# lzhangbj/ASVA

Measured on AMD Instinct MI355X. Metric: UNet denoising steps/sec, 12x256x256 bf16, CFG on, higher is better.
Workload: dtype bf16; 1 GPU; BASELINE configs[1]: AVSync15 shape, 1 clip(s) per GPU per forward, 12x256x256 (latent 12x32x32), SD1.5-shaped AudioUNet3D 1.17B params random-init, CFG batch 2 (audio guidance 4.0), DDIM-50 schedule, step = UNet forward + guidance + scheduler update; clips_per_gpu=1, unet_batch=2, frames=12, launch=hipGraph replay, parallelism=dp1 (independent clips)

## Files before the change

### asva_amd/_lib.py

```python
from __future__ import annotations

import ctypes as C
import os

import torch

from . import precision as P

_HERE = os.path.dirname(os.path.abspath(__file__))
LIB_PATH = os.environ.get("AVSD_LIB_PATH") or os.path.join(_HERE, "libavsd_hip.so")
LIB_PATHS = {"bf16": LIB_PATH, "fp16": os.environ.get("AVSD_LIB_PATH_F16") or os.path.join(_HERE, "libavsd_hip_f16.so")}

c_void_p, c_int, c_float, c_int64 = C.c_void_p, C.c_int, C.c_float, C.c_int64


class GemmDesc(C.Structure):

    _fields_ = [
        ("A", c_void_p), ("A2", c_void_p), ("W", c_void_p), ("out", c_void_p),
        ("bias", c_void_p), ("rowvec", c_void_p), ("res1", c_void_p), ("res2", c_void_p),
        ("M", C.c_int32), ("N", C.c_int32), ("K", C.c_int32),
        ("lda", C.c_int32), ("lda2", C.c_int32), ("k_split", C.c_int32), ("ldw", C.c_int32),
        ("ldc", C.c_int32), ("ldr1", C.c_int32), ("ldr2", C.c_int32),
        ("rows_per_vec", C.c_int32), ("ldv", C.c_int32),
        ("alpha", C.c_float),
        ("mode", C.c_int32), ("flags", C.c_int32), ("batch", C.c_int32),
        ("batch_stride_a", C.c_int64), ("batch_stride_w", C.c_int64), ("batch_stride_out", C.c_int64),
        ("hw", C.c_int32), ("frames", C.c_int32), ("cseg", C.c_int32),
        ("hs", C.c_int32), ("ws", C.c_int32), ("ho", C.c_int32), ("wo", C.c_int32),
        ("cin", C.c_int32), ("stride", C.c_int32), ("ups", C.c_int32), ("pad", C.c_int32),
        ("tile", C.c_int32),
        ("split_k", C.c_int32), ("splitk_ws", c_void_p),
        ("rowstats", c_void_p), ("ln_stats", c_void_p), ("ln_colsum", c_void_p), ("ln_nblk", C.c_int32), ("ln_eps", C.c_float),
        ("out_master", c_void_p), ("ldm", C.c_int32), ("raster_g", C.c_int32),
        ("a_lo", C.c_int64), ("a2_lo", C.c_int64), ("w_lo", C.c_int64), ("out_lo", C.c_int64), ("res1_lo", C.c_int64),
        ("res2_lo", C.c_int64),
        ("stats_pos", c_void_p), ("ln_rowvec", c_void_p), ("pos_hw", C.c_int32), ("pos_frames", C.c_int32),
    ]


class XAttnDesc(C.Structure):

    _fields_ = [
        ("h", c_void_p), ("ldh", C.c_int32), ("res_f32", C.c_int32),
        ("res", c_void_p), ("ldres", C.c_int32),
        ("M", C.c_int32), ("C", C.c_int32), ("heads", C.c_int32), ("L", C.c_int32),
        ("ln_stats", c_void_p), ("ln_eps", C.c_float), ("scale", C.c_float),
        ("wq", c_void_p), ("ldwq", C.c_int32), ("lk", C.c_int32),
        ("q_colsum", c_void_p), ("q_bias", c_void_p),
        ("k", c_void_p), ("vt", c_void_p),
        ("lk_pad", C.c_int32), ("q_per_kv", C.c_int32),
        ("wo", c_void_p), ("ldwo", C.c_int32), ("ldo", C.c_int32),
        ("o_bias", c_void_p), ("out", c_void_p),
        ("out_master", c_void_p), ("ldm", C.c_int32), ("reserved0", C.c_int32),
        ("rowstats", c_void_p),
        ("stats_pos", c_void_p), ("pos_hw", C.c_int32), ("pos_frames", C.c_int32),
    ]


SIGNATURES = {
    "avsd_abi_version": (c_int, []),
    "avsd_precision": (C.c_char_p, []),
    "avsd_last_error": (C.c_char_p, []),
    "avsd_device_info": (c_int, [C.c_char_p, c_int, C.POINTER(c_int)]),
    "avsd_gemm_bf16": (c_int, [C.POINTER(GemmDesc), c_void_p]),
    "avsd_sizeof_gemm_desc": (c_int, []),
    "avsd_cross_attention_block": (c_int, [C.POINTER(XAttnDesc), c_void_p]),
    "avsd_gemm_conv3r_supported": (c_int, [c_int, c_int, c_int, c_int]),
    "avsd_gemm_conv3r2d_supported": (c_int, [c_int, c_int, c_int, c_int]),
    "avsd_cross_attention_block_supported": (c_int, [c_int, c_int, c_int]),
    "avsd_sizeof_xattn_desc": (c_int, []),
    "avsd_linear_small_m": (c_int, [c_void_p, c_void_p, c_void_p, c_void_p, c_int, c_int, c_int, c_int, c_int, c_int, c_void_p]),
    "avsd_groupnorm_stats": (c_int, [c_void_p, c_int, c_int, c_void_p, c_int, c_int, c_int, c_int, c_int, c_void_p, c_int, c_void_p]),
    "avsd_groupnorm_apply": (c_int, [c_void_p, c_int, c_int, c_void_p, c_int, c_int, c_int, c_int, c_int, c_void_p, c_void_p, c_float,
                                     c_void_p, c_int, c_int, c_void_p, c_int, c_void_p]),
    "avsd_ln_fold": (c_int, [c_void_p, c_int, c_int, c_void_p, c_void_p]),
    "avsd_groupnorm_fused_supported": (c_int, [c_int, c_int, c_int, c_int, c_int, c_int]),
    "avsd_groupnorm_fused": (c_int, [c_void_p, c_int, c_int, c_void_p, c_int, c_int, c_int, c_int, c_int, c_void_p, c_void_p, c_float,
                                     c_int, c_void_p, c_int, c_void_p]),
    "avsd_groupnorm_nchunks": (c_int, [c_int, c_int, c_int]),
    "avsd_groupnorm_scratch_floats": (c_int, [c_int, c_int, c_int, c_int]),
    "avsd_layernorm": (c_int, [c_void_p, c_int, c_void_p, c_int, c_int, c_int, c_void_p, c_void_p, c_float, c_void_p, c_int, c_int, c_void_p]),
    "avsd_softmax_rows": (c_int, [c_void_p, c_int, c_void_p, c_int, c_int, c_int, c_void_p]),
    "avsd_attention": (c_int, [c_void_p, c_int, c_void_p, c_int, c_void_p, c_int, c_void_p, c_int, c_int, c_int, c_int, c_int,
                               c_int, c_int, c_int, c_void_p, c_int, c_float, c_void_p]),
    "avsd_attention_fp8": (c_int, [c_void_p, c_int, c_void_p, c_int, c_void_p, c_int, c_void_p, c_int, c_int, c_int, c_int, c_int,
                                   c_int, c_int, c_int, c_void_p, c_int, c_float, c_float, c_float, c_float, c_void_p]),
    "avsd_temporal_attention": (c_int, [c_void_p, c_int, c_void_p, c_int, c_int, c_int, c_int, c_int, c_int, c_float, c_void_p]),
    "avsd_ncfhw_to_rows": (c_int, [c_void_p, c_void_p, c_int, c_int, c_int, c_int, c_int, c_int, c_float, c_void_p]),
    "avsd_rows_to_ncfhw": (c_int, [c_void_p, c_int, c_void_p, c_int, c_int, c_int, c_int, c_void_p]),
    "avsd_timestep_embedding": (c_int, [c_void_p, c_void_p, c_int, c_int, c_void_p]),
    "avsd_guided_step": (c_int, [c_void_p, c_int, c_float, c_float, c_void_p, c_int, c_float, C.POINTER(C.c_int32), C.POINTER(C.c_float),
                                 c_int, c_void_p, c_void_p, c_float, c_float, c_int, c_int, c_int, c_int, c_void_p]),
    "avsd_guided_multistep": (c_int, [c_void_p, c_int, c_float, c_float, c_void_p, c_int, C.POINTER(C.c_int32), C.POINTER(C.c_float),
                                      c_int, c_void_p, c_void_p, c_float, c_float, c_float, c_float, c_int, c_int, c_int, c_int, c_void_p]),
    "avsd_vae_postprocess":(c_int, [c_void_p, c_int, c_void_p, c_int, c_int, c_void_p]),
    "avsd_vae_postprocess_u8": (c_int, [c_void_p, c_int, c_void_p, c_int, c_int, c_void_p]),
    "avsd_kaldi_fbank": (c_int, [c_void_p, c_int, c_int, C.c_int64, c_void_p, c_void_p, c_int, c_int, c_int, c_int, c_float, c_int,
                                 c_void_p, c_int, c_float, c_float, c_void_p]),
    "avsd_resample_sinc_f32": (c_int, [c_void_p, c_int, c_int, c_int64, c_void_p, c_int, c_int, c_int, c_void_p, c_int, c_int64, c_void_p]),
    "avsd_patchify": (c_int, [c_void_p, c_void_p, c_int, c_int, c_int, c_int, c_int, c_int, c_int, c_void_p]),
    "avsd_vit_tokens": (c_int, [c_void_p, c_void_p, c_void_p, c_void_p, c_int, c_int, c_int, c_int, c_void_p]),
    "avsd_copy": (c_int, [c_void_p, c_void_p, c_int64, c_int, c_void_p]),
    "avsd_xattn_pack_kv": (c_int, [c_void_p, c_int, c_int, c_int, c_void_p, c_int, c_int, c_void_p, c_void_p, c_int, c_void_p]),
    "avsd_linear_small_m_x2": (c_int, [c_void_p, c_void_p, c_int64, c_void_p, c_void_p, c_int, c_int, c_int, c_int, c_int, c_int, c_void_p]),
    "avsd_groupnorm_stats_x2": (c_int, [c_void_p, c_int, c_int, c_int64, c_void_p, c_int, c_int, c_int64, c_int, c_int, c_int, c_void_p,
                                        c_int, c_void_p]),
    "avsd_groupnorm_apply_x2": (c_int, [c_void_p, c_int, c_int, c_int64, c_void_p, c_int, c_int, c_int64, c_int, c_int, c_int, c_void_p,
                                        c_void_p, c_float, c_void_p, c_int, c_int, c_void_p, c_int, c_int64, c_void_p]),
    "avsd_groupnorm_fused_x2": (c_int, [c_void_p, c_int, c_int, c_int64, c_void_p, c_int, c_int, c_int64, c_int, c_int, c_int, c_void_p,
                                        c_void_p, c_float, c_int, c_void_p, c_int, c_int64, c_void_p]),
    "avsd_layernorm_x2": (c_int, [c_void_p, c_int, c_int64, c_void_p, c_int, c_int64, c_int, c_int, c_void_p, c_void_p, c_float, c_void_p,
                                  c_int, c_int, c_void_p]),
    "avsd_attention_x2": (c_int, [c_void_p, c_int, c_int64, c_void_p, c_int, c_int64, c_void_p, c_int, c_int64, c_void_p, c_int, c_int64,
                                  c_int, c_int, c_int, c_int, c_int, c_int, c_int, c_void_p, c_int, c_float, c_void_p]),
    "avsd_temporal_attention_x2": (c_int, [c_void_p, c_int, c_int64, c_void_p, c_int, c_int64, c_int, c_int, c_int, c_int, c_int, c_float,
                                           c_void_p]),
    "avsd_softmax_rows_x2": (c_int, [c_void_p, c_int, c_void_p, c_int, c_int64, c_int, c_int, c_void_p]),
    "avsd_ncfhw_to_rows_x2": (c_int, [c_void_p, c_void_p, c_int64, c_int, c_int, c_int, c_int, c_int, c_int, c_float, c_void_p]),
    "avsd_split_f32": (c_int, [c_void_p, c_void_p, c_int64, c_int64, c_void_p]),
# ... 83 lines not shown
```

### asva_amd/build.py

```python
from __future__ import annotations

import os
import subprocess
import sys
from concurrent.futures import ThreadPoolExecutor

HERE = os.path.dirname(os.path.abspath(__file__))
CSRC = os.path.join(HERE, "csrc")
OBJ = os.path.join(CSRC, "_obj")
LIB = os.path.join(HERE, "libavsd_hip.so")
VARIANTS = {"bf16": ("", LIB, []), "fp16": ("_f16", os.path.join(HERE, "libavsd_hip_f16.so"), ["-DAVSD_F16=1"])}
SOURCES = ["lib.hip", "attention.hip", "attention_x2.hip", "gemm_f32.hip", "gemm4.hip", "nstream.hip", "conv3r.hip", "norm.hip", "groupnorm_fused.hip", "elementwise.hip", "audio.hip", "xattn.hip", "attention_fp8.hip", "avsync.hip", "clip_text.hip", "imagebind_eval.hip", "plan.hip"]
GEMM_UNITS = 7
HEADERS = [os.path.join(CSRC, "avsd_common.h"), os.path.join(CSRC, "gemm_common.h"), os.path.join(CSRC, "gemm4_loops.inc"),
           os.path.join(HERE, "..", "include", "avsd.h")]
FLAGS = ["--offload-arch=gfx950", "-O3", "-std=c++17", "-fPIC", "-Wall", "-Wno-unused-function"]


PLAN_HOST = os.path.join(HERE, "plan_host")


def _hipcc() -> str:
    for cand in (os.environ.get("HIPCC"), "/opt/rocm/bin/hipcc", "hipcc"):
        if cand and (os.path.isabs(cand) and os.path.exists(cand) or not os.path.isabs(cand)):
            return cand
    raise RuntimeError("hipcc not found")


def _stale(target: str, deps: list[str]) -> bool:
    if not os.path.exists(target):
        return True
    t = os.path.getmtime(target)
    return any(os.path.getmtime(d) > t for d in deps)


def build(verbose: bool = False, force: bool = False, variants=("bf16", "fp16")) -> str:
    hipcc = _hipcc()
    jobs = []
    links = []
    for var in variants:
        suffix, lib, defs = VARIANTS[var]
        objdir = OBJ + suffix
        os.makedirs(objdir, exist_ok=True)
        objs = []
        stale = False
        for src in SOURCES:
            s = os.path.join(CSRC, src)
            o = os.path.join(objdir, src.replace(".hip", ".o"))
            objs.append(o)
            if force or _stale(o, [s] + HEADERS):
                jobs.append([hipcc, *FLAGS, *defs, "-c", s, "-o", o])
                stale = True
        gsrc = os.path.join(CSRC, "gemm.hip")
        for u in range(GEMM_UNITS):
            o = os.path.join(objdir, f"gemm_tu{u}.o")
            objs.append(o)
            if force or _stale(o, [gsrc] + HEADERS):
                jobs.insert(0, [hipcc, *FLAGS, *defs, f"-DAVSD_GEMM_TU={u}", "-c", gsrc, "-o", o])
                stale = True
        links.append((lib, objs, stale))

    def run(cmd):
        if verbose:
            print(" ".join(cmd), flush=True)
        r = subprocess.run(cmd, capture_output=True, text=True)
        if r.returncode != 0:
            raise RuntimeError(f"hipcc failed: {' '.join(cmd)}\n{r.stdout}\n{r.stderr}")
        if verbose and r.stderr.strip():
            print(r.stderr, file=sys.stderr)

    with ThreadPoolExecutor(max_workers=min(7, max(1, len(jobs)))) as ex:
        list(ex.map(run, jobs))
    for lib, objs, stale in links:
        if force or stale or _stale(lib, objs):
            run([hipcc, "--offload-arch=gfx950", "-shared", "-fPIC", "-o", lib, *objs])
    host_src = os.path.join(HERE, "..", "tools", "plan_host.cpp")
    if os.path.exists(host_src) and (force or _stale(PLAN_HOST, [host_src] + HEADERS)):
        run([hipcc, "-O2", "-std=c++17", "-I", os.path.join(HERE, "..", "include"), host_src, "-ldl", "-o", PLAN_HOST])
    return LIB


if __name__ == "__main__":
    print(build(verbose=True, force="--force" in sys.argv))
```

### asva_amd/csrc/gemm.hip

```cpp
#include "avsd_common.h"
#include "gemm_common.h"

namespace {

constexpr int LDS_STRIDE = BK + 8;

struct RowInfo {
  int64_t o0, o1, o2;
  int hb, wb;
  bool valid;
};

template <int MODE>
__device__ __forceinline__ RowInfo make_row(const avsd_gemm_desc& p, int m) {
  RowInfo r;
  r.valid = m < p.M;
  r.o0 = r.o1 = r.o2 = 0;
  r.hb = r.wb = 0;
  if (!r.valid) return r;
  if (MODE == AVSD_GEMM_PLAIN) {
    r.o0 = (int64_t)m * p.lda;
    r.o1 = (int64_t)m * p.lda2;
  } else if (MODE == AVSD_GEMM_TMIX) {
    const int f = (m / p.hw) % p.frames;
// ... 156 lines not shown
int launch(const avsd_gemm_desc& d, hipStream_t s) {
  constexpr size_t lds = (size_t)2 * (BM + BN) * LDS_STRIDE * sizeof(h16_t);
  static bool attr_set = false;
  if (!attr_set) {
    hipError_t e = hipFuncSetAttribute(reinterpret_cast<const void*>(&gemm_kernel<BM, BN, MODE, EX>),
                                       hipFuncAttributeMaxDynamicSharedMemorySize, (int)lds);
    if (e != hipSuccess) {
      avsd_set_error("gemm: hipFuncSetAttribute(%zu B LDS): %s", lds, hipGetErrorString(e));
      return AVSD_ELAUNCH;
    }
    attr_set = true;
  }
  const int ntm = (d.M + BM - 1) / BM, ntn = (d.N + BN - 1) / BN;
  dim3 grid((unsigned)(ntm * ntn), 1, (unsigned)d.batch);
  hipLaunchKernelGGL((gemm_kernel<BM, BN, MODE, EX>), grid, dim3(256), lds, s, d);
  AVSD_CHECK_LAUNCH("gemm launch");
  return AVSD_OK;
}


constexpr unsigned OOB = 0x80000000u;

struct RowInfo32 {
  int o0, o1, o2;
  int hb, wb;
  bool valid;
};

template <int MODE>
__device__ __forceinline__ RowInfo32 make_row32(const avsd_gemm_desc& p, int m) {
  RowInfo32 r;
  r.valid = m < p.M;
  r.o0 = r.o1 = r.o2 = r.hb = r.wb = 0;
  if (!r.valid) return r;
  if (MODE == AVSD_GEMM_PLAIN) {
    r.o0 = m * p.lda;
    r.o1 = m * p.lda2;
  } else if (MODE == AVSD_GEMM_TMIX) {
    const int f = (m / p.hw) % p.frames;
    r.o0 = (m - f * p.hw) * p.lda;
    r.o1 = (f > 0 ? m - p.hw : m) * p.lda;
    r.o2 = m * p.lda;
  } else {
    const int per = p.ho * p.wo;
    const int n = m / per;
    const int rem = m - n * per;
    const int oh = rem / p.wo;
    r.o0 = n;
    r.hb = oh * p.stride - p.pad;
    r.wb = (rem - oh * p.wo) * p.stride - p.pad;
  }
  return r;
}

template <int MODE>
__device__ __forceinline__ unsigned a_voffset(const avsd_gemm_desc& p, const RowInfo32& r, int k0) {
  if (!r.valid || k0 >= p.K) return OOB;
  if (MODE == AVSD_GEMM_PLAIN) {
    return (unsigned)((k0 < p.k_split) ? (r.o0 + k0) : (r.o1 + (k0 - p.k_split))) * 2u;
  } else if (MODE == AVSD_GEMM_TMIX) {
    const int seg = k0 / p.cseg;
    const int kk = k0 - seg * p.cseg;
    const int o = r.o2 + (seg == 0 ? r.o0 - r.o2 : 0) + (seg == 1 ? r.o1 - r.o2 : 0);
    return (unsigned)(o + kk) * 2u;
  } else {
    const int tap = k0 / p.cin;
    const int c = k0 - tap * p.cin;
    const int kh = tap / 3;
    const int kw = tap - kh * 3;
    const int hi = r.hb + kh;
    const int wi = r.wb + kw;
    if (tap >= 9 || hi < 0 || hi >= (p.hs << p.ups) || wi < 0 || wi >= (p.ws << p.ups)) return OOB;
    return (unsigned)(((r.o0 * p.hs + (hi >> p.ups)) * p.ws + (wi >> p.ups)) * p.lda + c) * 2u;
  }
}

constexpr int gemm2_min_waves(int bm, int bn, int stages, bool x2, int waves) {
  const int lds = stages * (bm + bn) * 128 * (x2 ? 2 : 1);
  const int wgs = (160 * 1024) / lds < 1 ? 1 : (160 * 1024) / lds;
  const int w = (wgs * waves + 3) / 4;
  return w > 3 ? 3 : w;
}
constexpr int MODE_SUBPIX = 3;
template <int BM, int BN, int WM, int WN, int STAGES, int MODE, int LW = 0, bool X2 = false, int EX = EPI_PLAIN>
__global__ __launch_bounds__(64 * (WM * WN + LW), gemm2_min_waves(BM, BN, STAGES, X2, WM * WN + LW)) void gemm2_kernel(const avsd_gemm_desc p) {
  extern __shared__ __attribute__((aligned(1024))) unsigned char smem2[];
  constexpr int NC = WM * WN;
  constexpr int NWAVES = LW > 0 ? LW : NC;
  constexpr int A_BYTES = BM * 128;
  constexpr int W_BYTES = BN * 128;
  constexpr int PLANE_BYTES = A_BYTES + W_BYTES;
  constexpr int STAGE_BYTES = PLANE_BYTES * (X2 ? 2 : 1);
  constexpr int PA = (BM / 8) / NWAVES;
  constexpr int PW = (BN / 8) / NWAVES;
  static_assert(PA * NWAVES * 8 == BM && PW * NWAVES * 8 == BN, "tile rows must split evenly into 1-KiB pieces per wave");
  constexpr int LPT = (PA + PW) * (X2 ? 2 : 1);
  static_assert((STAGES - 2) * LPT < 64, "vmcnt is a 6-bit counter");
  constexpr int FM = BM / WM / 32;
  constexpr int FN = BN / WN / 32;

  const int tid = threadIdx.x;
  const int lane = tid & 63;
  const int wave_all = __builtin_amdgcn_readfirstlane(tid >> 6);
  const bool is_loader = LW == 0 || wave_all >= NC;
  const int wave = LW == 0 ? wave_all : (wave_all >= NC ? wave_all - NC : 0);
  const int wm = wave_all % WM;
  const int wn = (wave_all / WM) % WN;

  const int ntm = (p.M + BM - 1) / BM;
  const int ntn = (p.N + BN - 1) / BN;
  const int nwg = ntm * ntn;
  const int nsplit = p.split_k > 1 ? p.split_k : 1;
  int wg, ksplit;
  {
    const int total = nwg * nsplit;
    const int bid = blockIdx.y * gridDim.x + blockIdx.x;
    const int q = total >> 3, r = total & 7;
    const int xcd = bid & 7, idx = bid >> 3;
    const int c = (xcd < r ? xcd * (q + 1) : r * (q + 1) + (xcd - r) * q) + idx;
    wg = c / nsplit;
    ksplit = c - wg * nsplit;
  }
  int tm, tn;
  tile_of_item(wg, ntm, ntn, (p.flags & AVSD_GEMM_XCD_N) != 0, p.raster_g, tm, tn);
  const int64_t bz = blockIdx.z;
  const int nk_all = (p.K + BK - 1) / BK;
  const int per_split = (nk_all + nsplit - 1) / nsplit;
  const int kt0 = ksplit * per_split;
  const int kt1 = min(nk_all, kt0 + per_split);

  const h16_t* Ab = reinterpret_cast<const h16_t*>(p.A) + bz * p.batch_stride_a;
  const h16_t* A2b = p.A2 ? reinterpret_cast<const h16_t*>(p.A2) + bz * p.batch_stride_a : Ab;
  const h16_t* Wb = reinterpret_cast<const h16_t*>(p.W) + bz * p.batch_stride_w;
  const __amdgpu_buffer_rsrc_t rsA = __builtin_amdgcn_make_buffer_rsrc((void*)Ab, 0, 0x7fffffff, 0x00020000);
  const __amdgpu_buffer_rsrc_t rsA2 = __builtin_amdgcn_make_buffer_rsrc((void*)A2b, 0, 0x7fffffff, 0x00020000);
  const __amdgpu_buffer_rsrc_t rsW = __builtin_amdgcn_make_buffer_rsrc((void*)Wb, 0, 0x7fffffff, 0x00020000);
  const __amdgpu_buffer_rsrc_t rsAr = __builtin_amdgcn_make_buffer_rsrc((void*)(Ab + (X2 ? p.a_lo : 0)), 0, 0x7fffffff, 0x00020000);
  const __amdgpu_buffer_rsrc_t rsA2r = __builtin_amdgcn_make_buffer_rsrc((void*)(A2b + (X2 ? (p.A2 ? p.a2_lo : p.a_lo) : 0)), 0, 0x7fffffff, 0x00020000);
  const __amdgpu_buffer_rsrc_t rsWr = __builtin_amdgcn_make_buffer_rsrc((void*)(Wb + (X2 ? p.w_lo : 0)), 0, 0x7fffffff, 0x00020000);

  int ro0[PA], ro1[PA], ro2[PA], rhb[PA], rwb[PA], kca[PA];
  bool rvalid[PA];
#pragma unroll
  for (int j = 0; j < PA; ++j) {
    const int L = (wave + j * NWAVES) * 4 + (lane >> 4);
    const int x = (lane & 15) ^ (L & 15);
    const RowInfo32 r = make_row32<MODE>(p, tm * BM + 2 * L + (x >> 3));
    ro0[j] = r.o0; ro1[j] = r.o1; ro2[j] = r.o2; rhb[j] = r.hb; rwb[j] = r.wb; rvalid[j] = r.valid;
    kca[j] = (x & 7) * 8;
  }
  int wo[PW], kcw[PW];
  bool wv[PW];
#pragma unroll
  for (int j = 0; j < PW; ++j) {
    const int L = (wave + j * NWAVES) * 4 + (lane >> 4);
    const int x = (lane & 15) ^ (L & 15);
    const int n = tn * BN + 2 * L + (x >> 3);
    wv[j] = n < p.N;
    kcw[j] = (x & 7) * 8;
    wo[j] = n * p.ldw + kcw[j];
  }

  const bool fast = (MODE == AVSD_GEMM_PLAIN) || (MODE == AVSD_GEMM_TMIX && p.cseg % BK == 0) ||
                    ((MODE == AVSD_GEMM_CONV3 || MODE == MODE_SUBPIX) && p.cin % BK == 0);
  const int nk_slice = max(kt1 - kt0, 0);
  const int krot = ((p.flags & AVSD_GEMM_KROT) && nk_slice > 1 && ntm > 1) ? (int)(((long long)tm * nk_slice) / ntm) : 0;
  constexpr bool subpix = MODE == MODE_SUBPIX;
  constexpr int KS = subpix ? 2 : 3;
  const int ush = subpix ? 0 : p.ups;
  const int sub_par = subpix ? (tn * BN) / (p.N >> 2) : 0;
  const int sub_dy = sub_par >> 1, sub_dx = sub_par & 1;
  int i_kbase = 0;
  int i_c0 = 0;
  int i_kh = 0, i_kw = 0, i_seg = 0;
  bool i_second = false;
  auto seek = [&](int kbase) {
    i_kbase = kbase;
    if (MODE == AVSD_GEMM_PLAIN) {
      i_c0 = i_kbase;
      i_second = p.A2 != nullptr && i_kbase >= p.k_split;
    } else if (MODE == AVSD_GEMM_TMIX) {
      i_seg = i_kbase / p.cseg;
      i_c0 = i_kbase - i_seg * p.cseg;
    } else {
      const int tap = i_kbase / p.cin;
      i_c0 = i_kbase - tap * p.cin;
      i_kh = tap / KS;
      i_kw = tap - i_kh * KS;
    }
  };
  seek((kt0 + krot) * BK);
  const int hin = p.hs << ush, win = p.ws << ush;
  int abase[PA];
  bool aok[PA];

  auto rebase = [&]() {
#pragma unroll
    for (int j = 0; j < PA; ++j) {
      if (MODE == AVSD_GEMM_PLAIN) {
        abase[j] = (i_second ? ro1[j] - p.k_split : ro0[j]) + kca[j];
        aok[j] = rvalid[j];
      } else if (MODE == AVSD_GEMM_TMIX) {
        const int o = ro2[j] + (i_seg == 0 ? ro0[j] - ro2[j] : 0) + (i_seg == 1 ? ro1[j] - ro2[j] : 0);
        abase[j] = o + kca[j];
        aok[j] = rvalid[j] && i_seg < 3;
      } else {
        const int hi = rhb[j] + i_kh + sub_dy;
        const int wi = rwb[j] + i_kw + sub_dx;
        aok[j] = rvalid[j] && i_kh < KS && (unsigned)hi < (unsigned)hin && (unsigned)wi < (unsigned)win;
        abase[j] = ((ro0[j] * p.hs + (hi >> ush)) * p.ws + (wi >> ush)) * p.lda + kca[j];
      }
    }
  };
  rebase();

  auto issue = [&](int stage) {
    unsigned char* sb = smem2 + stage * STAGE_BYTES;
    const int kbase = i_kbase;
#pragma unroll
    for (int j = 0; j < PA; ++j) {
      unsigned vo;
      if (!fast) {
        RowInfo32 r;
        r.o0 = ro0[j]; r.o1 = ro1[j]; r.o2 = ro2[j]; r.hb = rhb[j]; r.wb = rwb[j]; r.valid = rvalid[j];
        vo = a_voffset<MODE>(p, r, kbase + kca[j]);
      } else {
        const bool ok = aok[j] && (kbase + kca[j] < p.K);
        vo = ok ? (unsigned)(abase[j] + i_c0) * 2u : OOB;
      }
      lds_ptr_t dst = (lds_ptr_t)(sb + (wave + j * NWAVES) * 1024);
      if (i_second) __builtin_amdgcn_raw_ptr_buffer_load_lds(rsA2, dst, 16, (int)vo, 0, 0, 0);
      else __builtin_amdgcn_raw_ptr_buffer_load_lds(rsA, dst, 16, (int)vo, 0, 0, 0);
      if constexpr (X2) {
        lds_ptr_t dr = (lds_ptr_t)(sb + PLANE_BYTES + (wave + j * NWAVES) * 1024);
        if (i_second) __builtin_amdgcn_raw_ptr_buffer_load_lds(rsA2r, dr, 16, (int)vo, 0, 0, 0);
        else __builtin_amdgcn_raw_ptr_buffer_load_lds(rsAr, dr, 16, (int)vo, 0, 0, 0);
      }
    }
#pragma unroll
    for (int j = 0; j < PW; ++j) {
      const unsigned vo = (wv[j] && kbase + kcw[j] < p.K) ? (unsigned)(wo[j] + kbase) * 2u : OOB;
      lds_ptr_t dst = (lds_ptr_t)(sb + A_BYTES + (wave + j * NWAVES) * 1024);
      __builtin_amdgcn_raw_ptr_buffer_load_lds(rsW, dst, 16, (int)vo, 0, 0, 0);
      if constexpr (X2) {
        lds_ptr_t dr = (lds_ptr_t)(sb + PLANE_BYTES + A_BYTES + (wave + j * NWAVES) * 1024);
        __builtin_amdgcn_raw_ptr_buffer_load_lds(rsWr, dr, 16, (int)vo, 0, 0, 0);
      }
    }
    i_kbase += BK;
    if (krot != 0 && i_kbase >= kt1 * BK) {
      seek(kt0 * BK);
      rebase();
    } else
    if (MODE == AVSD_GEMM_PLAIN) {
      i_c0 = i_kbase;
      if (!i_second && i_kbase >= p.k_split && i_kbase < p.K) { i_second = true; rebase(); }
    } else if (MODE == AVSD_GEMM_TMIX) {
      i_c0 += BK;
      if (i_c0 >= p.cseg) { i_c0 = 0; ++i_seg; rebase(); }
    } else {
      i_c0 += BK;
      if (i_c0 >= p.cin) {
        i_c0 = 0;
        if (++i_kw == KS) { i_kw = 0; ++i_kh; }
        rebase();
      }
    }
  };

  f32x16 acc[FN][FM];
#pragma unroll
  for (int a = 0; a < FN; ++a)
#pragma unroll
    for (int b = 0; b < FM; ++b)
#pragma unroll
      for (int r = 0; r < 16; ++r) acc[a][b][r] = 0.f;

  int a_line[FM], a_sw[FM], a_hi[FM];
#pragma unroll
  for (int b = 0; b < FM; ++b) {
    const int r = wm * (BM / WM) + b * 32 + (lane & 31);
    a_line[b] = (r >> 1) * 256;
    a_sw[b] = (r >> 1) & 15;
    a_hi[b] = (r & 1) << 3;
  }
  int w_line[FN], w_sw[FN], w_hi[FN];
#pragma unroll
  for (int a = 0; a < FN; ++a) {
    const int r = wn * (BN / WN) + a * 32 + (lane & 31);
    w_line[a] = (r >> 1) * 256;
    w_sw[a] = (r >> 1) & 15;
    w_hi[a] = (r & 1) << 3;
  }
  const int chalf = lane >> 5;

  const int nk = max(kt1 - kt0, 0);
  auto wait_stage = [&](int kt) {
    wait_tiles_ahead<STAGES - 2, LPT>(nk - 1 - kt);
  };
  if (is_loader) {
#pragma unroll
    for (int s = 0; s < STAGES - 1; ++s)
      if (s < nk) issue(s);
  }
  float pre_ln[2 * FM] = {};
  const bool pre = (p.flags & AVSD_GEMM_LNFUSE) != 0 && !(LW > 0 && is_loader);
  if (pre) {
#pragma unroll
    for (int b = 0; b < FM; ++b) {
      const int m = tm * BM + wm * (BM / WM) + b * 32 + (lane & 31);
      pre_ln[2 * b] = 1.f; pre_ln[2 * b + 1] = 0.f;
      if (m < p.M) ln_row_stats(p, m, bz, pre_ln[2 * b], pre_ln[2 * b + 1]);
    }
  }
  if (LW > 0 && is_loader) {
    for (int kt = 0; kt < nk; ++kt) {
      wait_stage(kt);
      __builtin_amdgcn_s_barrier();
      if (kt + STAGES - 1 < nk) issue((kt + STAGES - 1) % STAGES);
    }
    return;
  }

  for (int kt = 0; kt < nk; ++kt) {
    if (LW == 0) wait_stage(kt);
    __builtin_amdgcn_s_barrier();
    if (LW == 0 && kt + STAGES - 1 < nk) issue((kt + STAGES - 1) % STAGES);

    const unsigned char* sA = smem2 + (kt % STAGES) * STAGE_BYTES;
    const unsigned char* sW = sA + A_BYTES;
#pragma unroll
    for (int ks = 0; ks < BK / 16; ++ks) {
      const int c = ks * 2 + chalf;
      h16x8 xf[FM], wf[FN];
#pragma unroll
      for (int b = 0; b < FM; ++b)
        xf[b] = *reinterpret_cast<const h16x8*>(sA + a_line[b] + (((a_hi[b] | c) ^ a_sw[b]) << 4));
#pragma unroll
      for (int a = 0; a < FN; ++a)
        wf[a] = *reinterpret_cast<const h16x8*>(sW + w_line[a] + (((w_hi[a] | c) ^ w_sw[a]) << 4));
      if constexpr (X2) {
        h16x8 xr[FM], wr[FN];
#pragma unroll
        for (int b = 0; b < FM; ++b)
          xr[b] = *reinterpret_cast<const h16x8*>(sA + PLANE_BYTES + a_line[b] + (((a_hi[b] | c) ^ a_sw[b]) << 4));
#pragma unroll
        for (int a = 0; a < FN; ++a)
          wr[a] = *reinterpret_cast<const h16x8*>(sW + PLANE_BYTES + w_line[a] + (((w_hi[a] | c) ^ w_sw[a]) << 4));
        __builtin_amdgcn_s_setprio(1);
#pragma unroll
        for (int a = 0; a < FN; ++a)
#pragma unroll
          for (int b = 0; b < FM; ++b) {
            acc[a][b] = mfma32x32x16(wr[a], xf[b], acc[a][b], 0, 0, 0);
            acc[a][b] = mfma32x32x16(wf[a], xr[b], acc[a][b], 0, 0, 0);
            acc[a][b] = mfma32x32x16(wf[a], xf[b], acc[a][b], 0, 0, 0);
          }
        __builtin_amdgcn_s_setprio(0);
      } else {
      __builtin_amdgcn_s_setprio(1);
#pragma unroll
      for (int a = 0; a < FN; ++a)
#pragma unroll
        for (int b = 0; b < FM; ++b)
          acc[a][b] = mfma32x32x16(wf[a], xf[b], acc[a][b], 0, 0, 0);
      __builtin_amdgcn_s_setprio(0);
      }
    }
  }

  if (p.split_k > 1) {
    float* ws = p.splitk_ws + (int64_t)ksplit * p.M * p.N;
    const int hsel = (lane >> 5) * 4;
#pragma unroll
    for (int b = 0; b < FM; ++b) {
      const int m = tm * BM + wm * (BM / WM) + b * 32 + (lane & 31);
      if (m >= p.M) continue;
#pragma unroll
      for (int a = 0; a < FN; ++a)
#pragma unroll
        for (int q = 0; q < 4; ++q) {
          const int n = tn * BN + wn * (BN / WN) + a * 32 + 8 * q + hsel;
          if (n < p.N)
            *reinterpret_cast<float4*>(ws + (int64_t)m * p.N + n) =
                make_float4(acc[a][b][4 * q], acc[a][b][4 * q + 1], acc[a][b][4 * q + 2], acc[a][b][4 * q + 3]);
        }
    }
    if (p.split_k != 0x7fffffff) return;
#pragma unroll
    for (int a = 0; a < FN; ++a)
#pragma unroll
      for (int b = 0; b < FM; ++b)
#pragma unroll
        for (int r = 0; r < 16; ++r) acc[a][b][r] = 0.f;
    for (int sl = 0; sl < nsplit; ++sl) {
      const float* slab = p.splitk_ws + (int64_t)sl * p.M * p.N;
#pragma unroll
      for (int b = 0; b < FM; ++b) {
        const int m = min(tm * BM + wm * (BM / WM) + b * 32 + (lane & 31), p.M - 1);
#pragma unroll
        for (int a = 0; a < FN; ++a)
#pragma unroll
          for (int q = 0; q < 4; ++q) {
            const int n = min(tn * BN + wn * (BN / WN) + a * 32 + 8 * q + hsel, p.N - 4);
            const float4 v = *reinterpret_cast<const float4*>(slab + (int64_t)m * p.N + n);
            acc[a][b][4 * q] += v.x; acc[a][b][4 * q + 1] += v.y; acc[a][b][4 * q + 2] += v.z; acc[a][b][4 * q + 3] += v.w;
          }
      }
    }
  }
  if constexpr (subpix) {
    if constexpr (X2) epilogue_x2<FN, FM, true>(p, acc, tm * BM + wm * (BM / WM), tn * BN + wn * (BN / WN), lane, bz, pre_ln, pre);
    else epilogue_each<FN, FM, (64 * (WM * WN + LW) > 512), EPI_SHUF>(p, acc, tm * BM + wm * (BM / WM), tn * BN + wn * (BN / WN), lane, bz, pre_ln, pre);
  } else if constexpr (X2) epilogue_x2<FN, FM>(p, acc, tm * BM + wm * (BM / WM), tn * BN + wn * (BN / WN), lane, bz, pre_ln, pre);
  else if constexpr (EX == EPI_REST) {
    if constexpr (FN * FM >= 10) epilogue_each<FN, FM, (64 * (WM * WN + LW) > 512), EPI_REST>(p, acc, tm * BM + wm * (BM / WM), tn * BN + wn * (BN / WN), lane, bz, pre_ln, pre);
    else epilogue<FN, FM, (64 * (WM * WN + LW) > 512), EPI_REST>(p, acc, tm * BM + wm * (BM / WM), tn * BN + wn * (BN / WN), lane, bz, pre_ln, pre);
  } else if constexpr (FN * FM >= 10)
    epilogue_each<FN, FM, (64 * (WM * WN + LW) > 512)>(p, acc, tm * BM + wm * (BM / WM), tn * BN + wn * (BN / WN), lane, bz, pre_ln, pre);
  else epilogue<FN, FM, (64 * (WM * WN + LW) > 512)>(p, acc, tm * BM + wm * (BM / WM), tn * BN + wn * (BN / WN), lane, bz, pre_ln, pre);
}

template <int S, bool EXTRA = false>
__global__ __launch_bounds__(256) void splitk_reduce_kernel(const avsd_gemm_desc p) {
  const int nq = p.N / 4;
  const int64_t total = (int64_t)p.M * nq;
  const h16_t* R1 = reinterpret_cast<const h16_t*>(p.res1);
  const h16_t* R2 = reinterpret_cast<const h16_t*>(p.res2);
  const bool x2 = (p.flags & AVSD_GEMM_X2) != 0;
  const bool out_rest = EXTRA && (p.flags & AVSD_GEMM_OUT_REST) != 0;
  for (int64_t i = blockIdx.x * (int64_t)blockDim.x + threadIdx.x; i < total; i += (int64_t)gridDim.x * blockDim.x) {
    const int m = (int)(i / nq);
    const int n = (int)(i - (int64_t)m * nq) * 4;
    float4 acc = make_float4(0.f, 0.f, 0.f, 0.f);
    float4 pre_bias = make_float4(0.f, 0.f, 0.f, 0.f), pre_vec = pre_bias, pre_r1f = pre_bias, pre_r2f = pre_bias;
    uint2 pre_r1 = make_uint2(0, 0), pre_r1lo = pre_r1, pre_r2 = pre_r1, pre_r2lo = pre_r1;
    if (p.bias) pre_bias = *reinterpret_cast<const float4*>(p.bias + n);
    if (p.rowvec) pre_vec = *reinterpret_cast<const float4*>(p.rowvec + (int64_t)(m / p.rows_per_vec) * p.ldv + n);
    if (R1) {
      if (p.flags & AVSD_GEMM_RES1_F32) {
        pre_r1f = *reinterpret_cast<const float4*>(reinterpret_cast<const float*>(p.res1) + (int64_t)m * p.ldr1 + n);
      } else {
        pre_r1 = *reinterpret_cast<const uint2*>(R1 + (int64_t)m * p.ldr1 + n);
        if (x2) pre_r1lo = *reinterpret_cast<const uint2*>(R1 + p.res1_lo + (int64_t)m * p.ldr1 + n);
      }
    }
    if (R2) {
      if (p.flags & AVSD_GEMM_RES2_F32) {
        pre_r2f = *reinterpret_cast<const float4*>(reinterpret_cast<const float*>(p.res2) + (int64_t)m * p.ldr2 + n);
      } else {
        pre_r2 = *reinterpret_cast<const uint2*>(R2 + (int64_t)m * p.ldr2 + n);
        if (x2) pre_r2lo = *reinterpret_cast<const uint2*>(R2 + p.res2_lo + (int64_t)m * p.ldr2 + n);
      }
    }
    if constexpr (S > 0) {
      float4 sv[S];
#pragma unroll
      for (int s = 0; s < S; ++s) sv[s] = *reinterpret_cast<const float4*>(p.splitk_ws + ((int64_t)s * p.M + m) * p.N + n);
#pragma unroll
      for (int s = 0; s < S; ++s) { acc.x += sv[s].x; acc.y += sv[s].y; acc.z += sv[s].z; acc.w += sv[s].w; }
    } else {
      for (int s = 0; s < p.split_k; ++s) {
        const float4 v = *reinterpret_cast<const float4*>(p.splitk_ws + ((int64_t)s * p.M + m) * p.N + n);
        acc.x += v.x; acc.y += v.y; acc.z += v.z; acc.w += v.w;
      }
    }
    float v[4] = {p.alpha * acc.x, p.alpha * acc.y, p.alpha * acc.z, p.alpha * acc.w};
    if (p.flags & AVSD_GEMM_LNFUSE) {
      const float2* st = reinterpret_cast<const float2*>(p.ln_stats) + (int64_t)m * p.ln_nblk;
      float sm = 0.f, sq = 0.f;
      for (int j = 0; j < p.ln_nblk; ++j) { const float2 t = st[j]; sm += t.x; sq += t.y; }
      const float inv_k = 1.0f / (float)p.K;
      const float mean = sm * inv_k;
      const float rstd = rsqrtf(fmaxf(sq * inv_k - mean * mean, 0.f) + p.ln_eps);
      const float4 cs = *reinterpret_cast<const float4*>(p.ln_colsum + n);
      if (p.ln_rowvec) {
        const float4 pv = *reinterpret_cast<const float4*>(pos_row(p, p.ln_rowvec, m) + n);
        v[0] += pv.x; v[1] += pv.y; v[2] += pv.z; v[3] += pv.w;
      }
      v[0] = fmaf(v[0], rstd, -mean * rstd * cs.x); v[1] = fmaf(v[1], rstd, -mean * rstd * cs.y);
      v[2] = fmaf(v[2], rstd, -mean * rstd * cs.z); v[3] = fmaf(v[3], rstd, -mean * rstd * cs.w);
    }
    if (p.bias) { v[0] += pre_bias.x; v[1] += pre_bias.y; v[2] += pre_bias.z; v[3] += pre_bias.w; }
    if (p.rowvec) { v[0] += pre_vec.x; v[1] += pre_vec.y; v[2] += pre_vec.z; v[3] += pre_vec.w; }
    if (p.flags & AVSD_GEMM_GELU) {
      for (int i = 0; i < 4; ++i) v[i] = gelu_erf_f(v[i]);
    }
    if (R1) {
      if (p.flags & AVSD_GEMM_RES1_F32) {
        v[0] += pre_r1f.x; v[1] += pre_r1f.y; v[2] += pre_r1f.z; v[3] += pre_r1f.w;
      } else {
        v[0] += lo2f(pre_r1.x); v[1] += hi2f(pre_r1.x); v[2] += lo2f(pre_r1.y); v[3] += hi2f(pre_r1.y);
        if (x2) { v[0] += lo2f(pre_r1lo.x); v[1] += hi2f(pre_r1lo.x); v[2] += lo2f(pre_r1lo.y); v[3] += hi2f(pre_r1lo.y); }
// ... 12 lines not shown
    if (EXTRA && p.mode == AVSD_GEMM_CONV3 && p.ups == 2) {
      int radd;
      shuf_col(p, n, radd, no);
      mo = shuf_row(p, m) + radd;
    }
    if (p.out_master) *reinterpret_cast<float4*>(p.out_master + mo * p.ldm + no) = make_float4(v[0], v[1], v[2], v[3]);
    const int64_t o = mo * p.ldc + no;
    if (p.flags & AVSD_GEMM_OUT_F32) {
      *reinterpret_cast<float4*>(reinterpret_cast<float*>(p.out) + o) = make_float4(v[0], v[1], v[2], v[3]);
    } else {
      uint2 st;
      st.x = pack2h(v[0], v[1]);
      st.y = pack2h(v[2], v[3]);
      *reinterpret_cast<uint2*>(reinterpret_cast<h16_t*>(p.out) + o) = st;
      float e0 = 0.f, e1 = 0.f, e2 = 0.f, e3 = 0.f;
      if (x2 || out_rest) {
        uint2 sr;
        sr.x = pack2h(v[0] - lo2f(st.x), v[1] - hi2f(st.x));
        sr.y = pack2h(v[2] - lo2f(st.y), v[3] - hi2f(st.y));
        *reinterpret_cast<uint2*>(reinterpret_cast<h16_t*>(p.out) + p.out_lo + o) = sr;
        if (x2) { e0 = lo2f(sr.x); e1 = hi2f(sr.x); e2 = lo2f(sr.y); e3 = hi2f(sr.y); }
      }
      if (p.flags & AVSD_GEMM_ROWSTATS) {
        float a0 = lo2f(st.x) + e0, a1 = hi2f(st.x) + e1;
        float a2 = lo2f(st.y) + e2, a3 = hi2f(st.y) + e3;
        if (p.stats_pos) {
          const float4 pv = *reinterpret_cast<const float4*>(pos_row(p, p.stats_pos, m) + n);
          a0 += pv.x; a1 += pv.y; a2 += pv.z; a3 += pv.w;
        }
        float sm = (a0 + a1) + (a2 + a3);
        float sq = fmaf(a0, a0, fmaf(a1, a1, fmaf(a2, a2, a3 * a3)));
#pragma unroll
        for (int off = 1; off < 8; off <<= 1) {
          sm += __shfl_xor(sm, off, 64);
          sq += __shfl_xor(sq, off, 64);
        }
        if ((threadIdx.x & 7) == 0)
          reinterpret_cast<float2*>(p.rowstats)[(int64_t)m * (p.N >> 5) + (n >> 5)] = make_float2(sm, sq);
      }
    }
  }
}

template <int BM, int BN, int WM, int WN, int STAGES, int MODE, int LW = 0, bool X2 = false, int EX = EPI_PLAIN>
int launch2(const avsd_gemm_desc& d, hipStream_t s) {
  constexpr size_t lds = (size_t)STAGES * (BM + BN) * 128 * (X2 ? 2 : 1);
  static_assert(lds <= 160 * 1024, "tile does not fit the 160 KB of LDS");
  if (MODE == MODE_SUBPIX && (d.N / 4) % BN != 0) {
    avsd_set_error("gemm/conv3: ups = 2 needs whole column tiles per output-pixel parity: cout (%d) %% %d != 0 for this tile", d.N / 4, BN);
    return AVSD_EINVAL;
  }
  static bool attr_set = false;
  if (!attr_set) {
    hipError_t e = hipFuncSetAttribute(reinterpret_cast<const void*>(&gemm2_kernel<BM, BN, WM, WN, STAGES, MODE, LW, X2, EX>),
                                       hipFuncAttributeMaxDynamicSharedMemorySize, (int)lds);
    if (e != hipSuccess) {
      avsd_set_error("gemm2: hipFuncSetAttribute(%zu B LDS): %s", lds, hipGetErrorString(e));
      return AVSD_ELAUNCH;
    }
    attr_set = true;
  }
  const int ntm = (d.M + BM - 1) / BM, ntn = (d.N + BN - 1) / BN;
  const int nsplit = d.split_k > 1 ? d.split_k : 1;
  dim3 grid((unsigned)(ntm * ntn), (unsigned)nsplit, (unsigned)d.batch);
  hipLaunchKernelGGL((gemm2_kernel<BM, BN, WM, WN, STAGES, MODE, LW, X2, EX>), grid, dim3(64 * (WM * WN + LW)), lds, s, d);
  AVSD_CHECK_LAUNCH("gemm2 launch");
  if (nsplit > 1) {
    const int64_t total = (int64_t)d.M * (d.N / 4);
    int64_t g = (total + 255) / 256;
    if (g > 2048) g = 2048;
    if (MODE == MODE_SUBPIX || (d.flags & AVSD_GEMM_OUT_REST)) {
      hipLaunchKernelGGL((splitk_reduce_kernel<0, true>), dim3((unsigned)g), dim3(256), 0, s, d);
    } else
    switch (nsplit) {
      case 2: hipLaunchKernelGGL(splitk_reduce_kernel<2>, dim3((unsigned)g), dim3(256), 0, s, d); break;
      case 4: hipLaunchKernelGGL(splitk_reduce_kernel<4>, dim3((unsigned)g), dim3(256), 0, s, d); break;
      case 8: hipLaunchKernelGGL(splitk_reduce_kernel<8>, dim3((unsigned)g), dim3(256), 0, s, d); break;
      case 3: hipLaunchKernelGGL(splitk_reduce_kernel<3>, dim3((unsigned)g), dim3(256), 0, s, d); break;
      case 5: hipLaunchKernelGGL(splitk_reduce_kernel<5>, dim3((unsigned)g), dim3(256), 0, s, d); break;
      default: hipLaunchKernelGGL(splitk_reduce_kernel<0>, dim3((unsigned)g), dim3(256), 0, s, d); break;
    }
    AVSD_CHECK_LAUNCH("gemm split-K reduce launch");
  }
  return AVSD_OK;
}

template <int MODE, int EX = EPI_PLAIN>
int dispatch_tile(const avsd_gemm_desc& d, int tile, hipStream_t s) {
  switch (tile) {
    case 1: return launch<128, 128, MODE, EX>(d, s);
    case 2: return launch<128, 64, MODE, EX>(d, s);
    case 3: return launch<64, 64, MODE, EX>(d, s);
    case 4: return launch2<128, 64, 2, 2, 3, MODE, 0, false, EX>(d, s);
    case 6: return launch2<128, 128, 2, 4, 3, MODE, 0, false, EX>(d, s);
    case 7: return launch2<64, 64, 2, 2, 4, MODE, 0, false, EX>(d, s);
    case 9: return launch2<256, 128, 4, 2, 3, MODE, 0, false, EX>(d, s);
    case 11: return launch2<128, 128, 2, 2, 2, MODE, 0, false, EX>(d, s);
    case 12: return launch2<128, 64, 2, 2, 2, MODE, 0, false, EX>(d, s);
    case 13: return launch2<64, 64, 2, 2, 2, MODE, 0, false, EX>(d, s);
    case 14: return launch2<256, 128, 4, 2, 2, MODE, 0, false, EX>(d, s);
    case 17: return launch2<128, 320, 4, 2, 2, MODE, 0, false, EX>(d, s);
    case 19: return launch2<256, 320, 4, 2, 2, MODE, 0, false, EX>(d, s);
    case 20: return launch2<256, 128, 4, 2, 3, MODE, 4, false, EX>(d, s);
    case 24: return launch2<128, 64, 2, 2, 3, MODE, 2, false, EX>(d, s);
    case 25: return launch2<64, 64, 2, 2, 4, MODE, 2, false, EX>(d, s);
    case 30: return launch2<128, 128, 2, 4, 4, MODE, 0, false, EX>(d, s);
    case 31: return launch2<128, 256, 2, 4, 3, MODE, 0, false, EX>(d, s);
    case AVSD_GEMM_TILE_256x160_8W: return launch2<256, 160, 8, 1, 3, MODE, 4, false, EX>(d, s);
    default:
      avsd_set_error("gemm: tile id %d is not built (gemm.hip dispatch_tile)", tile);
      return AVSD_EINVAL;
  }
}

template <int MODE>
int dispatch_tile_x2(const avsd_gemm_desc& d, int tile, hipStream_t s) {
  switch (tile) {
    case 7: return launch2<64, 64, 2, 2, 4, MODE, 0, true>(d, s);
    case 11: return launch2<128, 128, 2, 2, 2, MODE, 0, true>(d, s);
    case 13: return launch2<64, 64, 2, 2, 2, MODE, 0, true>(d, s);
    case 24: return launch2<128, 64, 2, 2, 3, MODE, 2, true>(d, s);
    case 25: return launch2<64, 64, 2, 2, 4, MODE, 2, true>(d, s);
    case 34: return launch2<128, 160, 4, 1, 2, MODE, 0, true>(d, s);
    case 35: return launch2<256, 64, 4, 2, 2, MODE, 0, true>(d, s);
    case 36: return launch2<128, 192, 2, 2, 2, MODE, 0, true>(d, s);
    default:
      avsd_set_error("gemm: AVSD_GEMM_X2 runs on tiles 7, 11, 13, 24, 25, 34, 35, 36 (got %d)", tile);
      return AVSD_EINVAL;
  }
}

int pick_tile(int M, int N, int batch) {
  static int num_cu = 0;
  if (num_cu == 0) {
    hipDeviceProp_t prop;
    int dev = 0;
    if (hipGetDevice(&dev) == hipSuccess && hipGetDeviceProperties(&prop, dev) == hipSuccess)
      num_cu = prop.multiProcessorCount;
    if (num_cu <= 0) num_cu = 256;
  }
  const int bm[3] = {128, 128, 64}, bn[3] = {128, 64, 64};
  const double eff[3] = {1.0, 0.85, 0.62};
  const int slots[3] = {2 * num_cu, 3 * num_cu, 4 * num_cu};
  int best = 3;
  double best_cost = 1e300;
  for (int t = 0; t < 3; ++t) {
    const long blocks = (long)((M + bm[t] - 1) / bm[t]) * ((N + bn[t] - 1) / bn[t]) * batch;
    const long waves = (blocks + slots[t] - 1) / slots[t];
    const double cost = (double)waves * bm[t] * bn[t] / eff[t] * slots[t];
    if (cost < best_cost) { best_cost = cost; best = t + 1; }
  }
  return best;
}

}

int avsd_gemm_dispatch_plain(const avsd_gemm_desc& d, int tile, hipStream_t s);
int avsd_gemm_dispatch_tmix(const avsd_gemm_desc& d, int tile, hipStream_t s);
int avsd_gemm_dispatch_conv3(const avsd_gemm_desc& d, int tile, hipStream_t s);
#ifdef AVSD_F16
#define AVSD_DISPATCH_TILE(MODE) ((d.flags & AVSD_GEMM_OUT_REST) ? dispatch_tile<MODE, EPI_REST>(d, tile, s) : dispatch_tile<MODE>(d, tile, s))
#else
#define AVSD_DISPATCH_TILE(MODE) dispatch_tile<MODE>(d, tile, s)
#endif
#if !defined(AVSD_GEMM_TU) || AVSD_GEMM_TU == 0
int avsd_gemm_dispatch_plain(const avsd_gemm_desc& d, int tile, hipStream_t s) { return AVSD_DISPATCH_TILE(AVSD_GEMM_PLAIN); }
#endif
#if !defined(AVSD_GEMM_TU) || AVSD_GEMM_TU == 1
int avsd_gemm_dispatch_tmix(const avsd_gemm_desc& d, int tile, hipStream_t s) { return AVSD_DISPATCH_TILE(AVSD_GEMM_TMIX); }
#endif
#if !defined(AVSD_GEMM_TU) || AVSD_GEMM_TU == 2
int avsd_gemm_dispatch_conv3(const avsd_gemm_desc& d, int tile, hipStream_t s) { return AVSD_DISPATCH_TILE(AVSD_GEMM_CONV3); }
#endif
int avsd_gemm_dispatch_subpix(const avsd_gemm_desc& d, int tile, hipStream_t s);
int avsd_gemm_dispatch_x2_subpix(const avsd_gemm_desc& d, int tile, hipStream_t s);
#if !defined(AVSD_GEMM_TU) || AVSD_GEMM_TU == 6
int avsd_gemm_dispatch_subpix(const avsd_gemm_desc& d, int tile, hipStream_t s) {
  switch (tile) {
    case 4: return launch2<128, 64, 2, 2, 3, MODE_SUBPIX>(d, s);
    case 6: return launch2<128, 128, 2, 4, 3, MODE_SUBPIX>(d, s);
    case 9: return launch2<256, 128, 4, 2, 3, MODE_SUBPIX>(d, s);
    case 11: return launch2<128, 128, 2, 2, 2, MODE_SUBPIX>(d, s);
    case 13: return launch2<64, 64, 2, 2, 2, MODE_SUBPIX>(d, s);
    case 17: return launch2<128, 320, 4, 2, 2, MODE_SUBPIX>(d, s);
    case 20: return launch2<256, 128, 4, 2, 3, MODE_SUBPIX, 4>(d, s);
    case 24: return launch2<128, 64, 2, 2, 3, MODE_SUBPIX, 2>(d, s);
    case 25: return launch2<64, 64, 2, 2, 4, MODE_SUBPIX, 2>(d, s);
    case 30: return launch2<128, 128, 2, 4, 4, MODE_SUBPIX>(d, s);
    case AVSD_GEMM_TILE_256x160_8W: return launch2<256, 160, 8, 1, 3, MODE_SUBPIX, 4>(d, s);
    default:
      avsd_set_error("gemm/conv3: ups = 2 runs on tiles 4, 6, 9, 11, 13, 17, 20, 24, 25, 30, 38 (got %d)", tile);
      return AVSD_EINVAL;
  }
}
int avsd_gemm_dispatch_x2_subpix(const avsd_gemm_desc& d, int tile, hipStream_t s) {
  switch (tile) {
    case 7: return launch2<64, 64, 2, 2, 4, MODE_SUBPIX, 0, true>(d, s);
    case 11: return launch2<128, 128, 2, 2, 2, MODE_SUBPIX, 0, true>(d, s);
    case 13: return launch2<64, 64, 2, 2, 2, MODE_SUBPIX, 0, true>(d, s);
    case 24: return launch2<128, 64, 2, 2, 3, MODE_SUBPIX, 2, true>(d, s);
    case 25: return launch2<64, 64, 2, 2, 4, MODE_SUBPIX, 2, true>(d, s);
    case 34: return launch2<128, 160, 4, 1, 2, MODE_SUBPIX, 0, true>(d, s);
    case 35: return launch2<256, 64, 4, 2, 2, MODE_SUBPIX, 0, true>(d, s);
    default:
      avsd_set_error("gemm/conv3: ups = 2 with AVSD_GEMM_X2 runs on tiles 7, 11, 13, 24, 25, 34, 35 (got %d)", tile);
      return AVSD_EINVAL;
  }
}
#endif

int avsd_gemm_dispatch_x2_plain(const avsd_gemm_desc& d, int tile, hipStream_t s);
int avsd_gemm_dispatch_x2_tmix(const avsd_gemm_desc& d, int tile, hipStream_t s);
int avsd_gemm_dispatch_x2_conv3(const avsd_gemm_desc& d, int tile, hipStream_t s);
#if !defined(AVSD_GEMM_TU) || AVSD_GEMM_TU == 4
int avsd_gemm_dispatch_x2_plain(const avsd_gemm_desc& d, int tile, hipStream_t s) { return dispatch_tile_x2<AVSD_GEMM_PLAIN>(d, tile, s); }
int avsd_gemm_dispatch_x2_tmix(const avsd_gemm_desc& d, int tile, hipStream_t s) { return dispatch_tile_x2<AVSD_GEMM_TMIX>(d, tile, s); }
#endif
#if !defined(AVSD_GEMM_TU) || AVSD_GEMM_TU == 5
int avsd_gemm_dispatch_x2_conv3(const avsd_gemm_desc& d, int tile, hipStream_t s) { return dispatch_tile_x2<AVSD_GEMM_CONV3>(d, tile, s); }
#endif

#if !defined(AVSD_GEMM_TU) || AVSD_GEMM_TU == 3
int avsd_gemm_dispatch_conv3r(const avsd_gemm_desc& d, hipStream_t s);
int avsd_gemm_dispatch_asm(const avsd_gemm_desc& d, hipStream_t s);
int avsd_gemm_dispatch_nstream(const avsd_gemm_desc& d, hipStream_t s);

int avsd_gemm_splitk_reduce(const avsd_gemm_desc& d, hipStream_t s) {
  const int64_t total = (int64_t)d.M * (d.N / 4);
  int64_t g = (total + 255) / 256;
  if (g > 2048) g = 2048;
  if (d.flags & AVSD_GEMM_OUT_REST) {
    hipLaunchKernelGGL((splitk_reduce_kernel<0, true>), dim3((unsigned)g), dim3(256), 0, s, d);
  } else
  switch (d.split_k) {
    case 2: hipLaunchKernelGGL(splitk_reduce_kernel<2>, dim3((unsigned)g), dim3(256), 0, s, d); break;
    case 4: hipLaunchKernelGGL(splitk_reduce_kernel<4>, dim3((unsigned)g), dim3(256), 0, s, d); break;
    case 8: hipLaunchKernelGGL(splitk_reduce_kernel<8>, dim3((unsigned)g), dim3(256), 0, s, d); break;
    case 3: hipLaunchKernelGGL(splitk_reduce_kernel<3>, dim3((unsigned)g), dim3(256), 0, s, d); break;
    case 5: hipLaunchKernelGGL(splitk_reduce_kernel<5>, dim3((unsigned)g), dim3(256), 0, s, d); break;
    case 10: hipLaunchKernelGGL(splitk_reduce_kernel<10>, dim3((unsigned)g), dim3(256), 0, s, d); break;
    default: hipLaunchKernelGGL(splitk_reduce_kernel<0>, dim3((unsigned)g), dim3(256), 0, s, d); break;
  }
  AVSD_CHECK_LAUNCH("gemm split-K reduce launch");
  return AVSD_OK;
}

extern "C" int avsd_gemm_bf16(const avsd_gemm_desc* dp, void* stream) {
  AVSD_REQUIRE(dp != nullptr, "gemm: null descriptor");
  avsd_gemm_desc d = *dp;
  AVSD_REQUIRE(d.A && d.W && d.out, "gemm: A, W and out must be non-null");
  AVSD_REQUIRE(d.M > 0 && d.N > 0 && d.K > 0, "gemm: M,N,K must be positive (got %d,%d,%d)", d.M, d.N, d.K);
  AVSD_REQUIRE(!(d.flags & AVSD_GEMM_W_FRAG) || d.tile == AVSD_GEMM_TILE_NSTREAM, "gemm: fragment-ordered W (AVSD_GEMM_W_FRAG) is read by tile %d only (got %d)", AVSD_GEMM_TILE_NSTREAM, d.tile);
  if (d.flags & AVSD_GEMM_W_FRAG) d.ldw = d.K;
  AVSD_REQUIRE(d.K % 8 == 0 && d.ldw % 8 == 0 && d.ldw >= d.K, "gemm: K (%d) and ldw (%d) must be multiples of 8, ldw >= K", d.K, d.ldw);
  AVSD_REQUIRE(d.N % 4 == 0 && d.ldc % 4 == 0, "gemm: N (%d) and ldc (%d) must be multiples of 4", d.N, d.ldc);
  AVSD_REQUIRE(d.lda % 8 == 0, "gemm: lda (%d) must be a multiple of 8", d.lda);
  if (d.batch <= 0) d.batch = 1;
  AVSD_REQUIRE(d.raster_g >= 0 && d.raster_g <= 64, "gemm: raster_g (%d) must be 0 (library default) .. 64", d.raster_g);
  if (d.flags & AVSD_GEMM_GEGLU) AVSD_REQUIRE(d.N % 32 == 0, "gemm: GEGLU needs N %% 32 == 0 (got %d)", d.N);
  AVSD_REQUIRE(!((d.flags & AVSD_GEMM_GEGLU) && (d.flags & AVSD_GEMM_GELU)), "gemm: GEGLU and GELU are exclusive");
  if (d.flags & AVSD_GEMM_ROWSTATS) {
    AVSD_REQUIRE(d.rowstats, "gemm: ROWSTATS without a rowstats buffer");
    AVSD_REQUIRE(!(d.flags & (AVSD_GEMM_GEGLU | AVSD_GEMM_OUT_F32)) && d.N % 32 == 0 && d.ldc % 8 == 0 &&
                     (!d.res1 || d.ldr1 % 8 == 0) && (!d.res2 || d.ldr2 % 8 == 0),
                 "gemm: ROWSTATS needs bf16 output, N %% 32 == 0 and 16-byte-aligned rows");
  }
  if (d.flags & AVSD_GEMM_LNFUSE) {
    AVSD_REQUIRE(d.ln_stats && d.ln_colsum && d.ln_nblk > 0 && d.mode == AVSD_GEMM_PLAIN && !d.A2,
                 "gemm: LNFUSE needs ln_stats, ln_colsum, ln_nblk and a single-source PLAIN operand");
    AVSD_REQUIRE(d.ln_nblk * 32 == d.K || d.ln_nblk == 1, "gemm: LNFUSE statistics are K / 32 pairs per row or one pre-folded pair (got %d for K = %d)", d.ln_nblk, d.K);
    AVSD_REQUIRE(d.batch == 1 || d.batch_stride_a % d.lda == 0, "gemm: LNFUSE batch stride must be whole rows");
  }
  if (d.stats_pos || d.ln_rowvec) {
    AVSD_REQUIRE(d.pos_hw > 0 && d.pos_frames > 0 && d.batch == 1 && !(d.flags & AVSD_GEMM_X2),
                 "gemm: stats_pos / ln_rowvec need pos_hw > 0, pos_frames > 0, batch 1 and no AVSD_GEMM_X2 (got hw %d, frames %d)", d.pos_hw, d.pos_frames);
    AVSD_REQUIRE(!d.stats_pos || (d.flags & AVSD_GEMM_ROWSTATS), "gemm: stats_pos without AVSD_GEMM_ROWSTATS");
    AVSD_REQUIRE(!d.ln_rowvec || (d.flags & AVSD_GEMM_LNFUSE), "gemm: ln_rowvec without AVSD_GEMM_LNFUSE");
  }
  if (d.res1) AVSD_REQUIRE(d.ldr1 % 4 == 0, "gemm: ldr1 must be a multiple of 4");
  if (d.res2) AVSD_REQUIRE(d.ldr2 % 4 == 0, "gemm: ldr2 must be a multiple of 4");
  if (d.out_master) AVSD_REQUIRE(d.ldm % 4 == 0 && d.ldm >= ((d.mode == AVSD_GEMM_CONV3 && d.ups == 2) ? d.N / 4 : d.N) && !(d.flags & AVSD_GEMM_GEGLU),
                                 "gemm: out_master needs ldm %% 4 == 0, ldm >= N (ups = 2: cout) and no GEGLU");
  if (d.rowvec) AVSD_REQUIRE(d.rows_per_vec > 0 && d.ldv % 4 == 0, "gemm: rowvec needs rows_per_vec > 0 and ldv %% 4 == 0");
  if (d.flags & AVSD_GEMM_OUT_REST) {
#ifndef AVSD_F16
    AVSD_REQUIRE(d.mode == AVSD_GEMM_CONV3 && d.ups == 2,
                 "gemm: OUT_REST is compiled into the IEEE-half build only (libavsd_hip_f16.so: the per-layer precision plan is fp16 storage)");
#endif
    AVSD_REQUIRE(!(d.flags & (AVSD_GEMM_X2 | AVSD_GEMM_OUT_F32 | AVSD_GEMM_GEGLU)) && d.out_lo != 0 && (d.out_lo & 7) == 0 && d.batch == 1 &&
                     d.tile != AVSD_GEMM_TILE_NSTREAM && !(d.tile >= AVSD_GEMM_TILE_CONV3R_FIRST && d.tile <= AVSD_GEMM_TILE_CONV3R2D_LAST),
                 "gemm: OUT_REST is for one-pass 16-bit outputs (no X2 / OUT_F32 / GEGLU / batch, not on tiles 40..54 / 70) and needs out_lo %% 8 == 0, != 0");
  }
  if (d.mode == AVSD_GEMM_PLAIN) {
    if (!d.A2) d.k_split = d.K;
    AVSD_REQUIRE(d.k_split % 8 == 0 && d.k_split <= d.K, "gemm: k_split (%d) must be a multiple of 8 and <= K", d.k_split);
    if (d.A2) AVSD_REQUIRE(d.lda2 % 8 == 0, "gemm: lda2 must be a multiple of 8");
  } else if (d.mode == AVSD_GEMM_TMIX) {
    AVSD_REQUIRE(d.cseg > 0 && d.cseg % 8 == 0 && d.K == 3 * d.cseg, "gemm/tmix: K (%d) must equal 3*cseg (%d)", d.K, d.cseg);
    AVSD_REQUIRE(d.hw > 0 && d.frames > 0 && d.M % (d.hw * d.frames) == 0, "gemm/tmix: M (%d) must be a multiple of frames*hw (%d*%d)", d.M, d.frames, d.hw);
  } else if (d.mode == AVSD_GEMM_CONV3) {
    AVSD_REQUIRE(d.stride == 1 || d.stride == 2, "gemm/conv3: stride must be 1 or 2");
    if (d.ups == 2) {
      AVSD_REQUIRE(d.cin > 0 && d.cin % 64 == 0 && d.K == 4 * d.cin, "gemm/conv3: ups = 2 needs K (%d) == 4*cin (%d), cin %% 64 == 0", d.K, d.cin);
      AVSD_REQUIRE(d.stride == 1 && d.pad == 1 && d.hs > 0 && d.ws > 0 && d.ho == d.hs && d.wo == d.ws && d.M % (d.hs * d.ws) == 0,
                   "gemm/conv3: ups = 2 needs stride 1, pad 1, (ho, wo) = (hs, ws) and whole images");
      AVSD_REQUIRE(d.N % 4 == 0 && (d.N / 4) % 64 == 0 && d.ldc >= d.N / 4, "gemm/conv3: ups = 2 needs N = 4 * cout, cout %% 64 == 0, ldc >= cout");
      AVSD_REQUIRE(!d.A2 && !d.res1 && !d.res2 && !d.rowvec && !(d.flags & (AVSD_GEMM_GEGLU | AVSD_GEMM_GELU | AVSD_GEMM_ROWSTATS | AVSD_GEMM_LNFUSE)) && d.batch == 1,
                   "gemm/conv3: ups = 2 takes bias / out_master / the rest plane only");
      AVSD_REQUIRE((double)d.M * 4.0 * d.ldc < 2147483648.0, "gemm/conv3: ups = 2 output too large");
      AVSD_REQUIRE(d.tile >= 4 && !(d.tile >= AVSD_GEMM_TILE_CONV3R_FIRST && d.tile <= AVSD_GEMM_TILE_CONV3R2D_LAST) && !(d.tile >= AVSD_GEMM_TILE_ASM_FIRST),
                   "gemm/conv3: ups = 2 runs on the LDS-direct tiles (4..38), got %d", d.tile);
    } else {
    AVSD_REQUIRE(d.cin > 0 && d.cin % 8 == 0 && d.K == 9 * d.cin, "gemm/conv3: K (%d) must equal 9*cin (%d), cin %% 8 == 0", d.K, d.cin);
    AVSD_REQUIRE(d.ups == 0 || d.ups == 1, "gemm/conv3: ups must be 0, 1 or 2");
    AVSD_REQUIRE(d.pad == 0 || d.pad == 1, "gemm/conv3: pad must be 0 or 1");
    AVSD_REQUIRE(d.hs > 0 && d.ws > 0 && d.ho > 0 && d.wo > 0 && d.M % (d.ho * d.wo) == 0, "gemm/conv3: bad image geometry");
    const int hin = d.hs << d.ups, win = d.ws << d.ups;
    AVSD_REQUIRE(d.ho == (hin + 2 - 3) / d.stride + 1 && d.wo == (win + 2 - 3) / d.stride + 1, "gemm/conv3: (ho,wo)=(%d,%d) inconsistent with input (%d,%d) stride %d", d.ho, d.wo, hin, win, d.stride);
    }
  } else {
    AVSD_REQUIRE(false, "gemm: unknown mode %d", d.mode);
  }
  if ((d.tile >= AVSD_GEMM_TILE_CONV3R_FIRST && d.tile <= AVSD_GEMM_TILE_CONV3R_LAST) ||
      (d.tile >= AVSD_GEMM_TILE_CONV3R2D_FIRST && d.tile <= AVSD_GEMM_TILE_CONV3R2D_LAST)) {
    if (d.split_k > 1) AVSD_REQUIRE(d.splitk_ws != nullptr, "gemm: split_k needs a workspace");
    return avsd_gemm_dispatch_conv3r(d, reinterpret_cast<hipStream_t>(stream));
  }
  AVSD_REQUIRE(d.mode == AVSD_GEMM_PLAIN || !d.A2, "gemm: a two-source A needs the PLAIN mode or a resident convolution tile (40..54), got mode %d tile %d", d.mode, d.tile);
  if (d.tile == AVSD_GEMM_TILE_NSTREAM) return avsd_gemm_dispatch_nstream(d, reinterpret_cast<hipStream_t>(stream));
  const bool asm_tile = d.tile >= AVSD_GEMM_TILE_ASM_FIRST && d.tile <= AVSD_GEMM_TILE_ASM_LAST;
  if (asm_tile && !(d.flags & AVSD_GEMM_X2)) return avsd_gemm_dispatch_asm(d, reinterpret_cast<hipStream_t>(stream));
  if (d.split_k > 1 && !asm_tile) {
    AVSD_REQUIRE(d.splitk_ws != nullptr, "gemm: split_k needs a workspace");
    AVSD_REQUIRE(!(d.flags & AVSD_GEMM_GEGLU) && d.batch == 1, "gemm: split_k cannot be combined with GEGLU or batching");
    AVSD_REQUIRE((d.tile >= 4 && d.tile <= ((d.flags & AVSD_GEMM_X2) ? AVSD_GEMM_MAX_TILE_X2 : AVSD_GEMM_MAX_TILE)) ||
                     (!(d.flags & AVSD_GEMM_X2) && d.tile == AVSD_GEMM_TILE_256x160_8W),
                 "gemm: split_k needs an LDS-direct tile (4..33; split precision: ..36), got %d", d.tile);
    AVSD_REQUIRE(d.split_k <= (d.K + 63) / 64, "gemm: split_k (%d) exceeds the number of K tiles", d.split_k);
  }
  if (d.flags & AVSD_GEMM_X2) {
    AVSD_REQUIRE(d.a_lo != 0 && d.w_lo != 0 && (!d.A2 || d.a2_lo != 0), "gemm/x2: A, A2 and W need their rest-plane offsets");
    AVSD_REQUIRE((d.flags & AVSD_GEMM_OUT_F32) || d.out_lo != 0, "gemm/x2: a 16-bit output needs out_lo");
    AVSD_REQUIRE(!d.res1 || (d.flags & AVSD_GEMM_RES1_F32) || d.res1_lo != 0, "gemm/x2: a 16-bit res1 needs res1_lo");
    AVSD_REQUIRE(!d.res2 || (d.flags & AVSD_GEMM_RES2_F32) || d.res2_lo != 0, "gemm/x2: a 16-bit res2 needs res2_lo");
    AVSD_REQUIRE(((d.a_lo | d.a2_lo | d.w_lo | d.out_lo | d.res1_lo | d.res2_lo) & 7) == 0, "gemm/x2: plane offsets must be multiples of 8 elements");
    AVSD_REQUIRE(d.mode != AVSD_GEMM_PLAIN || !d.A2 || d.k_split % 64 == 0, "gemm/x2: a two-source A needs k_split %% 64 == 0 (got %d)", d.k_split);
    const double a_rows = d.mode == AVSD_GEMM_CONV3 ? (double)(d.M / (d.ho * d.wo)) * d.hs * d.ws : (double)d.M;
    AVSD_REQUIRE(a_rows * d.lda * 2.0 < 2147483648.0 && (double)d.N * d.ldw * 2.0 < 2147483648.0, "gemm/x2: operands must be < 2 GiB per plane");
    hipStream_t sx = reinterpret_cast<hipStream_t>(stream);
    if (asm_tile) return avsd_gemm_dispatch_asm(d, sx);
    switch (d.mode) {
      case AVSD_GEMM_PLAIN: return avsd_gemm_dispatch_x2_plain(d, d.tile, sx);
      case AVSD_GEMM_TMIX: return avsd_gemm_dispatch_x2_tmix(d, d.tile, sx);
      default: return d.ups == 2 ? avsd_gemm_dispatch_x2_subpix(d, d.tile, sx) : avsd_gemm_dispatch_x2_conv3(d, d.tile, sx);
    }
  }
  int tile = d.tile;
  {
    const double a_rows = d.mode == AVSD_GEMM_CONV3 ? (double)(d.M / (d.ho * d.wo)) * d.hs * d.ws : (double)d.M;
    const bool big = a_rows * d.lda * 2.0 >= 2147483648.0 || (double)d.N * d.ldw * 2.0 >= 2147483648.0 ||
                     (d.A2 && (double)d.M * d.lda2 * 2.0 >= 2147483648.0);
    AVSD_REQUIRE(!(big && d.mode == AVSD_GEMM_CONV3 && d.ups == 2), "gemm/conv3: ups = 2 needs operands < 2 GiB");
    if (big && (tile < 1 || tile > 3)) tile = (d.N > 64 && d.M > 2048) ? 1 : 3;
    if (d.mode == AVSD_GEMM_PLAIN && d.A2 && d.k_split % 64 != 0 && (tile < 1 || tile > 3)) {
      AVSD_REQUIRE(d.split_k <= 1, "gemm: split_k with a two-source A needs k_split %% 64 == 0 (got %d)", d.k_split);
      tile = (d.N > 64 && d.M > 2048) ? 2 : 3;
    }
  }
  if (tile < 1 || (tile > AVSD_GEMM_MAX_TILE && tile != AVSD_GEMM_TILE_256x160_8W)) tile = pick_tile(d.M, (d.flags & AVSD_GEMM_GEGLU) ? d.N : d.N, d.batch);
  hipStream_t s = reinterpret_cast<hipStream_t>(stream);
  switch (d.mode) {
    case AVSD_GEMM_PLAIN: return avsd_gemm_dispatch_plain(d, tile, s);
    case AVSD_GEMM_TMIX: return avsd_gemm_dispatch_tmix(d, tile, s);
    default: return d.ups == 2 ? avsd_gemm_dispatch_subpix(d, tile, s) : avsd_gemm_dispatch_conv3(d, tile, s);
  }
}
#endif
```

### asva_amd/csrc/gemm_common.h

```cpp
#pragma once
#include <utility>

#include "avsd_common.h"

namespace {

constexpr int BK = 64;

template <class F, int... I>
__device__ __forceinline__ void static_for_impl(F&& f, std::integer_sequence<int, I...>) {
  (f(std::integral_constant<int, I>{}), ...);
}
template <int N, class F>
__device__ __forceinline__ void static_for(F&& f) {
  static_for_impl(f, std::make_integer_sequence<int, N>{});
}

__device__ __forceinline__ void ln_row_stats(const avsd_gemm_desc& p, int m, int64_t bz, float& rstd, float& mr) {
  const float2* st = reinterpret_cast<const float2*>(p.ln_stats) + ((int64_t)bz * (p.batch_stride_a / p.lda) + m) * p.ln_nblk;
  float sm = 0.f, sq = 0.f;
  int j = 0;
  for (; j + 10 <= p.ln_nblk; j += 10) {
    float2 t[10];
#pragma unroll
    for (int u = 0; u < 10; ++u) t[u] = st[j + u];
#pragma unroll
    for (int u = 0; u < 10; ++u) { sm += t[u].x; sq += t[u].y; }
  }
  for (; j < p.ln_nblk; ++j) {
    const float2 t = st[j];
    sm += t.x;
    sq += t.y;
  }
  const float inv_k = 1.0f / (float)p.K;
  const float mean = sm * inv_k;
  const float var = fmaxf(sq * inv_k - mean * mean, 0.f);
  rstd = rsqrtf(var + p.ln_eps);
  mr = mean * rstd;
}

__device__ __forceinline__ const float* pos_row(const avsd_gemm_desc& p, const float* table, int m) {
  return table + (int64_t)((m / p.pos_hw) % p.pos_frames) * p.N;
}

__device__ __forceinline__ void rowstats16(const unsigned (&w8)[8], const float* pos16, float& sm, float& sq) {
  float pv[16];
#pragma unroll
  for (int i = 0; i < 16; ++i) pv[i] = 0.f;
  if (pos16) {
#pragma unroll
    for (int j = 0; j < 4; ++j) {
      const float4 t = *reinterpret_cast<const float4*>(pos16 + 4 * j);
      pv[4 * j] = t.x; pv[4 * j + 1] = t.y; pv[4 * j + 2] = t.z; pv[4 * j + 3] = t.w;
    }
  }
  sm = 0.f;
  sq = 0.f;
#pragma unroll
  for (int i = 0; i < 8; ++i) {
    const float lo = lo2f(w8[i]) + pv[2 * i], hi = hi2f(w8[i]) + pv[2 * i + 1];
    sm += lo + hi;
    sq = fmaf(lo, lo, fmaf(hi, hi, sq));
  }
}

constexpr int EPI_PLAIN = 0, EPI_REST = 1, EPI_SHUF = 2;
__device__ __forceinline__ unsigned rest2h(float v0, float v1, unsigned mainw) { return pack2h(v0 - lo2f(mainw), v1 - hi2f(mainw)); }
__device__ __forceinline__ int64_t shuf_row(const avsd_gemm_desc& p, int m) { return 4 * (int64_t)m - 2 * (m % p.ws); }
__device__ __forceinline__ void shuf_col(const avsd_gemm_desc& p, int n, int& radd, int& col) {
  const int cout = p.N >> 2, par = n / cout;
  col = n - par * cout;
  radd = (par >> 1) * 2 * p.ws + (par & 1);
}
template <int EX>
__device__ __forceinline__ bool epi_rest(const avsd_gemm_desc& p) {
  if constexpr (EX == EPI_REST) return true;
  else if constexpr (EX == EPI_SHUF) return (p.flags & AVSD_GEMM_OUT_REST) != 0;
  else return false;
}

template <int FN, int FM>
__device__ __forceinline__ void epilogue_fence() {
  if constexpr (FN * FM >= 8) __builtin_amdgcn_sched_barrier(0);
}

template <int FN, int FM>
__device__ __forceinline__ void epilogue_add_residual(const avsd_gemm_desc& p, f32x16 (&acc)[FN][FM], const void* R, int ldr, bool f32,
                                                      const int (&mld)[FM], int n_base, int hsel, int nmax, int64_t bo, bool wide_ok) {
  if (f32) {
    const float* Rf = reinterpret_cast<const float*>(R) + bo;
#pragma unroll
    for (int b = 0; b < FM; ++b)
#pragma unroll
      for (int a = 0; a < FN; ++a) {
#pragma unroll
        for (int q = 0; q < 4; ++q) {
          const float4 rr = *reinterpret_cast<const float4*>(Rf + (int64_t)mld[b] * ldr + min(n_base + a * 32 + 8 * q + hsel, nmax));
          acc[a][b][4 * q + 0] += rr.x; acc[a][b][4 * q + 1] += rr.y; acc[a][b][4 * q + 2] += rr.z; acc[a][b][4 * q + 3] += rr.w;
        }
        epilogue_fence<FN, FM>();
      }
    return;
  }
  const h16_t* Rh = reinterpret_cast<const h16_t*>(R) + bo;
#pragma unroll
  for (int b = 0; b < FM; ++b)
#pragma unroll
    for (int a = 0; a < FN; ++a) {
      const int nb = n_base + a * 32;
      if (wide_ok && nb + 32 <= p.N) {
        const h16_t* rp = Rh + (int64_t)mld[b] * ldr + nb + 4 * hsel;
        const uint4 lo = *reinterpret_cast<const uint4*>(rp);
        const uint4 hi = *reinterpret_cast<const uint4*>(rp + 8);
        const unsigned s0[2] = {lo.x, lo.y}, s1[2] = {lo.z, lo.w}, s2[2] = {hi.x, hi.y}, s3[2] = {hi.z, hi.w};
#pragma unroll
        for (int d = 0; d < 2; ++d) {
          const auto e = __builtin_amdgcn_permlane32_swap(s0[d], s1[d], false, false);
          const auto o = __builtin_amdgcn_permlane32_swap(s2[d], s3[d], false, false);
          acc[a][b][0 + 2 * d] += lo2f(e[0]); acc[a][b][1 + 2 * d] += hi2f(e[0]);
          acc[a][b][8 + 2 * d] += lo2f(e[1]); acc[a][b][9 + 2 * d] += hi2f(e[1]);
          acc[a][b][4 + 2 * d] += lo2f(o[0]); acc[a][b][5 + 2 * d] += hi2f(o[0]);
          acc[a][b][12 + 2 * d] += lo2f(o[1]); acc[a][b][13 + 2 * d] += hi2f(o[1]);
        }
      } else {
#pragma unroll
        for (int q = 0; q < 4; ++q) {
          const uint2 rr = *reinterpret_cast<const uint2*>(Rh + (int64_t)mld[b] * ldr + min(nb + 8 * q + hsel, nmax));
          acc[a][b][4 * q + 0] += lo2f(rr.x); acc[a][b][4 * q + 1] += hi2f(rr.x);
          acc[a][b][4 * q + 2] += lo2f(rr.y); acc[a][b][4 * q + 3] += hi2f(rr.y);
        }
      }
      epilogue_fence<FN, FM>();
    }
}

template <int FN, int FM, int EX = EPI_PLAIN>
__device__ __forceinline__ void epilogue_by_term(const avsd_gemm_desc& p, f32x16 (&acc)[FN][FM], int m_base, int n_base,
                                                 int lane, int64_t bz, const float (&pre_ln)[2 * FM], bool have_pre, int mstride = 32) {
  const int frow = lane & 31;
  const bool geglu = (p.flags & AVSD_GEMM_GEGLU) != 0;
  const bool out_f32 = (p.flags & AVSD_GEMM_OUT_F32) != 0;
  const bool gelu = (p.flags & AVSD_GEMM_GELU) != 0;
  const bool lnfuse = (p.flags & AVSD_GEMM_LNFUSE) != 0;
  const bool rowstats = (p.flags & AVSD_GEMM_ROWSTATS) != 0;
  const bool r1f = (p.flags & AVSD_GEMM_RES1_F32) != 0, r2f = (p.flags & AVSD_GEMM_RES2_F32) != 0;
  const int hsel = (lane >> 5) * 4;
  const int64_t bo = bz * p.batch_stride_out;
  int mrow[FM], mld[FM];
#pragma unroll
// ... 625 lines not shown
```

### asva_amd/ops.py

```python
from __future__ import annotations

import os
import ctypes as C
from typing import Optional

import torch

from . import _lib
from . import precision as P
from ._lib import GemmDesc, XAttnDesc, check

PLAIN, TMIX, CONV3 = 0, 1, 2
GEGLU, OUT_F32, GELU, XCD_N, ROWSTATS, LNFUSE, RES1_F32, RES2_F32, X2, KROT, W_FRAG, OUT_REST = 1, 2, 4, 8, 16, 32, 64, 128, 256, 512, 1024, 2048
_XCD_MODE = "auto"
F32 = torch.float32


class KernelTimer:

    def __init__(self):
        self.records = []
        self.replays = []

    def start(self):
        ev = torch.cuda.Event(enable_timing=True)
        ev.record()
        return ev

    def stop(self, ev0, family: str, flops: float, nbytes: float, flops_once: Optional[float] = None, flops_ref: Optional[float] = None):
        ev1 = torch.cuda.Event(enable_timing=True)
        ev1.record()
        once = flops if flops_once is None else flops_once
        self.records.append((family, flops, nbytes, ev0, ev1, once, once if flops_ref is None else flops_ref))

    def add_replay(self, family: str, fn, keep):
        self.replays.append((family, fn, keep))

    def replay_ms(self, families, reps: int = 3) -> float:
        fns = [fn for fam, fn, _ in self.replays if fam in families]
        g = torch.cuda.CUDAGraph()
        with torch.cuda.graph(g):
            for fn in fns:
                fn()
        g.replay()
        e0, e1 = torch.cuda.Event(enable_timing=True), torch.cuda.Event(enable_timing=True)
        e0.record()
        for _ in range(reps):
            g.replay()
        e1.record()
        e1.synchronize()
        return e0.elapsed_time(e1) / reps

    def summary(self):
        torch.cuda.synchronize()
        out = {}
        for fam, fl, nb, e0, e1, fo, fr in self.records:
            d = out.setdefault(fam, {"launches": 0, "ms": 0.0, "flops": 0.0, "bytes": 0.0, "flops_once": 0.0, "flops_ref": 0.0})
            d["launches"] += 1
            d["ms"] += e0.elapsed_time(e1)
            d["flops"] += fl
            d["bytes"] += nb
            d["flops_once"] += fo
            d["flops_ref"] += fr
        return out


_TIMER: Optional[KernelTimer] = None


def set_timer(t: Optional[KernelTimer]) -> None:
    global _TIMER
    _TIMER = t


def _timed(family: str, flops: float, nbytes: float, keep, *calls) -> None:
    ev = _TIMER.start() if _TIMER is not None else None
    for c in calls:
        c()
    if ev is not None:
        _TIMER.add_replay(family, lambda: [c() for c in calls], keep)
        _TIMER.stop(ev, family, flops, nbytes)


def _nbytes(*ts) -> float:
    return float(sum(t.numel() * t.element_size() for t in ts if t is not None))


def _stream() -> int:
    return torch.cuda.current_stream().cuda_stream


TILE_CANDIDATES = ((4, 1), (6, 1), (7, 1), (9, 1), (3, 1), (11, 1), (12, 1), (13, 1), (14, 1), (17, 1), (19, 1),
                   (20, 1), (24, 1), (25, 1), (30, 1), (31, 1), (38, 1))
SPLITK_CANDIDATES = ((6, 2), (6, 4), (6, 8), (9, 2), (9, 4), (4, 2), (4, 4), (4, 8), (7, 2), (7, 4),
                     (20, 2), (20, 4), (24, 2), (24, 4), (24, 8), (25, 2), (25, 4),
                     (30, 2), (30, 4), (30, 8), (31, 2), (31, 4), (31, 8))
X2_TILE_CANDIDATES = ((7, 1), (11, 1), (13, 1), (24, 1), (25, 1), (34, 1), (35, 1), (36, 1))
X2_SPLITK_CANDIDATES = ((34, 2), (34, 4), (35, 2), (35, 4), (36, 2), (36, 4), (7, 2), (7, 4), (7, 8), (11, 2), (11, 4), (24, 2), (24, 4), (24, 8), (25, 2), (25, 4), (25, 8))
ASM_CANDIDATES = ((60, 1), (61, 1), (62, 1), (63, 1), (64, 1), (65, 1), (66, 1), (67, 1))
ASM_SPLITK_CANDIDATES = ((63, 2), (63, 4), (63, 8), (61, 2), (62, 2), (62, 4), (64, 2), (64, 4), (65, 2), (65, 4), (66, 2), (66, 4),
                         (67, 2), (67, 3), (67, 4), (67, 5), (67, 6))
ASM_TILES = tuple(range(60, 68))
SUBPIX_TILES = (4, 6, 9, 11, 13, 17, 20, 24, 25, 30, 38)
SUBPIX_X2_TILES = (7, 11, 13, 24, 25, 34, 35)
TILE_BN = {4: 64, 6: 128, 7: 64, 9: 128, 11: 128, 12: 64, 13: 64, 14: 128, 17: 320, 19: 320, 20: 128, 24: 64, 25: 64, 30: 128, 31: 256, 34: 160,
           35: 64, 36: 192, 38: 160}
_SUBPIX_RELATIVE = {14: 20, 12: 24, 19: 17, 7: 25}
_SUBPIX_BY_BN = ({320: 17, 160: 38, 128: 11, 64: 24}, {160: 34, 128: 11, 64: 24})
ASM_X2_CANDIDATES = ((63, 1), (64, 1), (65, 1), (66, 1))
ASM_X2_SPLITK_CANDIDATES = ((63, 2), (63, 4), (64, 2), (64, 4), (65, 2), (65, 4), (66, 2), (66, 4), (66, 8))
_ASM_TILES = True
_KROT = os.environ.get("AVSD_KROT", "1") != "0"
_KROT_ASM_ONLY = False
_KROT_MAX_W = 16 << 20


def set_krot(on: bool) -> None:
    global _KROT
    _KROT = bool(on)


def _subpix_tile(tile: int, cout: int, x2: bool) -> int:
    if cout <= 0 or cout % 64:
        raise ValueError(f"gemm: ups = 2 needs cout % 64 == 0 (got {cout})")
    built = SUBPIX_X2_TILES if x2 else SUBPIX_TILES

    def ok(t):
        return t in built and cout % TILE_BN[t] == 0

    if ok(tile):
        return tile
    if ok(_SUBPIX_RELATIVE.get(tile, 0)):
        return _SUBPIX_RELATIVE[tile]
    bn0 = TILE_BN.get(tile, 128)
    return next(t for bn, t in sorted(_SUBPIX_BY_BN[int(x2)].items(), reverse=True) if bn <= max(bn0, 64) and ok(t))


NSTREAM_TILE = 70
_NSTREAM = os.environ.get("AVSD_NSTREAM", "1") != "0"


def nstream_supported(M: int, N: int, K: int) -> bool:
    return K in (320, 640) and N % 256 == 0 and N >= 4 * K and M >= 96


_RASTER_G = 0
CONV3R_TILES = (40, 42, 43, 44, 48)
CONV3R2D_TILES = (51, 52, 53, 54)
_CONV3R2D_BN = {51: 128, 52: 160, 53: 128, 54: 128}
CONV3R_SPLITS = (1, 2, 4, 5, 8, 10)
_CONV3R = True


_CONV3R_BN = (128, 128, 160, 160, 128, 128, 256, 320, 256, 64)


def conv3r_candidates(hs: int, ws: int, cin: int, M: int, N: int, one_d_only: bool = False):
    out = []
    for t in CONV3R_TILES:
        bm = _lib.lib().avsd_gemm_conv3r_supported(t, hs, ws, cin)
        if bm <= 0:
            continue
        bn = _CONV3R_BN[t - 40]
        wgs = ((M + bm - 1) // bm) * ((N + bn - 1) // bn)
        for sk in CONV3R_SPLITS:
            if sk > 1 and (wgs >= 256 or (cin // 64) // sk < 2 or (cin // 64) % sk != 0):
                continue
            out.append((t, sk))
    if not one_d_only:
        for t in CONV3R2D_TILES:
            bm = _lib.lib().avsd_gemm_conv3r2d_supported(t, hs, ws, cin)
            if bm <= 0:
                continue
            wgs = (M // bm) * ((N + _CONV3R2D_BN[t] - 1) // _CONV3R2D_BN[t])
            for sk in CONV3R_SPLITS:
                if sk > 1 and (wgs >= 256 or (cin // 64) // sk < 2 or (cin // 64) % sk != 0):
                    continue
                out.append((t, sk))
    return tuple(out)


def _heuristic_conv3r(cands, M: int, N: int):
    def cost(c):
        t, sk = c
        bn = _CONV3R_BN[t - 40] if t < 50 else _CONV3R2D_BN[t]
        bm = 256 if t in (40, 41, 42, 43, 48, 51, 52, 53) else 128
        wg = ((M + bm - 1) // bm) * ((N + bn - 1) // bn) * sk
        pad = ((N + bn - 1) // bn) * bn / N
        return (round(pad, 2), abs(wg - 256) if wg < 256 else (wg - 256) // 4, sk)
    return min(cands, key=cost)


_TILE_CACHE: dict = {}
# ... 204 lines not shown


def from_act(t: torch.Tensor) -> torch.Tensor:
    if not P.SPLIT:
        return t.float()
    half = _lo(t)
    return t.float() + torch.as_strided(t, t.shape, t.stride(), t.storage_offset() + half).float()


def alloc_planes(shape, device):
    n = 1
    for d in shape:
        n *= int(d)
    npad = (n + 7) // 8 * 8
    buf = torch.empty((2, npad), dtype=P.ACT, device=device)
    return buf[0, :n].view(tuple(shape)), buf[1, :n].view(tuple(shape))


def split_planes(x: torch.Tensor):
    x = x.contiguous()
    _req(x, F32, "x")
    main, rest = alloc_planes(tuple(x.shape), x.device)
    check(_lib.lib().avsd_split_f32(_p(x), _p(main), _rest_off(main, rest), x.numel(), _stream()), "avsd_split_f32")
    return main, rest


def _rest_off(main: torch.Tensor, rest: Optional[torch.Tensor]) -> int:
    if rest is None:
        return 0
    if rest.dtype != main.dtype or rest.shape != main.shape or rest.stride() != main.stride():
        raise ValueError("rest plane must match its main plane in dtype, shape and strides")
    off = rest.data_ptr() - main.data_ptr()
    if off == 0 or off % 16:
        raise ValueError("rest plane must be a distinct tensor, a multiple of 8 elements away from its main plane")
    return off // 2


def _req(t: torch.Tensor, dtype, name: str):
    if t.dtype != dtype:
        raise TypeError(f"{name}: expected {dtype}, got {t.dtype}")
    if not t.is_cuda:
        raise ValueError(f"{name}: expected a device tensor (libavsd_hip.so has no host path)")
    if t.dim() >= 1 and t.stride(-1) != 1:
        raise ValueError(f"{name}: innermost dimension must be contiguous")


def _ld(t: torch.Tensor) -> int:
    return t.stride(0) if t.dim() == 2 else t.stride(-2)


def gemm(
    a: torch.Tensor,
    w: torch.Tensor,
    *,
    n: Optional[int] = None,
    k: Optional[int] = None,
    a2: Optional[torch.Tensor] = None,
    bias: Optional[torch.Tensor] = None,
    rowvec: Optional[torch.Tensor] = None,
    rows_per_vec: int = 0,
    res1: Optional[torch.Tensor] = None,
    res2: Optional[torch.Tensor] = None,
    alpha: float = 1.0,
    geglu: bool = False,
    gelu: bool = False,
    rowstats: Optional[torch.Tensor] = None,
    ln: Optional[tuple] = None,
    stats_pos: Optional[tuple] = None,
    ln_pos: Optional[tuple] = None,
    out_f32: bool = False,
    out: Optional[torch.Tensor] = None,
    master: Optional[torch.Tensor] = None,
    mode: int = PLAIN,
    tmix: Optional[tuple] = None,
    conv: Optional[tuple] = None,
    m: Optional[int] = None,
    tile: int = 0,
    split_k: int = 1,
    a_rest: Optional[torch.Tensor] = None,
    a2_rest: Optional[torch.Tensor] = None,
    w_rest: Optional[torch.Tensor] = None,
    out_rest: Optional[torch.Tensor] = None,
    w_frag: Optional[torch.Tensor] = None,
) -> torch.Tensor:
    _req(a, P.ACT, "a")
    _req(w, P.ACT, "w")
    planes = w_rest is not None
    if planes:
        if P.SPLIT:
            raise ValueError("gemm: explicit rest planes are for the non-split modes (split precision carries them implicitly)")
        if a_rest is None or (a2 is not None) != (a2_rest is not None) or rowstats is not None or ln is not None:
            raise ValueError("gemm: a three-pass product needs a_rest and w_rest (a2_rest with a2), no rowstats / LayerNorm fold")
        if out_f32 == (out_rest is not None) or (out_f32 and master is not None):
            raise ValueError("gemm: a three-pass product writes f32 (out_f32) or a (main, rest) pair of planes (out=, out_rest=; optional f32 master)")
        if any(r is not None and r.dtype != F32 for r in (res1, res2)):
            raise ValueError("gemm: a three-pass product reads f32 residuals")
    elif a_rest is not None or a2_rest is not None:
        raise ValueError("gemm: a_rest / a2_rest without w_rest")
    if out_rest is not None and (P.SPLIT or out_f32 or geglu or out is None):
        raise ValueError("gemm: out_rest goes with an explicit 16-bit `out` outside split precision (no GEGLU)")
    x2 = P.SPLIT or planes
    if x2 and mode == PLAIN and a2 is not None and a.shape[1] % 64 != 0:
        if res1 is not None and res2 is not None:
            raise ValueError("gemm: split precision with an unaligned two-source A supports one residual")
        if gelu or geglu or rowstats is not None or ln is not None or stats_pos is not None or ln_pos is not None or (master is not None and not planes) or n is not None \
                or k is not None or m is not None or tile or split_k != 1:
            raise ValueError("gemm: split precision with an unaligned two-source A takes bias / rowvec / one residual / alpha only")
        k1 = a.shape[1]
        part = gemm(a, w[:, :k1], alpha=alpha, out_f32=True, a_rest=a_rest, w_rest=None if w_rest is None else w_rest[:, :k1])
        return gemm(a2, w[:, k1:], bias=bias, rowvec=rowvec, rows_per_vec=rows_per_vec, res1=part, res2=res1 if res1 is not None else res2,
                    alpha=alpha, out_f32=out_f32, out=out, out_rest=out_rest, master=master, a_rest=a2_rest, w_rest=None if w_rest is None else w_rest[:, k1:])
    d = GemmDesc()
    N = w.shape[0] if n is None else n
    lda = _ld(a)
    if mode == PLAIN:
        M = a.shape[0] if m is None else m
        K1 = a.shape[1]
        K = K1 + (a2.shape[1] if a2 is not None else 0)
        if a2 is not None:
            _req(a2, P.ACT, "a2")
            d.A2, d.lda2, d.k_split = _p(a2), _ld(a2), K1
        else:
            d.k_split = K
        if k is not None:
            K = k
    elif mode == TMIX:
        hw, frames = tmix
        M = a.shape[0]
        cseg = a.shape[1]
        K = 3 * cseg
        d.hw, d.frames, d.cseg = hw, frames, cseg
    elif mode == CONV3:
        n_img, hs, ws, stride, ups = conv[:5]
        pad = conv[5] if len(conv) > 5 else 1
        cin = a.shape[1]
        if a2 is not None:
            _req(a2, P.ACT, "a2")
            d.A2, d.lda2, d.k_split = _p(a2), _ld(a2), cin
            cin += a2.shape[1]
        if ups == 2:
            if stride != 1 or pad != 1 or a2 is not None or N % 4 or w.shape[1] != 4 * cin or cin % 64 or (N // 4) % 64:
                raise ValueError("gemm: ups = 2 (sub-pixel upsample convolution) needs stride 1, pad 1, one source, w [4 cout, 4 cin], cin % 64 == 0, cout % 64 == 0")
            if geglu or gelu or rowstats is not None or ln is not None or res1 is not None or res2 is not None or rowvec is not None:
                raise ValueError("gemm: ups = 2 takes bias / master / out_rest only")
            ho, wo = hs, ws
            M = n_img * hs * ws
            K = 4 * cin
        else:
            hin, win = hs << ups, ws << ups
            ho, wo = (hin + 2 - 3) // stride + 1, (win + 2 - 3) // stride + 1
            M = n_img * ho * wo
            K = 9 * cin
        d.hs, d.ws, d.ho, d.wo, d.cin, d.stride, d.ups, d.pad = hs, ws, ho, wo, cin, stride, ups, pad
    else:
        raise ValueError(f"unknown gemm mode {mode}")
    n_out = N // 2 if geglu else N
    m_out = M
    if mode == CONV3 and d.ups == 2:
        m_out, n_out = 4 * M, N // 4
    if out is None:
        out = torch.empty((m_out, n_out), dtype=F32, device=a.device) if out_f32 else alloc16((m_out, n_out), a.device)
    else:
        _req(out, F32 if out_f32 else P.ACT, "out")
        if tuple(out.shape) != (m_out, n_out) and mode == CONV3 and d.ups == 2:
            raise ValueError(f"gemm: ups = 2 writes [{m_out}, {n_out}], got {tuple(out.shape)}")
    d.A, d.W, d.out = _p(a), _p(w), _p(out)
    d.M, d.N, d.K = M, N, K
    d.lda, d.ldw, d.ldc = lda, _ld(w), _ld(out)
    if bias is not None:
        _req(bias, F32, "bias")
        d.bias = _p(bias)
    if rowvec is not None:
        _req(rowvec, F32, "rowvec")
        d.rowvec, d.rows_per_vec, d.ldv = _p(rowvec), rows_per_vec, _ld(rowvec)
    d.flags = (GEGLU if geglu else 0) | (OUT_F32 if out_f32 else 0) | (GELU if gelu else 0)
    if res1 is not None:
        _req(res1, F32 if res1.dtype == F32 else P.ACT, "res1")
        d.res1, d.ldr1 = _p(res1), _ld(res1)
        d.flags |= RES1_F32 if res1.dtype == F32 else 0
    if res2 is not None:
        _req(res2, F32 if res2.dtype == F32 else P.ACT, "res2")
        d.res2, d.ldr2 = _p(res2), _ld(res2)
        d.flags |= RES2_F32 if res2.dtype == F32 else 0
    if master is not None:
        _req(master, F32, "master")
        if master.shape != (m_out, n_out) or geglu:
            raise ValueError("gemm: master must be f32 [M, N] (not available with GEGLU)")
        d.out_master, d.ldm = _p(master), _ld(master)
    d.alpha = alpha
    d.mode = mode
    if rowstats is not None:
        _req(rowstats, F32, "rowstats")
        if not rowstats.is_contiguous() or rowstats.numel() != M * (N // 32) * 2:
            raise ValueError("gemm: rowstats must be contiguous f32 [M, N/32, 2]")
        d.rowstats = _p(rowstats)
        d.flags |= ROWSTATS
    x2_now = P.SPLIT or planes
    use_nstream = False
    if tile == NSTREAM_TILE or (tile == 0 and _NSTREAM and w_frag is not None):
        use_nstream = (w_frag is not None and not x2_now and mode == PLAIN and a2 is None and split_k == 1 and K in (320, 640) and N % 32 == 0
                       and (tile == NSTREAM_TILE or nstream_supported(M, N, K))
                       and stats_pos is None and ln_pos is None and w_frag.dtype == P.ACT and w_frag.is_contiguous() and w_frag.numel() == N * K)
        if tile == NSTREAM_TILE and not use_nstream:
            raise ValueError("gemm: tile 70 needs w_frag (weights.pack_frag) and a PLAIN single-source product with K = 320 / 640, N % 32 == 0")
    if w_frag is not None and not use_nstream and ln is not None and geglu and ln[0].shape[-2] != 1 and ln_pos is None:
        ln = (ln_fold(ln[0]), ln[1], ln[2])
    if ln is not None:
        st, colsum, eps = ln
        _req(st, F32, "ln stats")
        _req(colsum, F32, "ln colsum")
        if not st.is_contiguous() or st.shape[-2:] not in ((K // 32, 2), (1, 2)) or colsum.numel() != N:
            raise ValueError("gemm: ln = (stats [rows, K/32, 2], colsum [N], eps)")
        d.ln_stats, d.ln_colsum, d.ln_nblk, d.ln_eps = _p(st), _p(colsum), st.shape[-2], float(eps)
        d.flags |= LNFUSE
    for name, arg in (("stats_pos", stats_pos), ("ln_pos", ln_pos)):
        if arg is None:
            continue
        tbl, hw_, fr_ = arg
        _req(tbl, F32, name)
        if P.SPLIT or not tbl.is_contiguous() or tbl.shape != (fr_, N) or hw_ <= 0 or (rowstats is None if name == "stats_pos" else ln is None):
            raise ValueError(f"gemm: {name} = (f32 [frames, N], hw, frames) goes with " + ("rowstats" if name == "stats_pos" else "ln") +
                             "; not in split precision")
        if name == "stats_pos":
            d.stats_pos = _p(tbl)
        else:
            d.ln_rowvec = _p(tbl)
        d.pos_hw, d.pos_frames = int(hw_), int(fr_)
    a_bytes = M * (K // (4 if d.ups == 2 else 9) if mode == CONV3 else K // 3 if mode == TMIX else K)
    if _XCD_MODE == "n" or (_XCD_MODE == "auto" and N * K > a_bytes):
        d.flags |= XCD_N
    d.batch = 1
    d.raster_g = _RASTER_G
    ws = None
    key_flags, key_master = None, int(master is not None)
    if planes:
        d.flags |= X2
        d.a_lo, d.a2_lo, d.w_lo = _rest_off(a, a_rest), (_rest_off(a2, a2_rest) if a2 is not None else 0), _rest_off(w, w_rest)
        if out_rest is not None:
            d.out_lo = _rest_off(out, out_rest)
            key_flags, key_master = d.flags | OUT_F32, 0
    elif out_rest is not None:
        key_flags = d.flags
        d.flags |= OUT_REST
        d.out_lo = _rest_off(out, out_rest)
    elif P.SPLIT:
        if master is not None:
            raise ValueError("gemm: split precision has no f32 master (the planes carry 16 bits)")
        d.flags |= X2
        d.a_lo, d.a2_lo, d.w_lo = _lo(a), _lo(a2), _lo(w)
        d.out_lo = 0 if out_f32 else _lo(out)
        d.res1_lo = _lo(res1) if (res1 is not None and res1.dtype != F32) else 0
        d.res2_lo = _lo(res2) if (res2 is not None and res2.dtype != F32) else 0

    if use_nstream:
        tile = NSTREAM_TILE
        d.W = _p(w_frag)
        d.flags |= W_FRAG

    def _set(t, sk):
        nonlocal ws
        d.tile, d.split_k = t, sk
        krot = _KROT and (t in ASM_TILES or not _KROT_ASM_ONLY) and 2 * N * K <= _KROT_MAX_W
        d.flags = (d.flags | KROT) if krot else (d.flags & ~KROT)
        if sk > 1:
            if ws is None or ws.numel() < sk * M * N:
                ws = torch.empty((sk * M * N,), dtype=F32, device=a.device)
            d.splitk_ws = _p(ws)

    if tile == 0:
        def _launch(t, sk):
            _set(t, sk)
            check(_lib.lib().avsd_gemm_bf16(C.byref(d), _stream()), "avsd_gemm_bf16")

        cands = X2_TILE_CANDIDATES if x2 else TILE_CANDIDATES
        nk = (K + 63) // 64
        two_src_unaligned = a2 is not None and (a.shape[1] % 64 != 0)
        if not geglu and not two_src_unaligned and ((M + 127) // 128) * ((N + 127) // 128) < 256 and nk >= 16:
            cands = cands + tuple(c for c in (X2_SPLITK_CANDIDATES if x2 else SPLITK_CANDIDATES) if nk // c[1] >= 4)
        splitk_ok = not geglu and not two_src_unaligned
        if mode == CONV3 and d.ups == 2:
            ok_tiles = SUBPIX_X2_TILES if x2 else SUBPIX_TILES
            cands = tuple(c for c in cands if c[0] in ok_tiles and (N // 4) % TILE_BN[c[0]] == 0)
        two_src_conv = mode == CONV3 and a2 is not None
        if two_src_conv:
            cands = conv3r_candidates(d.hs, d.ws, d.cin, M, N)
            if not cands:
                raise ValueError("gemm: no LDS-resident convolution tile takes this two-source geometry")
        elif (_CONV3R and mode == CONV3 and not x2 and d.stride == 1 and d.ups == 0 and d.pad == 1 and ln is None and out_rest is None):
            cands = cands + conv3r_candidates(d.hs, d.ws, d.cin, M, N)
        key = (mode, M, N, K, d.flags if key_flags is None else key_flags, d.stride, d.ups, d.pad, key_master)
        if mode == CONV3 and not x2:
            key = key + (d.hs, d.ws)
        if two_src_conv:
            key = key + ("a2", d.k_split)
        asm = ()
        if (_ASM_TILES and a2 is None and K % 64 == 0 and M * lda < (1 << 29) and N * _ld(w) < (1 << 29) and
                (mode == PLAIN or (mode == TMIX and d.cseg % 64 == 0 and ln is None))):
            asm = ASM_X2_CANDIDATES if x2 else tuple(c for c in ASM_CANDIDATES if mode == PLAIN or c[0] != 60)
            if splitk_ok and ((M + 127) // 128) * ((N + 127) // 128) < 256 and nk >= 8:
                asm = asm + tuple(c for c in (ASM_X2_SPLITK_CANDIDATES if x2 else ASM_SPLITK_CANDIDATES)
                                  if nk // c[1] >= 4 and (c[1] - 1) * -(-nk // c[1]) < nk)
        if RECORD_KEYS is not None:
            rec = RECORD_KEYS.setdefault(key, {"n": 0, "cands": tuple(dict.fromkeys(tuple(cands) + tuple(asm))), "flops": 2.0 * M * N * K})
            rec["n"] += 1
        picked = _pick_tile(key, _launch, cands, warm=(a, a2, res1, res2), challengers=asm)
        if picked is not None and picked[0] in ASM_TILES and not asm:
            picked = None
        if picked is not None and picked[0] in CONV3R_TILES and not ((_CONV3R or two_src_conv) and _lib.lib().avsd_gemm_conv3r_supported(picked[0], d.hs, d.ws, d.cin)):
            picked = None
        if picked is not None and picked[0] in CONV3R2D_TILES and not ((_CONV3R or two_src_conv) and _lib.lib().avsd_gemm_conv3r2d_supported(picked[0], d.hs, d.ws, d.cin)):
            picked = None
        if picked is not None and two_src_conv and picked not in cands:
            picked = None
        if picked is not None and out_rest is not None and not planes and (picked[0] in CONV3R_TILES or picked[0] in CONV3R2D_TILES):
            picked = None
        heur = _heuristic_tile_x2 if x2 else _heuristic_tile
        if picked is None and two_src_conv:
            picked = _heuristic_conv3r(cands, M, N)
        tile, split_k = picked if picked is not None else heur(M, N, K, geglu, splitk_ok)
        if mode == CONV3 and d.ups == 2:
            tile = _subpix_tile(tile, N // 4, x2)
    _set(tile, split_k)
    ev = _TIMER.start() if _TIMER is not None else None
    check(_lib.lib().avsd_gemm_bf16(C.byref(d), _stream()), "avsd_gemm_bf16")
    if ev is not None:
        fam = ("gemm_plain", "gemm_tmix", "gemm_conv3")[mode]
        dc = GemmDesc.from_buffer_copy(d)
        _TIMER.add_replay(fam, lambda dc=dc: check(_lib.lib().avsd_gemm_bf16(C.byref(dc), _stream()), "avsd_gemm_bf16"),
                          (a, a2, w, out, bias, rowvec, res1, res2, ws, rowstats, ln, master, stats_pos, ln_pos, a_rest, a2_rest, w_rest, w_frag, out_rest))
        subpix = mode == CONV3 and d.ups == 2
        _TIMER.stop(ev, fam, 2.0 * M * N * K * (3 if x2 else 1), 2.0 * M * K * (1.0 / (4 if subpix else 9) if mode == CONV3 else 1.0 / 3 if mode == TMIX else 1.0)
                    + 2.0 * N * K + _nbytes(out, res1, res2), flops_once=2.0 * M * N * K, flops_ref=2.0 * M * N * K * (2.25 if subpix else 1.0))
    return out


def gemm_f32(a: torch.Tensor, w: torch.Tensor, bias: Optional[torch.Tensor] = None) -> torch.Tensor:
    _req(a, F32, "a")
    _req(w, F32, "w")
    M, K = a.shape
    N = w.shape[0]
    out = torch.empty((M, N), dtype=F32, device=a.device)
    check(_lib.lib().avsd_gemm_f32(_p(a), _ld(a), _p(w), _ld(w), _p(bias), _p(out), _ld(out), M, N, K, _stream()), "avsd_gemm_f32")
    return out


def gemm_batched(a: torch.Tensor, w: torch.Tensor, *, alpha: float = 1.0, out_f32: bool = False,
                 bias: Optional[torch.Tensor] = None, tile: int = 0, ln: Optional[tuple] = None) -> torch.Tensor:
    _req(a, P.ACT, "a")
    _req(w, P.ACT, "w")
    B, M, K = a.shape
    N = w.shape[1]
    out = torch.empty((B, M, N), dtype=F32, device=a.device) if out_f32 else alloc16((B, M, N), a.device)
    d = GemmDesc()
    d.A, d.W, d.out = _p(a), _p(w), _p(out)
    d.M, d.N, d.K, d.k_split = M, N, K, K
    d.lda, d.ldw, d.ldc = a.stride(1), w.stride(1), out.stride(1)
    d.alpha, d.mode, d.flags, d.batch, d.tile = alpha, PLAIN, (OUT_F32 if out_f32 else 0), B, tile
    d.batch_stride_a, d.batch_stride_w, d.batch_stride_out = a.stride(0), w.stride(0), out.stride(0)
    if bias is not None:
        _req(bias, F32, "bias")
        d.bias = _p(bias)
    if ln is not None:
        st, colsum, eps = ln
        _req(st, F32, "ln stats")
        _req(colsum, F32, "ln colsum")
        d.ln_stats, d.ln_colsum, d.ln_nblk, d.ln_eps = _p(st), _p(colsum), K // 32, float(eps)
        d.flags |= LNFUSE
    if P.SPLIT:
        d.flags |= X2
        d.a_lo, d.w_lo, d.out_lo = _lo(a), _lo(w), (0 if out_f32 else _lo(out))
    if tile == 0:
        def _launch(t):
            d.tile = t
            check(_lib.lib().avsd_gemm_bf16(C.byref(d), _stream()), "avsd_gemm_bf16(batched)")

        picked = _pick_tile(("batched", B, M, N, K, d.flags), lambda t, sk: _launch(t), X2_TILE_CANDIDATES if P.SPLIT else TILE_CANDIDATES)
        d.tile = picked[0] if picked is not None else (_heuristic_tile_x2 if P.SPLIT else _heuristic_tile)(B * M, N, K, False, False)[0]
    dc = GemmDesc.from_buffer_copy(d) if _TIMER is not None else d
    _timed("gemm_plain", 2.0 * B * M * N * K * (3 if P.SPLIT else 1), 2.0 * B * (M * K + N * K) + _nbytes(out), (a, w, out, bias, ln),
           lambda: check(_lib.lib().avsd_gemm_bf16(C.byref(dc), _stream()), "avsd_gemm_bf16(batched)"))
    return out


def linear_small_m(x: torch.Tensor, w: torch.Tensor, bias: Optional[torch.Tensor], *, act_in: bool = False,
                   act_out: bool = False, out: Optional[torch.Tensor] = None) -> torch.Tensor:
    _req(x, F32, "x")
    _req(w, P.ACT, "w")
    M, K = x.shape
    N = w.shape[0]
    if not x.is_contiguous():
        raise ValueError("linear_small_m: x must be contiguous")
    if out is None:
        out = torch.empty((M, N), dtype=F32, device=x.device)
    if P.SPLIT:
        check(_lib.lib().avsd_linear_small_m_x2(_p(x), _p(w), _lo(w), _p(bias), _p(out), M, N, K, _ld(w), int(act_in), int(act_out),
                                                _stream()), "avsd_linear_small_m_x2")
        return out
    check(_lib.lib().avsd_linear_small_m(_p(x), _p(w), _p(bias), _p(out), M, N, K, _ld(w), int(act_in), int(act_out),
                                         _stream()), "avsd_linear_small_m")
    return out


_GN_FUSED = True

def groupnorm(x1: torch.Tensor, x2: Optional[torch.Tensor], nb: int, rows_per_batch: int, groups: int,
              gamma: torch.Tensor, beta: torch.Tensor, eps: float, act: bool,
              out: Optional[torch.Tensor] = None) -> torch.Tensor:
    _req(x1, P.ACT, "x1")
    c1 = x1.shape[1]
    c2 = 0
    if x2 is not None:
        _req(x2, P.ACT, "x2")
        c2 = x2.shape[1]
# ... 55 lines not shown
def ncfhw_to_rows_planes(x: torch.Tensor, cpad: int, rep: int = 1, scale: float = 1.0):
    _req(x, F32, "x")
    if not x.is_contiguous():
        raise ValueError("ncfhw_to_rows: x must be contiguous")
    B, Cc, Fr, H, W = x.shape
    out, rest = alloc_planes((rep * B * Fr * H * W, cpad), x.device)
    check(_lib.lib().avsd_ncfhw_to_rows_x2(_p(x), _p(out), _rest_off(out, rest), B, Cc, Fr, H * W, cpad, rep, float(scale), _stream()),
          "avsd_ncfhw_to_rows_x2")
    return out, rest


def ln_fold(stats: torch.Tensor) -> torch.Tensor:
    _req(stats, F32, "stats")
    M, nblk = stats.shape[0], stats.shape[1]
    out = torch.empty((M, 1, 2), dtype=F32, device=stats.device)
    _timed("ln_fold", 0.0, _nbytes(stats, out), (stats, out), lambda: check(_lib.lib().avsd_ln_fold(_p(stats), M, nblk, _p(out), _stream()), "avsd_ln_fold"))
    return out


def layernorm(x: torch.Tensor, gamma: torch.Tensor, beta: torch.Tensor, eps: float = 1e-5,
              pos: Optional[torch.Tensor] = None, hw: int = 1, frames: int = 1,
              out: Optional[torch.Tensor] = None) -> torch.Tensor:
    _req(x, P.ACT, "x")
    _req(gamma, F32, "gamma")
    _req(beta, F32, "beta")
    M, Cc = x.shape
    if pos is not None:
        _req(pos, F32, "pos")
        if not pos.is_contiguous() or pos.shape != (frames, Cc):
            raise ValueError("layernorm: pos must be contiguous [frames, C]")
    if out is None:
        out = alloc16((M, Cc), x.device)
    if P.SPLIT:
        a_ = (_p(x), _ld(x), _lo(x), _p(out), _ld(out), _lo(out), M, Cc, _p(gamma), _p(beta), float(eps), _p(pos), hw, frames)
        call = lambda: check(_lib.lib().avsd_layernorm_x2(*a_, _stream()), "avsd_layernorm_x2")
    else:
        a_ = (_p(x), _ld(x), _p(out), _ld(out), M, Cc, _p(gamma), _p(beta), float(eps), _p(pos), hw, frames)
        call = lambda: check(_lib.lib().avsd_layernorm(*a_, _stream()), "avsd_layernorm")
    _timed("layernorm", 0.0, _nbytes(x, out), (x, out, gamma, beta, pos), call)
    return out


def softmax_rows(s: torch.Tensor) -> torch.Tensor:
    _req(s, F32, "s")
    rows, L = s.shape
    out = alloc16((rows, L), s.device)
    check(_lib.lib().avsd_softmax_rows_x2(_p(s), _ld(s), _p(out), _ld(out), _lo(out), rows, L, _stream()), "avsd_softmax_rows_x2")
    return out


def attention(q: torch.Tensor, k: torch.Tensor, v: torch.Tensor, *, bq: int, lq: int, lk: int, kv_rows: int,
              heads: int, q_per_kv: int, frames: int, key_index: Optional[torch.Tensor] = None,
              scale: Optional[float] = None, out: Optional[torch.Tensor] = None, fp8: Optional[tuple] = None) -> torch.Tensor:
    _req(q, P.ACT, "q")
    _req(k, P.ACT, "k")
    _req(v, P.ACT, "v")
    Cc = q.shape[1]
    d = Cc // heads
    if key_index is not None:
        if key_index.dtype != torch.int32 or not key_index.is_contiguous() or key_index.shape != (frames, lk):
            raise ValueError("attention: key_index must be contiguous int32 [frames, lk]")
    if out is None:
        out = alloc16((bq * lq, Cc), q.device)
    if scale is None:
        scale = float(d) ** -0.5
    if P.SPLIT:
        if fp8 is not None:
            raise ValueError("attention: fp8 Q/K/V and split precision are exclusive")
        a_ = (_p(q), _ld(q), _lo(q), _p(k), _ld(k), _lo(k), _p(v), _ld(v), _lo(v), _p(out), _ld(out), _lo(out), bq, lq, lk, kv_rows, heads, d,
              q_per_kv, _p(key_index), frames, float(scale))
        call = lambda: check(_lib.lib().avsd_attention_x2(*a_, _stream()), "avsd_attention_x2")
    elif fp8 is not None:
        qs, ks, vs = (float(x) for x in fp8)
        a_ = (_p(q), _ld(q), _p(k), _ld(k), _p(v), _ld(v), _p(out), _ld(out), bq, lq, lk, kv_rows, heads, d, q_per_kv, _p(key_index), frames,
              float(scale), qs, ks, vs)
        call = lambda: check(_lib.lib().avsd_attention_fp8(*a_, _stream()), "avsd_attention_fp8")
    else:
        a_ = (_p(q), _ld(q), _p(k), _ld(k), _p(v), _ld(v), _p(out), _ld(out), bq, lq, lk, kv_rows, heads, d, q_per_kv, _p(key_index), frames,
              float(scale))
        call = lambda: check(_lib.lib().avsd_attention(*a_, _stream()), "avsd_attention")
    _timed("attention", 4.0 * bq * heads * lq * lk * d * (3 if P.SPLIT else 1), _nbytes(q, out) + 4.0 * (bq // q_per_kv) * lk * Cc,
           (q, k, v, out, key_index), call)
    return out


def cross_attention_block_supported(C: int, heads: int, lk_pad: int, M: int, L: int) -> bool:
    return not P.SPLIT and bool(_lib.lib().avsd_cross_attention_block_supported(C, heads, lk_pad)) and M % 128 == 0 and L % 128 == 0


def cross_attention_block(h: torch.Tensor, stats: torch.Tensor, wq: torch.Tensor, q_colsum: torch.Tensor, q_bias: torch.Tensor,
                          k: torch.Tensor, vt: torch.Tensor, lk: int, wo: torch.Tensor, o_bias: torch.Tensor, *, res: torch.Tensor,
                          heads: int, L: int, q_per_kv: int, eps: float = 1e-5, scale: Optional[float] = None,
                          rowstats: Optional[torch.Tensor] = None, master: Optional[torch.Tensor] = None,
                          out: Optional[torch.Tensor] = None, stats_pos: Optional[tuple] = None) -> torch.Tensor:
    if P.SPLIT:
        raise ValueError("cross_attention_block: not built for split precision (use the separate kernels)")
    _req(h, P.ACT, "h")
    _req(wq, P.ACT, "wq")
    _req(wo, P.ACT, "wo")
    _req(k, P.ACT, "k")
    _req(vt, P.ACT, "vt")
    _req(stats, F32, "stats")
    M, Cc = h.shape
    lk_pad = k.shape[1]
    if not k.is_contiguous() or not vt.is_contiguous() or vt.shape != (k.shape[0], Cc, lk_pad) or k.shape[2] != Cc:
        raise ValueError("cross_attention_block: k must be contiguous [nkv, lk_pad, C] and vt [nkv, C, lk_pad]")
    if not stats.is_contiguous() or stats.shape != (M, Cc // 32, 2):
        raise ValueError("cross_attention_block: stats must be contiguous f32 [M, C/32, 2]")
    if (M // L) // q_per_kv > k.shape[0] or (M // L) % q_per_kv:
        raise ValueError("cross_attention_block: K/V blocks do not cover the query batches")
    if out is None:
        out = torch.empty((M, Cc), dtype=P.ACT, device=h.device)
    d = XAttnDesc()
    d.h, d.ldh = _p(h), _ld(h)
    _req(res, F32 if res.dtype == F32 else P.ACT, "res")
    d.res, d.ldres, d.res_f32 = _p(res), _ld(res), int(res.dtype == F32)
    d.M, d.C, d.heads, d.L = M, Cc, heads, L
    d.ln_stats, d.ln_eps = _p(stats), float(eps)
    d.scale = float(scale) if scale is not None else float(Cc // heads) ** -0.5
    d.wq, d.ldwq, d.q_colsum, d.q_bias = _p(wq), _ld(wq), _p(q_colsum), _p(q_bias)
    d.k, d.vt, d.lk, d.lk_pad, d.q_per_kv = _p(k), _p(vt), lk, lk_pad, q_per_kv
    d.wo, d.ldwo, d.o_bias = _p(wo), _ld(wo), _p(o_bias)
    d.out, d.ldo = _p(out), _ld(out)
    if master is not None:
        _req(master, F32, "master")
        d.out_master, d.ldm = _p(master), _ld(master)
    if rowstats is not None:
        _req(rowstats, F32, "rowstats")
        d.rowstats = _p(rowstats)
    if stats_pos is not None:
        tbl, hw_, fr_ = stats_pos
        _req(tbl, F32, "stats_pos")
        if rowstats is None or not tbl.is_contiguous() or tbl.shape != (fr_, Cc) or hw_ <= 0:
            raise ValueError("cross_attention_block: stats_pos = (f32 [frames, C], hw, frames) goes with rowstats")
        d.stats_pos, d.pos_hw, d.pos_frames = _p(tbl), int(hw_), int(fr_)
    ev = _TIMER.start() if _TIMER is not None else None
    check(_lib.lib().avsd_cross_attention_block(C.byref(d), _stream()), "avsd_cross_attention_block")
    if ev is not None:
        dc = XAttnDesc.from_buffer_copy(d)
        _TIMER.add_replay("cross_attention_block", lambda dc=dc: check(_lib.lib().avsd_cross_attention_block(C.byref(dc), _stream()),
                                                                         "avsd_cross_attention_block"),
                          (h, stats, wq, q_colsum, q_bias, k, vt, wo, o_bias, res, out, master, rowstats, stats_pos))
        _TIMER.stop(ev, "cross_attention_block", 4.0 * M * Cc * Cc + 4.0 * M * lk * Cc, _nbytes(h, out, res, master) + 4.0 * Cc * Cc)
    return out


def temporal_attention(qkv: torch.Tensor, *, b: int, frames: int, hw: int, heads: int,
                       scale: Optional[float] = None, out: Optional[torch.Tensor] = None) -> torch.Tensor:
    _req(qkv, P.ACT, "qkv")
    Cc = qkv.shape[1] // 3
    d = Cc // heads
    if out is None:
        out = alloc16((qkv.shape[0], Cc), qkv.device)
    if scale is None:
        scale = float(d) ** -0.5
    if P.SPLIT:
        a_ = (_p(qkv), _ld(qkv), _lo(qkv), _p(out), _ld(out), _lo(out), b, frames, hw, heads, d, float(scale))
        call = lambda: check(_lib.lib().avsd_temporal_attention_x2(*a_, _stream()), "avsd_temporal_attention_x2")
    else:
        a_ = (_p(qkv), _ld(qkv), _p(out), _ld(out), b, frames, hw, heads, d, float(scale))
        call = lambda: check(_lib.lib().avsd_temporal_attention(*a_, _stream()), "avsd_temporal_attention")
    _timed("temporal_attention", 4.0 * b * hw * heads * frames * frames * d, _nbytes(qkv, out), (qkv, out), call)
    return out


def ncfhw_to_rows(x: torch.Tensor, cpad: int, rep: int = 1, scale: float = 1.0) -> torch.Tensor:
# ... 495 lines not shown
```

### asva_amd/unet.py

```python
from __future__ import annotations

import inspect
import json
import math
import os
from typing import Any, Dict, Optional, Tuple, Union

import torch
from torch import nn

from . import precision as P

from . import ops
from .conditioning import mask_to_key_index
from .weights import Blob, _Pk, _Ref, from_act, pack_conv1x1, pack_device, pack_frag, pack_geglu, pack_linear, subpixel_ups, to_act, to_planes

CONFIG_NAME = "config.json"
SAFETENSORS_NAME = "diffusion_pytorch_model.safetensors"
BIN_NAME = "diffusion_pytorch_model.bin"

DOWN_TYPES = ("FFSpatioAudioTempCrossAttnDownBlock3D", "FFSpatioTempCrossAttnDownBlock3D", "FFSpatioTempResDownBlock3D")
UP_TYPES = ("FFSpatioAudioTempCrossAttnUpBlock3D", "FFSpatioTempCrossAttnUpBlock3D", "FFSpatioTempResUpBlock3D")
MID_TYPES = ("FFSpatioAudioTempCrossAttnUNetMidBlock3D", "FFSpatioTempCrossAttnUNetMidBlock3D")


_FUSE_LN = True
_FUSE_LN_TEMP = True
_F32_RES = os.environ.get("AVSD_F32_RESIDUAL", "0") != "0"
_ATTN_FP8 = os.environ.get("AVSD_ATTN_FP8", "0") != "0"
_FUSE_XATTN = True
_LN_PREFOLD = True
_SHARE_PREFIX = True
_F32_CONV_Y = True


def _replicate(a: "_Act", r: int) -> "_Act":
    return _Act(ops.copy(a.lo, rep=r), None if a.hi is None else ops.copy(a.hi, rep=r),
                None if a.rest is None else ops.copy(a.rest, rep=r))


def _xa_fill(kv: torch.Tensor, n_kv: int, rows: int, C: int, idx: Optional[torch.Tensor], old=None):
    nb, lk = (n_kv, rows) if idx is None else (n_kv * idx.shape[0], idx.shape[1])
    lkp = (lk + 31) // 32 * 32
    if lkp > 96 or P.SPLIT:
        return None
    if old is None:
        old = _Pk(k=torch.empty((nb, lkp, C), dtype=kv.dtype, device=kv.device),
                  vt=torch.empty((nb, C, lkp), dtype=kv.dtype, device=kv.device), lk=lk)
    ops.xattn_pack_kv(kv, n_kv, rows, C, idx, old.k, old.vt)
    return old


_FRAME_INDEX: dict = {}
_KEY_INDEX: dict = {}


def key_index_for(mask: torch.Tensor, device) -> torch.Tensor:
    key = (tuple(mask.shape), mask.numpy().tobytes(), str(device))
    if key not in _KEY_INDEX:
        if len(_KEY_INDEX) > 64:
            _KEY_INDEX.clear()
        _KEY_INDEX[key] = mask_to_key_index(mask).to(device)
    return _KEY_INDEX[key]



def frame_index(frames: int, device) -> torch.Tensor:
    key = (frames, str(device))
    if key not in _FRAME_INDEX:
        _FRAME_INDEX[key] = torch.arange(frames, dtype=torch.float32, device=device)
    return _FRAME_INDEX[key]


class FrozenConfig(dict):

    def __getattr__(self, k):
        try:
            return self[k]
        except KeyError as e:
            raise AttributeError(k) from e

    def __setattr__(self, k, v):
        raise AttributeError("config is read-only")


class UNet3DConditionOutput:

    def __init__(self, sample: torch.Tensor):
        self.sample = sample

    def __getitem__(self, i):
        return (self.sample,)[i]


class _Affine(nn.Module):

    def __init__(self, c: int):
        super().__init__()
        self.weight = nn.Parameter(torch.ones(c))
        self.bias = nn.Parameter(torch.zeros(c))


class _Linear(nn.Module):
    def __init__(self, cin: int, cout: int, bias: bool = True, zero: bool = False):
        super().__init__()
        w = torch.zeros(cout, cin)
        if not zero:
            nn.init.kaiming_uniform_(w, a=math.sqrt(5))
        self.weight = nn.Parameter(w)
        if bias:
# ... 504 lines not shown
        self._packed = None
        self._cond = None
        self._cond_key = None
        self._cond_refs = None

    @property
    def attn_processors(self) -> Dict[str, Any]:
        return {f"{n}.processor": "avsd_hip" for n, m in self.named_modules() if isinstance(m, _Attention)}

    def set_attn_processor(self, processor):
        if isinstance(processor, dict) and len(processor) != len(self.attn_processors):
            raise ValueError(f"expected {len(self.attn_processors)} processors, got {len(processor)}")

    def set_default_attn_processor(self):
        pass

    def set_attention_slice(self, slice_size):
        pass

    def pack(self, device: Optional[torch.device] = None):
        device = pack_device(device)
        if self._packed is not None and self._packed.key == P.pack_key() and (device is None or self._packed.blob.device == device):
            return self._packed
        device = pack_device(device, self.device, ops, "AudioUNet3DConditionModel.pack")
        pr = Packer()
        pk = _Pk(conv_in=pr.ffconv(self.conv_in, "conv_in"), t1=pr.lin(self.time_embedding.linear_1), t2=pr.lin(self.time_embedding.linear_2),
                 down=[pr.block(b, f"down_blocks.{i}") for i, b in enumerate(self.down_blocks)], mid=pr.block(self.mid_block, "mid_block"),
                 up=[pr.block(b, f"up_blocks.{i}") for i, b in enumerate(self.up_blocks)],
                 norm_out=pr.aff(self.conv_norm_out), conv_out=pr.ffconv(self.conv_out, "conv_out"))
        self._packed = pr.finish(pk, device, meta=next(self.parameters()).is_meta)
        return self._packed

    @torch.no_grad()
    def set_conditioning(self, encoder_hidden_states: torch.Tensor, audio_encoder_hidden_states: Optional[torch.Tensor],
                         audio_attention_mask: Optional[torch.Tensor], video_length: int):
        pk = self.pack()
        dev = pk.blob.device
        Fr = video_length
        self._cond_key = None
        self._cond_refs = None

        def rows(x):
            if x is None:
                return None, 1
            per_frame = 1
            if x.dim() == 4:
                if x.stride(1) == 0 or x.shape[1] == 1:
                    x = x[:, 0]
                else:
                    per_frame = x.shape[1]
                    x = x.reshape(x.shape[0] * x.shape[1], *x.shape[2:])
            return ops.to_act(x.to(device=dev)), per_frame

        text, text_pf = rows(encoder_hidden_states)
        audio, audio_pf = rows(audio_encoder_hidden_states)
        key_index, idx_frames = None, Fr
        if audio_attention_mask is not None:
            m = audio_attention_mask.detach().to("cpu", torch.bool)
            if m.dim() == 3:
                if bool((m == m[:1]).all()):
                    m = m[0]
                else:
                    m = m.reshape(-1, m.shape[-1])
            if not bool(m.all()):
                key_index = key_index_for(m, dev)
                idx_frames = m.shape[0]
        sig = (tuple(text.shape), text_pf, None if audio is None else tuple(audio.shape), audio_pf,
               None if key_index is None else tuple(key_index.shape), idx_frames, Fr, P.NAME, P.SPLIT, id(pk))
        nb = text.shape[0] // text_pf
        share = {r: bool(nb % r == 0 and all(torch.equal(text[: text.shape[0] // r], c) for c in text.chunk(r)[1:])) for r in (2, 3)}
        old = self._cond
        if old is not None and getattr(old, "sig", None) == sig:
            tb = text.reshape(-1, text.shape[-1])
            ab = None if audio is None else audio.reshape(-1, audio.shape[-1])
            if key_index is not None and key_index is not old.key_index:
                old.key_index.copy_(key_index)
            old.share = share
            for tp, c in zip(self._transformers(pk), old.blocks):
                ops.gemm(tb, tp.attn2.wkv, out=c.text_kv)
                if tp.audio:
                    ops.gemm(ab, tp.attn_audio.wkv, out=c.audio_kv)
                self._xa_caches(c, tp, old.key_index, idx_frames, Fr)
            return old
        blocks = [self.make_cond_block(tp, text, text_pf, audio, audio_pf, Fr, key_index, idx_frames) for tp in self._transformers(pk)]
        self._cond_version = getattr(self, "_cond_version", 0) + 1
        self._cond = _Pk(blocks=blocks, key_index=key_index, idx_frames=idx_frames, frames=Fr,
                         batch=text.shape[0] // text_pf, sig=sig, version=self._cond_version, share=share)
        return self._cond

    @staticmethod
    def _xa_caches(c, tp, key_index, idx_frames, frames):
        C = tp.dim
        c.xa_text = c.xa_audio = None
        if not _FUSE_XATTN:
            return
        if c.text_pf == 1:
            c.xa_text = _xa_fill(c.text_kv, c.text_kv.shape[0] // c.text_len, c.text_len, C, None, getattr(c, "_xa_text", None))
            if c.xa_text is not None:
                c.xa_text.q_per_kv = frames
        if tp.audio and c.audio_pf == 1 and key_index is not None and idx_frames == frames:
            c.xa_audio = _xa_fill(c.audio_kv, c.audio_kv.shape[0] // c.audio_len, c.audio_len, C, key_index, getattr(c, "_xa_audio", None))
            if c.xa_audio is not None:
                c.xa_audio.q_per_kv = 1
        c._xa_text, c._xa_audio = c.xa_text, c.xa_audio

    @staticmethod
    def make_cond_block(tp, text, text_pf, audio, audio_pf, frames, key_index=None, idx_frames=None):
        C = tp.dim
        c = _Pk()
        c.text_kv = ops.gemm(text.reshape(-1, text.shape[-1]), tp.attn2.wkv)
        c.text_len, c.text_pf = text.shape[1], text_pf
        if tp.audio:
            if audio is None:
                raise ValueError("audio_encoder_hidden_states is required by the audio cross-attention blocks")
            c.audio_kv = ops.gemm(audio.reshape(-1, audio.shape[-1]), tp.attn_audio.wkv)
            c.audio_len, c.audio_pf = audio.shape[1], audio_pf
        ar = frame_index(frames, text.device)
        emb = ops.timestep_embedding(ar, C)
        hid = ops.linear_small_m(emb, tp.pos1.w, tp.pos1.b, act_out=True)
        c.pos = ops.linear_small_m(hid, tp.pos2.w, tp.pos2.b)
        c.posw = None if P.SPLIT else ops.linear_small_m(c.pos, tp.attn_temp.wqkv_ln, None)
        AudioUNet3DConditionModel._xa_caches(c, tp, key_index, idx_frames if idx_frames is not None else frames, frames)
        return c

    @staticmethod
    def _transformers(pk):
        for b in list(pk.down) + [pk.mid] + list(pk.up):
            if b.attentions:
                yield from b.attentions

    @torch.no_grad()
    def forward(
        self,
        sample: torch.Tensor,
        timestep: Union[torch.Tensor, float, int],
        encoder_hidden_states: Optional[torch.Tensor] = None,
        audio_encoder_hidden_states: Optional[torch.Tensor] = None,
        class_labels=None,
        timestep_cond=None,
        attention_mask=None,
        audio_attention_mask: Optional[torch.Tensor] = None,
        cross_attention_kwargs=None,
        down_block_additional_residuals=None,
        mid_block_additional_residual=None,
        return_dict: bool = True,
    ):
        for name, v in (("class_labels", class_labels), ("timestep_cond", timestep_cond), ("attention_mask", attention_mask),
                        ("cross_attention_kwargs", cross_attention_kwargs),
                        ("down_block_additional_residuals", down_block_additional_residuals),
                        ("mid_block_additional_residual", mid_block_additional_residual)):
            if v is not None:
                raise NotImplementedError(f"{name} is not on the AVSyncD inference path")
        assert sample.ndim == 5, sample.size()
        pk = self.pack()
        B, Cin, Fr, H, W = sample.shape
        nblk = len(self.config.block_out_channels)
        if H % (1 << (nblk - 1)) or W % (1 << (nblk - 1)):
            raise NotImplementedError("latent H, W must be multiples of 2**(num_blocks-1)")
        if encoder_hidden_states is not None:
            key = tuple((t.data_ptr(), tuple(t.shape), t._version) if t is not None else None
                        for t in (encoder_hidden_states, audio_encoder_hidden_states, audio_attention_mask)) + (Fr,)
            if self._cond is None or self._cond_key != key:
                self._cond_key = None
                self.set_conditioning(encoder_hidden_states, audio_encoder_hidden_states, audio_attention_mask, Fr)
                self._cond_key = key
                self._cond_refs = (encoder_hidden_states, audio_encoder_hidden_states, audio_attention_mask)
        if self._cond is None:
            raise RuntimeError("no conditioning: pass encoder_hidden_states or call set_conditioning first")
        dev = pk.blob.device
        in_dtype = sample.dtype
        x32 = sample.to(device=dev, dtype=torch.float32).contiguous()
        if torch.is_tensor(timestep):
            t = timestep.to(device=dev, dtype=torch.float32).reshape(-1)
        else:
            t = torch.full((1,), float(timestep), dtype=torch.float32, device=dev)
        out = self.denoise_forward(x32, t, rep=1)
        if in_dtype != torch.float32:
            out = out.to(in_dtype)
        if not return_dict:
            return (out,)
        return UNet3DConditionOutput(sample=out)

    @torch.no_grad()
    def denoise_forward(self, x32: torch.Tensor, t: torch.Tensor, rep: int = 1) -> torch.Tensor:
        pk = self.pack()
        cond = self._cond
        if cond is None:
            raise RuntimeError("no conditioning: call set_conditioning first")
        b, Cin, Fr, H, W = x32.shape
        B = rep * b
        nblk = len(self.config.block_out_channels)
        if cond.frames != Fr or cond.batch != B:
            raise ValueError(f"conditioning was prepared for batch {cond.batch} x {cond.frames} frames, sample has {B} x {Fr}")
        if t.numel() not in (1, B):
            raise ValueError("timestep must be a scalar or have one entry per batch element")
        ch0 = self.config.block_out_channels[0]
        e = ops.timestep_embedding(t, ch0)
        e = ops.linear_small_m(e, pk.t1.w, pk.t1.b, act_out=True)
        e = ops.linear_small_m(e, pk.t2.w, pk.t2.b)
        temb = ops.linear_small_m(e, pk.temb_w, pk.temb_b, act_in=True)
        st = _Pk(B=B, F=Fr, temb=temb, temb_rows=(Fr if (t.numel() == B and B > 1) else B * Fr), cond=cond, tr_i=0,
                 groups=self.config.norm_num_groups, eps=float(self.config.norm_eps),
                 heads=_per_block(self.config.attention_head_dim, nblk), fuse_ln=getattr(self, "fuse_layernorm", _FUSE_LN),
                 f32_stream=(getattr(self, "f32_residual", _F32_RES) or P.PLAN is not None) and not P.SPLIT,
                 fp8=(tuple(getattr(self, "fp8_scales", (1.0, 1.0, 1.0))) if getattr(self, "fp8_attention", _ATTN_FP8) else None))

# ... 120 lines not shown
    B, Fr = st.B, st.F
    L = hw[0] * hw[1]
    C = p.dim
    c = st.cond.blocks[st.tr_i]
    st.tr_i += 1
    n = ops.groupnorm(x.lo, None, B * Fr, L, st.groups, p.norm.g, p.norm.b, 1e-6, False)
    fused = C % 32 == 0 and st.fuse_ln
    eps = 1e-5
    M = B * Fr * L
    stats = [torch.empty((M, C // 32, 2), dtype=torch.float32, device=n.device) for _ in range(2)] if fused else None
    si = 0

    def stream(a, w, bias, res, want_stats=True, stats_pos=None, rest=False):
        nonlocal si
        m = _master(st, a, w.shape[0])
        if fused and want_stats:
            si ^= 1
            return _Act(ops.gemm(a, w, bias=bias, res1=None if res is None else res.res, rowstats=stats[si], master=m, stats_pos=stats_pos), m)
        o16 = o16r = None
        if rest and m is not None:
            o16, o16r = ops.alloc_planes((a.shape[0], w.shape[0]), a.device)
        return _Act(ops.gemm(a, w, bias=bias, res1=None if res is None else res.res, master=m, out=o16, out_rest=o16r), m, o16r)

    def cross(h, a, norm, xa, want_stats, unfused, stats_pos=None):
        nonlocal si
        if fused and st.fp8 is None and xa is not None and ops.cross_attention_block_supported(C, heads, xa.k.shape[1], M, L):
            m = _master(st, h.lo, C)
            s_in = stats[si]
            s_out = None
            if want_stats:
                si ^= 1
                s_out = stats[si]
            out = ops.cross_attention_block(h.lo, s_in, a.wq_ln, a.sq_ln, a.bq_ln, xa.k, xa.vt, xa.lk, a.wo, a.bo, res=h.res,
                                            heads=heads, L=L, q_per_kv=xa.q_per_kv, eps=eps, rowstats=s_out, master=m, stats_pos=stats_pos)
            return _Act(out, m)
        return stream(unfused(), a.wo, a.bo, h, want_stats=want_stats, stats_pos=stats_pos)

    def proj(h, norm, wl, bl, sl, w_plain):
        if fused:
            return ops.gemm(h.lo, wl, bias=bl, ln=(stats[si], sl, eps))
        return ops.gemm(ops.layernorm(h.lo, norm.g, norm.b), w_plain)

    h = stream(n, p.proj_in.w, p.proj_in.b, None)
    a1 = p.attn1
    if fused:
        kv = ops.gemm_batched(h.lo.view(B, Fr * L, C)[:, :L], a1.wkv_ln.unsqueeze(0).expand(B, 2 * C, C), bias=a1.bkv_ln,
                              ln=(stats[si], a1.skv_ln, eps)).view(B * L, 2 * C)
        q = ops.gemm(h.lo, a1.wq_ln, bias=a1.bq_ln, ln=(stats[si], a1.sq_ln, eps))
    else:
        n1 = ops.layernorm(h.lo, p.norm1.g, p.norm1.b)
        q = ops.gemm(n1, a1.wq)
        kv = ops.gemm_batched(n1.view(B, Fr * L, C)[:, :L], a1.wkv.unsqueeze(0).expand(B, 2 * C, C)).view(B * L, 2 * C)
    o = ops.attention(q, kv[:, :C], kv[:, C:], bq=B * Fr, lq=L, lk=L, kv_rows=L, heads=heads, q_per_kv=Fr, frames=Fr, fp8=st.fp8)
    h = stream(o, a1.wo, a1.bo, h)
    if split > 1:
        h, x = _replicate(h, split), _replicate(x, split)
        st.B = B = B * split
        M = B * Fr * L
        if fused:
            cur = stats[si]
            stats = [torch.empty((M, C // 32, 2), dtype=torch.float32, device=n.device) for _ in range(2)]
            ops.copy(cur, stats[si], rep=split)
    if p.audio:
        aa = p.attn_audio

        def audio_attention():
            q = proj(h, p.norm_audio, getattr(aa, "wq_ln", None), getattr(aa, "bq_ln", None), getattr(aa, "sq_ln", None), aa.wq)
            idx = st.cond.key_index
            return ops.attention(q, c.audio_kv[:, :C], c.audio_kv[:, C:], bq=B * Fr, lq=L,
                                 lk=idx.shape[1] if idx is not None else c.audio_len, kv_rows=c.audio_len, heads=heads,
                                 q_per_kv=Fr if c.audio_pf == 1 else 1, frames=st.cond.idx_frames if idx is not None else Fr,
                                 key_index=idx, fp8=st.fp8)

        h = cross(h, aa, p.norm_audio, getattr(c, "xa_audio", None), True, audio_attention)
    a2 = p.attn2

    def text_attention():
        q = proj(h, p.norm2, getattr(a2, "wq_ln", None), getattr(a2, "bq_ln", None), getattr(a2, "sq_ln", None), a2.wq)
        return ops.attention(q, c.text_kv[:, :C], c.text_kv[:, C:], bq=B * Fr, lq=L, lk=c.text_len, kv_rows=c.text_len,
                             heads=heads, q_per_kv=Fr if c.text_pf == 1 else 1, frames=Fr, fp8=st.fp8)

    fold_temp = fused and _FUSE_LN_TEMP and not P.SPLIT and getattr(c, "posw", None) is not None and hasattr(p.attn_temp, "wqkv_ln")
    h = cross(h, a2, p.norm2, getattr(c, "xa_text", None), fold_temp, text_attention, stats_pos=(c.pos, L, Fr) if fold_temp else None)
    if fold_temp:
        qkv = ops.gemm(h.lo, p.attn_temp.wqkv_ln, bias=p.attn_temp.bqkv_ln, ln=(stats[si], p.attn_temp.sqkv_ln, eps), ln_pos=(c.posw, L, Fr))
    else:
        nt = ops.layernorm(h.lo, p.norm_temp.g, p.norm_temp.b, pos=c.pos, hw=L, frames=Fr)
        qkv = ops.gemm(nt, p.attn_temp.wqkv)
    o = ops.temporal_attention(qkv, b=B, frames=Fr, hw=L, heads=heads)
    h = stream(o, p.attn_temp.wo, p.attn_temp.bo, h)
    if fused:
        wf = getattr(p, "w1_ln_f", None)
        if wf is not None and ops._NSTREAM and not P.SPLIT and ops.nstream_supported(M, 8 * C, C):
            g = ops.gemm(h.lo, p.w1_ln, bias=p.b1_ln, geglu=True, ln=(stats[si], p.s1_ln, eps), w_frag=wf)
        else:
            g = ops.gemm(h.lo, p.w1_ln, bias=p.b1_ln, geglu=True, ln=(ops.ln_fold(stats[si]) if _LN_PREFOLD else stats[si], p.s1_ln, eps))
    else:
        g = ops.gemm(ops.layernorm(h.lo, p.norm3.g, p.norm3.b), p.w1, bias=p.b1, geglu=True)
    h = stream(g, p.ff2.w, p.ff2.b, h, want_stats=False)
    return stream(h.lo, p.proj_out.w, p.proj_out.b, x, want_stats=False, rest=rest)


AudioUNet3DConditionModel._ffconv = staticmethod(_ffconv)
AudioUNet3DConditionModel._resblock = staticmethod(_resblock)
AudioUNet3DConditionModel._transformer = staticmethod(_transformer)
```

### asva_amd/weights.py

```python
from __future__ import annotations

import torch

from . import precision as P


def to_act(w: torch.Tensor) -> torch.Tensor:
    w = w.detach().float().contiguous()
    if not P.SPLIT or w.device.type == "meta":
        return w.to(P.ACT)
    n = w.numel()
    npad = (n + 7) // 8 * 8
    base = torch.zeros((2, npad), dtype=P.ACT, device=w.device)
    main = w.reshape(-1).to(P.ACT)
    base[0, :n] = main
    base[1, :n] = (w.reshape(-1) - main.float()).to(P.ACT)
    return base[0, :n].view(w.shape)


def to_planes(w: torch.Tensor):
    w = w.detach().float().contiguous()
    main = w.to(P.ACT)
    if w.device.type == "meta":
        return main, torch.empty_like(main)
    return main, (w - main.float()).to(P.ACT)


def is_twin(t: torch.Tensor) -> bool:
    nb = t.untyped_storage().nbytes()
    if t.numel() == 0 or nb % 32:
        return False
    last = sum((s - 1) * st for s, st in zip(t.shape, t.stride()))
    return (t.storage_offset() + last + 1) * t.element_size() <= nb // 2


def rest_of(t: torch.Tensor) -> torch.Tensor:
    half = t.untyped_storage().nbytes() // 2 // t.element_size()
    return torch.as_strided(t, t.shape, t.stride(), t.storage_offset() + half)


def from_act(t: torch.Tensor) -> torch.Tensor:
    if P.SPLIT and is_twin(t):
        return t.float() + rest_of(t).float()
    return t.float()


def pack_linear(w: torch.Tensor) -> torch.Tensor:
    return to_act(w)


def pack_conv1x1(w: torch.Tensor) -> torch.Tensor:
    return to_act(w.detach().reshape(w.shape[0], w.shape[1]))


def pack_conv3x3(w: torch.Tensor, cin_pad: int | None = None, cout_pad: int | None = None) -> torch.Tensor:
    cout, cin, kh, kw = w.shape
    assert kh == 3 and kw == 3
    cin_pad = cin_pad or (cin + 7) // 8 * 8
    cout_pad = cout_pad or (cout + 3) // 4 * 4
    p = torch.zeros((cout_pad, 3, 3, cin_pad), dtype=torch.float32, device=w.device)
    p[:cout, :, :, :cin] = w.detach().float().permute(0, 2, 3, 1)
    return to_act(p.reshape(cout_pad, 9 * cin_pad))


def subpixel_conv3x3(wf: torch.Tensor) -> torch.Tensor:
    cout, kh, kw, cin = wf.shape
    assert kh == 3 and kw == 3
    sets = (((0,), (1, 2)), ((0, 1), (2,)))
    out = torch.zeros((2, 2, cout, 2, 2, cin), dtype=torch.float32, device=wf.device)
    for dy in range(2):
        for dx in range(2):
            for i in range(2):
                for j in range(2):
                    for ky in sets[dy][i]:
                        for kx in sets[dx][j]:
                            out[dy, dx, :, i, j, :] += wf[:, ky, kx, :]
    return out.reshape(4 * cout, 4 * cin)


def subpixel_ups(wf: torch.Tensor, b: torch.Tensor):
    return subpixel_conv3x3(wf), b.repeat(4)


def geglu_row_order(nh: int) -> torch.Tensor:
    assert nh % 16 == 0, "GEGLU packing needs the inner dim to be a multiple of 16"
    blk = torch.arange(nh // 16).repeat_interleave(32)
    p = torch.arange(32).repeat(nh // 16)
    return torch.where(p < 16, blk * 16 + p, nh + blk * 16 + p - 16)


def pack_geglu(w: torch.Tensor, b: torch.Tensor | None):
    nh = w.shape[0] // 2
    order = geglu_row_order(nh).to(w.device)
    wp = to_act(w.detach()[order])
    bp = None if b is None else b.detach()[order].float().contiguous()
    return wp, bp


def pack_frag(wp: torch.Tensor) -> torch.Tensor:
    N, K = wp.shape
    assert N % 32 == 0 and K % 16 == 0
    return wp.reshape(N // 32, 32, K // 16, 2, 8).permute(0, 2, 3, 1, 4).contiguous().reshape(N // 32, K // 16, 64, 8)


def pad_rows(w: torch.Tensor, mult: int = 4) -> torch.Tensor:
    n = w.shape[0]
    if n % mult == 0:
        return w
    pad = torch.zeros((mult - n % mult,) + tuple(w.shape[1:]), dtype=w.dtype, device=w.device)
    return torch.cat([w, pad], 0).contiguous()


class _Pk:

    def __init__(self, **kw):
        self.__dict__.update(kw)


class _Ref:

    def __init__(self, idx: int):
        self.idx = idx


class Blob:

    def __init__(self):
        self.items = []

    def reg(self, t: torch.Tensor) -> _Ref:
        self.items.append(t.contiguous())
        return _Ref(len(self.items) - 1)

    def finish(self, root: _Pk, device, meta: bool = False) -> _Pk:
        offs, total = [], 0
        for t in self.items:
            offs.append(total)
            total += (t.numel() * t.element_size() + 255) // 256 * 256
        blob = torch.zeros(total * (2 if P.SPLIT else 1), dtype=torch.uint8, device=device)
        views = []
        for t, o in zip(self.items, offs):
            nb = t.numel() * t.element_size()
            if not meta:
                blob[o:o + nb].copy_(t.reshape(-1).view(torch.uint8))
                if P.SPLIT and t.dtype == P.ACT:
                    if not is_twin(t):
                        raise RuntimeError("split-precision packing: a 16-bit item was not produced by weights.to_act")
                    blob[total + o:total + o + nb].copy_(rest_of(t).reshape(-1).view(torch.uint8))
            views.append(blob[o:o + nb].view(t.dtype).view(t.shape))

        def resolve(obj):
            if isinstance(obj, _Pk):
                for k, v in list(obj.__dict__.items()):
                    if isinstance(v, _Ref):
                        obj.__dict__[k] = views[v.idx]
                    else:
                        resolve(v)
            elif isinstance(obj, list):
                for v in obj:
                    resolve(v)

        resolve(root)
        root.blob = blob
        root.key = P.pack_key()
        root.split = P.SPLIT
        return root


def pack_device(device, own=None, ops=None, who="pack"):
    if device is not None:
        device = torch.device(device)
        if device.type == "cuda" and device.index is None:
            device = torch.device("cuda", torch.cuda.current_device())
    if own is None:
        return device
    device = own if device is None else device
    if device.type == "meta":
        raise RuntimeError(f"{who}: pass the target device explicitly for a meta-initialised model")
    if device.type != "cuda" and not getattr(ops, "EMULATED", False):
        raise RuntimeError(f"{who}: the MI355X path needs a cuda (HIP) device; move the model with .to('cuda') first — "
                           "there is no CPU compute path")
    return device
```

### include/avsd.h

```cpp
#ifndef AVSD_H
#define AVSD_H

#include <stddef.h>
#include <stdint.h>

#ifdef __cplusplus
extern "C" {
#endif

#define AVSD_OK 0
#define AVSD_EINVAL (-1)
#define AVSD_ELAUNCH (-2)
#define AVSD_ENODEV (-3)

#define AVSD_ABI_VERSION 10

int avsd_abi_version(void);
const char* avsd_precision(void);
const char* avsd_last_error(void);
int avsd_device_info(char* name_host, int len, int* num_cu_host);

enum { AVSD_GEMM_PLAIN = 0, AVSD_GEMM_TMIX = 1, AVSD_GEMM_CONV3 = 2 };
enum { AVSD_GEMM_GEGLU = 1, AVSD_GEMM_OUT_F32 = 2, AVSD_GEMM_GELU = 4, AVSD_GEMM_XCD_N = 8, AVSD_GEMM_ROWSTATS = 16,
       AVSD_GEMM_LNFUSE = 32, AVSD_GEMM_RES1_F32 = 64, AVSD_GEMM_RES2_F32 = 128, AVSD_GEMM_X2 = 256, AVSD_GEMM_KROT = 512, AVSD_GEMM_W_FRAG = 1024,
       AVSD_GEMM_OUT_REST = 2048 };
#define AVSD_GEMM_MAX_TILE 33
#define AVSD_GEMM_MAX_TILE_X2 36
#define AVSD_GEMM_TILE_256x160_8W 38
#define AVSD_GEMM_TILE_ASM_FIRST 60
#define AVSD_GEMM_TILE_ASM_LAST 67
#define AVSD_GEMM_TILE_NSTREAM 70
#define AVSD_GEMM_TILE_CONV3R_FIRST 40
#define AVSD_GEMM_TILE_CONV3R_LAST 49
#define AVSD_GEMM_TILE_CONV3R2D_FIRST 51
#define AVSD_GEMM_TILE_CONV3R2D_LAST 54
typedef struct avsd_gemm_desc {
  const void* A;
  const void* A2;
  const void* W;
  void* out;
  const float* bias;
  const float* rowvec;
  const void* res1;
  const void* res2;
  int32_t M, N, K;
  int32_t lda, lda2, k_split, ldw, ldc, ldr1, ldr2;
  int32_t rows_per_vec, ldv;
  float alpha;
  int32_t mode, flags;
  int32_t batch;
  int64_t batch_stride_a, batch_stride_w, batch_stride_out;
  int32_t hw, frames, cseg;
  int32_t hs, ws, ho, wo, cin, stride, ups;
  int32_t pad;
  int32_t tile;
  int32_t split_k;
  float* splitk_ws;
  float* rowstats;
  const float* ln_stats;
  const float* ln_colsum;
  int32_t ln_nblk;
  float ln_eps;
  float* out_master;
  int32_t ldm;
  int32_t raster_g;
  int64_t a_lo, a2_lo, w_lo, out_lo, res1_lo, res2_lo;
  const float* stats_pos;
  const float* ln_rowvec;
  int32_t pos_hw, pos_frames;
} avsd_gemm_desc;

int avsd_gemm_bf16(const avsd_gemm_desc* desc_host, void* stream);
int avsd_gemm_conv3r_supported(int tile, int hs, int ws, int cin);
int avsd_gemm_conv3r2d_supported(int tile, int hs, int ws, int cin);
int avsd_sizeof_gemm_desc(void);

typedef struct avsd_xattn_desc {
  const void* h;        int32_t ldh;
  int32_t res_f32;
  const void* res;      int32_t ldres;
  int32_t M, C, heads, L;
  const float* ln_stats; float ln_eps;
  float scale;
  const void* wq;       int32_t ldwq;  int32_t lk;
  const float* q_colsum;
  const float* q_bias;
  const void* k;        const void* vt;
  int32_t lk_pad, q_per_kv;
  const void* wo;       int32_t ldwo;  int32_t ldo;
  const float* o_bias;
  void* out;
  float* out_master;    int32_t ldm;   int32_t reserved0;
  float* rowstats;
  const float* stats_pos;
  int32_t pos_hw, pos_frames;
} avsd_xattn_desc;
int avsd_cross_attention_block_supported(int C, int heads, int lk_pad);
int avsd_cross_attention_block(const avsd_xattn_desc* desc_host, void* stream);
int avsd_sizeof_xattn_desc(void);

int avsd_linear_small_m(const float* x, const void* W_bf16, const float* bias, float* out,
                        int M, int N, int K, int ldw, int act_in, int act_out, void* stream);

int avsd_groupnorm_stats(const void* x1, int ld1, int c1, const void* x2, int ld2, int c2,
                         int nb, int rows_per_batch, int groups, float* scratch, int nchunks, void* stream);
int avsd_groupnorm_apply(const void* x1, int ld1, int c1, const void* x2, int ld2, int c2,
                         int nb, int rows_per_batch, int groups, const float* gamma, const float* beta, float eps,
                         const float* scratch, int nchunks, int act, void* y, int ldy, void* stream);
int avsd_groupnorm_fused_supported(int nb, int rows_per_batch, int groups, int c1, int c2, int split);
int avsd_groupnorm_fused(const void* x1, int ld1, int c1, const void* x2, int ld2, int c2, int nb, int rows_per_batch,
                         int groups, const float* gamma, const float* beta, float eps, int act, void* y, int ldy, void* stream);
int avsd_groupnorm_nchunks(int nb, int rows_per_batch, int channels);
int avsd_groupnorm_scratch_floats(int nb, int nchunks, int groups, int channels);

int avsd_ln_fold(const float* stats, int M, int nblk, float* out, void* stream);
int avsd_layernorm(const void* x, int ldx, void* y, int ldy, int M, int C,
                   const float* gamma, const float* beta, float eps,
                   const float* pos, int hw, int frames, void* stream);

int avsd_softmax_rows(const float* S, int lds, void* P, int ldp, int rows, int L, void* stream);

int avsd_attention(const void* Q, int ldq, const void* K, int ldk, const void* V, int ldv,
                   void* O, int ldo, int Bq, int Lq, int Lk, int kv_rows, int heads, int d,
                   int q_per_kv, const int32_t* key_index, int frames, float scale, void* stream);

int avsd_attention_fp8(const void* Q, int ldq, const void* K, int ldk, const void* V, int ldv, void* O, int ldo,
                       int Bq, int Lq, int Lk, int kv_rows, int heads, int d, int q_per_kv,
                       const int32_t* key_index, int frames, float scale, float q_scale, float k_scale,
                       float v_scale, void* stream);

int avsd_temporal_attention(const void* QKV, int ldqkv, void* O, int ldo, int B, int frames,
                            int hw, int heads, int d, float scale, void* stream);

int avsd_ncfhw_to_rows(const float* src, void* dst, int B, int C, int F, int HW, int cpad,
                       int rep, float scale, void* stream);
int avsd_rows_to_ncfhw(const float* src, int ld, float* dst, int B, int C, int F, int HW,
                       void* stream);
int avsd_timestep_embedding(const float* t, float* out, int n, int dim, void* stream);

int avsd_guided_step(const float* noise_pred, int n_branch, float g, float g2, float* eps_hist,
                     int store_slot, float w_cur, const int32_t* hist_idx_host,
                     const float* w_host, int n_hist, const float* x_in, float* x_out, float ca,
                     float cb, int B, int C, int F, int HW, void* stream);

int avsd_guided_multistep(const float* noise_pred, int n_branch, float g, float g2, float* hist, int store_slot,
                          const int32_t* hist_idx_host, const float* w_host, int n_hist, const float* x_in,
                          float* x_out, float ca, float c_cur, float s_x, float s_e, int B, int C, int F,
                          int HW, void* stream);

int avsd_vae_postprocess(const void* src, int ld, float* dst, int N, int HW, void* stream);
int avsd_vae_postprocess_u8(const void* src, int ld, void* dst_u8, int N, int HW, void* stream);

// ... 104 lines not shown
```

Baseline: 85.62 steps/s.

## Fuse temporal self-attention into the LN-folded QKV GEMM epilogue

Adds an EPI_TATTN epilogue to the gemm2 kernel that computes temporal self-attention directly from the QKV tile held in LDS. Row tiles are remapped so each tile holds whole frame sequences for a set of pixels, and QKV weights are repacked head-major and padded to 128/256 columns per head. This removes the QKV activation round trip to memory and the separate temporal attention launch, at the cost of padded GEMM columns (120 of 128 used) and extra epilogue work. It is enabled by default only for head_dim 40 blocks.

```diff
diff --git a/asva_amd/_lib.py b/asva_amd/_lib.py
--- a/asva_amd/_lib.py
+++ b/asva_amd/_lib.py
@@ -36,6 +36,7 @@
         ("a_lo", C.c_int64), ("a2_lo", C.c_int64), ("w_lo", C.c_int64), ("out_lo", C.c_int64), ("res1_lo", C.c_int64),
         ("res2_lo", C.c_int64),
         ("stats_pos", c_void_p), ("ln_rowvec", c_void_p), ("pos_hw", C.c_int32), ("pos_frames", C.c_int32),
+        ("heads", C.c_int32), ("head_dim", C.c_int32), ("attn_scale", C.c_float),
     ]
 
 
diff --git a/asva_amd/build.py b/asva_amd/build.py
--- a/asva_amd/build.py
+++ b/asva_amd/build.py
@@ -11,7 +11,7 @@
 LIB = os.path.join(HERE, "libavsd_hip.so")
 VARIANTS = {"bf16": ("", LIB, []), "fp16": ("_f16", os.path.join(HERE, "libavsd_hip_f16.so"), ["-DAVSD_F16=1"])}
 SOURCES = ["lib.hip", "attention.hip", "attention_x2.hip", "gemm_f32.hip", "gemm4.hip", "nstream.hip", "conv3r.hip", "norm.hip", "groupnorm_fused.hip", "elementwise.hip", "audio.hip", "xattn.hip", "attention_fp8.hip", "avsync.hip", "clip_text.hip", "imagebind_eval.hip", "plan.hip"]
-GEMM_UNITS = 7
+GEMM_UNITS = 8
 HEADERS = [os.path.join(CSRC, "avsd_common.h"), os.path.join(CSRC, "gemm_common.h"), os.path.join(CSRC, "gemm4_loops.inc"),
            os.path.join(HERE, "..", "include", "avsd.h")]
 FLAGS = ["--offload-arch=gfx950", "-O3", "-std=c++17", "-fPIC", "-Wall", "-Wno-unused-function"]
diff --git a/asva_amd/csrc/gemm.hip b/asva_amd/csrc/gemm.hip
--- a/asva_amd/csrc/gemm.hip
+++ b/asva_amd/csrc/gemm.hip
@@ -262,6 +262,130 @@
   return w > 3 ? 3 : w;
 }
 constexpr int MODE_SUBPIX = 3;
+
+template <int BM>
+__host__ __device__ __forceinline__ int tattn_row_tiles(const avsd_gemm_desc& p) {
+  const int ppt = BM / p.frames;
+  return (p.M / (p.frames * p.hw)) * ((p.hw + ppt - 1) / ppt);
+}
+template <int D, int F, int SS>
+__device__ __forceinline__ void tattn_query(const h16_t* sT, int pl, int i, int s, float scale, float (&o)[20]) {
+  constexpr int DS = D / 20;
+  const h16_t* base = sT + pl * F * SS + s * 20;
+  uint2 q[5];
+#pragma unroll
+  for (int d = 0; d < 5; ++d) q[d] = *reinterpret_cast<const uint2*>(base + i * SS + 4 * d);
+  float sc[F];
+  float mx = -1e30f;
+#pragma unroll
+  for (int j = 0; j < F; ++j) {
+    const h16_t* kr = base + j * SS + D;
+    float d0 = 0.f, d1 = 0.f;
+#pragma unroll
+    for (int d = 0; d < 5; ++d) {
+      const uint2 kv = *reinterpret_cast<const uint2*>(kr + 4 * d);
+      d0 = dot2h(q[d].x, kv.x, d0);
+      d1 = dot2h(q[d].y, kv.y, d1);
+    }
+    float dot = d0 + d1;
+#pragma unroll
+    for (int x = DS / 2; x > 0; x >>= 1) dot += __shfl_xor(dot, x, 64);
+    dot *= scale;
+    mx = fmaxf(mx, dot);
+    sc[j] = dot;
+    __builtin_amdgcn_sched_barrier(0);
+  }
+  float sum = 0.f;
+#pragma unroll
+  for (int j = 0; j < F; ++j) {
+    sc[j] = __expf(sc[j] - mx);
+    sum += sc[j];
+  }
+  const float inv = 1.0f / sum;
+#pragma unroll
+  for (int e = 0; e < 20; ++e) o[e] = 0.f;
+#pragma unroll
+  for (int j = 0; j < F; ++j) {
+    const h16_t* vr = base + j * SS + 2 * D;
+#pragma unroll
+    for (int d = 0; d < 5; ++d) {
+      const uint2 vv = *reinterpret_cast<const uint2*>(vr + 4 * d);
+      o[4 * d] = fmaf(sc[j], lo2f(vv.x), o[4 * d]);
+      o[4 * d + 1] = fmaf(sc[j], hi2f(vv.x), o[4 * d + 1]);
+      o[4 * d + 2] = fmaf(sc[j], lo2f(vv.y), o[4 * d + 2]);
+      o[4 * d + 3] = fmaf(sc[j], hi2f(vv.y), o[4 * d + 3]);
+    }
+    __builtin_amdgcn_sched_barrier(0);
+  }
+#pragma unroll
+  for (int e = 0; e < 20; ++e) o[e] *= inv;
+}
+template <int BN>
+__host__ __device__ constexpr int tattn_table_bytes(int frames) { return (2 + frames) * BN * 4; }
+template <int BN>
+__device__ __forceinline__ void tattn_fill_table(const avsd_gemm_desc& p, float* tab, int head, int tid, int nthreads) {
+  const int nvec = (2 + p.frames) * (BN / 4);
+  for (int v = tid; v < nvec; v += nthreads) {
+    const int row = v / (BN / 4), c = (v - row * (BN / 4)) * 4;
+    const float* src = row == 0 ? p.ln_colsum : row == 1 ? p.bias : (p.ln_rowvec ? p.ln_rowvec + (int64_t)(row - 2) * p.N : nullptr);
+    *reinterpret_cast<float4*>(tab + row * BN + c) = src ? *reinterpret_cast<const float4*>(src + head * BN + c) : make_float4(0.f, 0.f, 0.f, 0.f);
+  }
+}
+template <int BM, int BN, int WM, int WN, int FN, int FM>
+__device__ __forceinline__ void tattn_epilogue(const avsd_gemm_desc& p, f32x16 (&acc)[FN][FM], unsigned char* smem, const float* tab, int wm, int wn, int lane,
+                                               int tid, int head, int br, int pix0, const float (&pre_ln)[2 * FM]) {
+  constexpr int D = (BN / 128) * 40;
+  constexpr int SS = BN + 8;
+  constexpr int DS = D / 20;
+  static_assert(BN == 128 || BN == 256, "one head per column tile: 3 x 40 of 128 or 3 x 80 of 256 columns");
+  static_assert(BM * DS <= 64 * WM * WN, "one thread per (tile row, 20-channel slice)");
+  h16_t* sT = reinterpret_cast<h16_t*>(smem);
+  const int F = p.frames;
+  const int ppt = BM / F;
+  __syncthreads();
+  const int hsel = (lane >> 5) * 4;
+#pragma unroll
+  for (int b = 0; b < FM; ++b) {
+    const int r = wm * (BM / WM) + b * 32 + (lane & 31);
+    const int pl = r / F, f = r - pl * F;
+    if (pl >= ppt || pix0 + pl >= p.hw) continue;
+    const float ln_rstd = pre_ln[2 * b], ln_mr = pre_ln[2 * b + 1];
+    const float* lrv = tab + (2 + f) * BN;
+#pragma unroll
+    for (int a = 0; a < FN; ++a)
+#pragma unroll
+      for (int q = 0; q < 4; ++q) {
+        const int c = wn * (BN / WN) + a * 32 + 8 * q + hsel;
+        float v[4];
+#pragma unroll
+        for (int i = 0; i < 4; ++i) v[i] = p.alpha * acc[a][b][4 * q + i];
+        const float4 cs = *reinterpret_cast<const float4*>(tab + c);
+        const float4 pv = *reinterpret_cast<const float4*>(lrv + c);
+        const float4 bb = *reinterpret_cast<const float4*>(tab + BN + c);
+        v[0] += pv.x; v[1] += pv.y; v[2] += pv.z; v[3] += pv.w;
+        v[0] = fmaf(v[0], ln_rstd, -ln_mr * cs.x); v[1] = fmaf(v[1], ln_rstd, -ln_mr * cs.y);
+        v[2] = fmaf(v[2], ln_rstd, -ln_mr * cs.z); v[3] = fmaf(v[3], ln_rstd, -ln_mr * cs.w);
+        v[0] += bb.x; v[1] += bb.y; v[2] += bb.z; v[3] += bb.w;
+        *reinterpret_cast<uint2*>(sT + r * SS + c) = make_uint2(pack2h(v[0], v[1]), pack2h(v[2], v[3]));
+      }
+  }
+  __syncthreads();
+  const int qi = tid / DS, s = tid - qi * DS;
+  const int pl_raw = qi / F;
+  const bool active = pl_raw < ppt && pix0 + pl_raw < p.hw;
+  const int pl = active ? pl_raw : 0;
+  const int i = active ? qi - pl_raw * F : 0;
+  float o[20];
+  if (F == 12) tattn_query<D, 12, SS>(sT, pl, i, s, p.attn_scale, o);
+  else tattn_query<D, 24, SS>(sT, pl, i, s, p.attn_scale, o);
+  if (!active) return;
+  const int64_t m = (int64_t)(br * F + i) * p.hw + pix0 + pl;
+  h16_t* op = reinterpret_cast<h16_t*>(p.out) + m * p.ldc + head * D + s * 20;
+#pragma unroll
+  for (int d = 0; d < 5; ++d)
+    *reinterpret_cast<uint2*>(op + 4 * d) = make_uint2(pack2h(o[4 * d], o[4 * d + 1]), pack2h(o[4 * d + 2], o[4 * d + 3]));
+}
+
 template <int BM, int BN, int WM, int WN, int STAGES, int MODE, int LW = 0, bool X2 = false, int EX = EPI_PLAIN>
 __global__ __launch_bounds__(64 * (WM * WN + LW), gemm2_min_waves(BM, BN, STAGES, X2, WM * WN + LW)) void gemm2_kernel(const avsd_gemm_desc p) {
   extern __shared__ __attribute__((aligned(1024))) unsigned char smem2[];
@@ -287,7 +411,8 @@
   const int wm = wave_all % WM;
   const int wn = (wave_all / WM) % WN;
 
-  const int ntm = (p.M + BM - 1) / BM;
+  constexpr bool TATTN = EX == EPI_TATTN;
+  const int ntm = TATTN ? tattn_row_tiles<BM>(p) : (p.M + BM - 1) / BM;
   const int ntn = (p.N + BN - 1) / BN;
   const int nwg = ntm * ntn;
   const int nsplit = p.split_k > 1 ? p.split_k : 1;
@@ -304,6 +429,14 @@
   int tm, tn;
   tile_of_item(wg, ntm, ntn, (p.flags & AVSD_GEMM_XCD_N) != 0, p.raster_g, tm, tn);
   const int64_t bz = blockIdx.z;
+  const int ta_ppt = TATTN ? BM / p.frames : 1;
+  const int ta_tpb = TATTN ? (p.hw + ta_ppt - 1) / ta_ppt : 1;
+  const int ta_br = TATTN ? tm / ta_tpb : 0;
+  const int ta_pix0 = TATTN ? (tm - ta_br * ta_tpb) * ta_ppt : 0;
+  [[maybe_unused]] auto ta_row = [&](int r) -> int {
+    const int pl = r / p.frames, f = r - pl * p.frames;
+    return (pl < ta_ppt && ta_pix0 + pl < p.hw) ? (ta_br * p.frames + f) * p.hw + ta_pix0 + pl : -1;
+  };
   const int nk_all = (p.K + BK - 1) / BK;
   const int per_split = (nk_all + nsplit - 1) / nsplit;
   const int kt0 = ksplit * per_split;
@@ -325,7 +458,13 @@
   for (int j = 0; j < PA; ++j) {
     const int L = (wave + j * NWAVES) * 4 + (lane >> 4);
     const int x = (lane & 15) ^ (L & 15);
-    const RowInfo32 r = make_row32<MODE>(p, tm * BM + 2 * L + (x >> 3));
+    RowInfo32 r;
+    if constexpr (TATTN) {
+      const int m = ta_row(2 * L + (x >> 3));
+      r.valid = m >= 0;
+      r.o0 = r.valid ? m * p.lda : 0;
+      r.o1 = r.o2 = r.hb = r.wb = 0;
+    } else r = make_row32<MODE>(p, tm * BM + 2 * L + (x >> 3));
     ro0[j] = r.o0; ro1[j] = r.o1; ro2[j] = r.o2; rhb[j] = r.hb; rwb[j] = r.wb; rvalid[j] = r.valid;
     kca[j] = (x & 7) * 8;
   }
@@ -488,11 +627,16 @@
   if (pre) {
 #pragma unroll
     for (int b = 0; b < FM; ++b) {
-      const int m = tm * BM + wm * (BM / WM) + b * 32 + (lane & 31);
+      int m = tm * BM + wm * (BM / WM) + b * 32 + (lane & 31);
+      if constexpr (TATTN) {
+        m = ta_row(wm * (BM / WM) + b * 32 + (lane & 31));
+        if (m < 0) m = p.M;
+      }
       pre_ln[2 * b] = 1.f; pre_ln[2 * b + 1] = 0.f;
       if (m < p.M) ln_row_stats(p, m, bz, pre_ln[2 * b], pre_ln[2 * b + 1]);
     }
   }
+  if constexpr (TATTN) tattn_fill_table<BN>(p, reinterpret_cast<float*>(smem2 + STAGES * STAGE_BYTES), tn, tid, 64 * NC);
   if (LW > 0 && is_loader) {
     for (int kt = 0; kt < nk; ++kt) {
       wait_stage(kt);
@@ -589,6 +733,10 @@
       }
     }
   }
+  if constexpr (TATTN) {
+    static_assert(LW == 0 && !X2 && MODE == AVSD_GEMM_PLAIN && BM * (BN + 8) * 2 <= STAGES * STAGE_BYTES, "EPI_TATTN: PLAIN tiles whose ring holds the staged tile");
+    tattn_epilogue<BM, BN, WM, WN>(p, acc, smem2, reinterpret_cast<const float*>(smem2 + STAGES * STAGE_BYTES), wm, wn, lane, tid, tn, ta_br, ta_pix0, pre_ln);
+  } else
   if constexpr (subpix) {
     if constexpr (X2) epilogue_x2<FN, FM, true>(p, acc, tm * BM + wm * (BM / WM), tn * BN + wn * (BN / WN), lane, bz, pre_ln, pre);
     else epilogue_each<FN, FM, (64 * (WM * WN + LW) > 512), EPI_SHUF>(p, acc, tm * BM + wm * (BM / WM), tn * BN + wn * (BN / WN), lane, bz, pre_ln, pre);
@@ -767,6 +915,27 @@
     }
     AVSD_CHECK_LAUNCH("gemm split-K reduce launch");
   }
+  return AVSD_OK;
+}
+
+template <int BM, int BN, int WM, int WN, int STAGES>
+int launch2_tattn(const avsd_gemm_desc& d, hipStream_t s) {
+  constexpr size_t lds = (size_t)STAGES * (BM + BN) * 128 + tattn_table_bytes<BN>(24);
+  static_assert(lds <= 160 * 1024, "tile does not fit the 160 KB of LDS");
+  static bool attr_set = false;
+  if (!attr_set) {
+    hipError_t e = hipFuncSetAttribute(reinterpret_cast<const void*>(&gemm2_kernel<BM, BN, WM, WN, STAGES, AVSD_GEMM_PLAIN, 0, false, EPI_TATTN>),
+                                       hipFuncAttributeMaxDynamicSharedMemorySize, (int)lds);
+    if (e != hipSuccess) {
+      avsd_set_error("gemm2 (temporal attention epilogue): hipFuncSetAttribute(%zu B LDS): %s", lds, hipGetErrorString(e));
+      return AVSD_ELAUNCH;
+    }
+    attr_set = true;
+  }
+  dim3 grid((unsigned)(tattn_row_tiles<BM>(d) * (d.N / BN)), 1, 1);
+  const size_t lds_now = (size_t)STAGES * (BM + BN) * 128 + tattn_table_bytes<BN>(d.frames);
+  hipLaunchKernelGGL((gemm2_kernel<BM, BN, WM, WN, STAGES, AVSD_GEMM_PLAIN, 0, false, EPI_TATTN>), grid, dim3(64 * WM * WN), lds_now, s, d);
+  AVSD_CHECK_LAUNCH("gemm2 (temporal attention epilogue) launch");
   return AVSD_OK;
 }
 
@@ -894,6 +1063,14 @@
 }
 #endif
 
+int avsd_gemm_dispatch_tattn(const avsd_gemm_desc& d, hipStream_t s);
+#if !defined(AVSD_GEMM_TU) || AVSD_GEMM_TU == 7
+int avsd_gemm_dispatch_tattn(const avsd_gemm_desc& d, hipStream_t s) {
+  if (d.head_dim == 40) return launch2_tattn<128, 128, 2, 2, 2>(d, s);
+  return launch2_tattn<128, 256, 2, 4, 2>(d, s);
+}
+#endif
+
 int avsd_gemm_dispatch_x2_plain(const avsd_gemm_desc& d, int tile, hipStream_t s);
 int avsd_gemm_dispatch_x2_tmix(const avsd_gemm_desc& d, int tile, hipStream_t s);
 int avsd_gemm_dispatch_x2_conv3(const avsd_gemm_desc& d, int tile, hipStream_t s);
@@ -1006,6 +1183,21 @@
   } else {
     AVSD_REQUIRE(false, "gemm: unknown mode %d", d.mode);
   }
+  if (d.flags & AVSD_GEMM_TATTN) {
+    AVSD_REQUIRE(d.mode == AVSD_GEMM_PLAIN && (d.flags & AVSD_GEMM_LNFUSE) && !d.A2 && d.batch == 1 && d.split_k <= 1 &&
+                     !(d.flags & (AVSD_GEMM_X2 | AVSD_GEMM_GEGLU | AVSD_GEMM_GELU | AVSD_GEMM_OUT_F32 | AVSD_GEMM_ROWSTATS | AVSD_GEMM_OUT_REST | AVSD_GEMM_W_FRAG)) &&
+                     !d.res1 && !d.res2 && !d.rowvec && !d.out_master,
+                 "gemm/tattn: a single-source PLAIN product with AVSD_GEMM_LNFUSE and a 16-bit single-plane output; bias only, no split_k / batch / AVSD_GEMM_X2");
+    AVSD_REQUIRE((d.head_dim == 40 || d.head_dim == 80) && (d.frames == 12 || d.frames == 24) && d.heads > 0 && d.hw > 0 && d.attn_scale > 0.f,
+                 "gemm/tattn: head_dim 40 / 80 and frames 12 / 24 are built (got head_dim %d, frames %d, heads %d, hw %d)", d.head_dim, d.frames, d.heads, d.hw);
+    const int bn = d.head_dim == 40 ? 128 : 256;
+    AVSD_REQUIRE(d.N == d.heads * bn && d.M % (d.frames * d.hw) == 0 && d.ldc >= d.heads * d.head_dim,
+                 "gemm/tattn: N (%d) must be heads * %d (head-major padded q|k|v), M (%d) whole branches of frames * hw rows, ldc (%d) >= heads * head_dim", d.N, bn, d.M, d.ldc);
+    AVSD_REQUIRE(!d.ln_rowvec || (d.pos_hw == d.hw && d.pos_frames == d.frames), "gemm/tattn: ln_rowvec needs pos_hw == hw and pos_frames == frames");
+    AVSD_REQUIRE((double)d.M * d.lda * 2.0 < 2147483648.0 && (double)d.N * d.ldw * 2.0 < 2147483648.0, "gemm/tattn: operands must be < 2 GiB");
+    AVSD_REQUIRE(d.tile == 0 || d.tile == (d.head_dim == 40 ? 11 : 31), "gemm/tattn: head_dim %d runs on the form of tile %d (or tile 0), got %d", d.head_dim, d.head_dim == 40 ? 11 : 31, d.tile);
+    return avsd_gemm_dispatch_tattn(d, reinterpret_cast<hipStream_t>(stream));
+  }
   if ((d.tile >= AVSD_GEMM_TILE_CONV3R_FIRST && d.tile <= AVSD_GEMM_TILE_CONV3R_LAST) ||
       (d.tile >= AVSD_GEMM_TILE_CONV3R2D_FIRST && d.tile <= AVSD_GEMM_TILE_CONV3R2D_LAST)) {
     if (d.split_k > 1) AVSD_REQUIRE(d.splitk_ws != nullptr, "gemm: split_k needs a workspace");
diff --git a/asva_amd/csrc/gemm_common.h b/asva_amd/csrc/gemm_common.h
--- a/asva_amd/csrc/gemm_common.h
+++ b/asva_amd/csrc/gemm_common.h
@@ -64,7 +64,7 @@
   }
 }
 
-constexpr int EPI_PLAIN = 0, EPI_REST = 1, EPI_SHUF = 2;
+constexpr int EPI_PLAIN = 0, EPI_REST = 1, EPI_SHUF = 2, EPI_TATTN = 3;
 __device__ __forceinline__ unsigned rest2h(float v0, float v1, unsigned mainw) { return pack2h(v0 - lo2f(mainw), v1 - hi2f(mainw)); }
 __device__ __forceinline__ int64_t shuf_row(const avsd_gemm_desc& p, int m) { return 4 * (int64_t)m - 2 * (m % p.ws); }
 __device__ __forceinline__ void shuf_col(const avsd_gemm_desc& p, int n, int& radd, int& col) {
diff --git a/asva_amd/ops.py b/asva_amd/ops.py
--- a/asva_amd/ops.py
+++ b/asva_amd/ops.py
@@ -11,7 +11,7 @@
 from ._lib import GemmDesc, XAttnDesc, check
 
 PLAIN, TMIX, CONV3 = 0, 1, 2
-GEGLU, OUT_F32, GELU, XCD_N, ROWSTATS, LNFUSE, RES1_F32, RES2_F32, X2, KROT, W_FRAG, OUT_REST = 1, 2, 4, 8, 16, 32, 64, 128, 256, 512, 1024, 2048
+GEGLU, OUT_F32, GELU, XCD_N, ROWSTATS, LNFUSE, RES1_F32, RES2_F32, X2, KROT, W_FRAG, OUT_REST, TATTN = 1, 2, 4, 8, 16, 32, 64, 128, 256, 512, 1024, 2048, 4096
 _XCD_MODE = "auto"
 F32 = torch.float32
 
@@ -109,6 +109,8 @@
 _SUBPIX_BY_BN = ({320: 17, 160: 38, 128: 11, 64: 24}, {160: 34, 128: 11, 64: 24})
 ASM_X2_CANDIDATES = ((63, 1), (64, 1), (65, 1), (66, 1))
 ASM_X2_SPLITK_CANDIDATES = ((63, 2), (63, 4), (64, 2), (64, 4), (65, 2), (65, 4), (66, 2), (66, 4), (66, 8))
+TATTN_HEAD_DIMS = {128: 40, 256: 80}
+TATTN_TILE = {40: 11, 80: 31}
 _ASM_TILES = True
 _KROT = os.environ.get("AVSD_KROT", "1") != "0"
 _KROT_ASM_ONLY = False
@@ -479,9 +481,25 @@
     w_rest: Optional[torch.Tensor] = None,
     out_rest: Optional[torch.Tensor] = None,
     w_frag: Optional[torch.Tensor] = None,
+    tattn: Optional[tuple] = None,
 ) -> torch.Tensor:
     _req(a, P.ACT, "a")
     _req(w, P.ACT, "w")
+    if tattn is not None:
+        t_heads, t_hw, t_frames = (int(v) for v in tattn)
+        t_bn = w.shape[0] // t_heads if t_heads > 0 else 0
+        t_d = TATTN_HEAD_DIMS.get(t_bn, 0)
+        if t_d == 0 or w.shape[0] != t_heads * t_bn or not temporal_attention_fused_supported(t_heads * t_d, t_heads, t_frames):
+            raise ValueError(f"gemm: tattn needs the head-major padded q|k|v weights of head width 40 / 80 ([heads * 128 or 256, K], got {tuple(w.shape)} "
+                             f"for {t_heads} heads), 12 or 24 frames (got {t_frames}) and single-plane storage")
+        if (ln is None or mode != PLAIN or a2 is not None or geglu or gelu or out_f32 or alpha != 1.0 or split_k != 1 or n is not None or k is not None or m is not None
+                or any(v is not None for v in (rowvec, res1, res2, rowstats, stats_pos, master, a_rest, a2_rest, w_rest, out_rest, w_frag))):
+            raise ValueError("gemm: tattn goes with ln (and ln_pos) and a bias only")
+        if t_hw <= 0 or a.shape[0] % (t_hw * t_frames) or (ln_pos is not None and tuple(ln_pos[1:]) != (t_hw, t_frames)):
+            raise ValueError("gemm: tattn rows are (branch, frame, pixel) — M must be whole branches of frames * hw rows, ln_pos of the same (hw, frames)")
+        if tile not in (0, TATTN_TILE[t_d]):
+            raise ValueError(f"gemm: tattn with head width {t_d} runs on the form of tile {TATTN_TILE[t_d]}")
+        tile = TATTN_TILE[t_d]
     planes = w_rest is not None
     if planes:
         if P.SPLIT:
@@ -555,6 +573,8 @@
     m_out = M
     if mode == CONV3 and d.ups == 2:
         m_out, n_out = 4 * M, N // 4
+    if tattn is not None:
+        n_out = t_heads * t_d
     if out is None:
         out = torch.empty((m_out, n_out), dtype=F32, device=a.device) if out_f32 else alloc16((m_out, n_out), a.device)
     else:
@@ -586,6 +606,9 @@
         d.out_master, d.ldm = _p(master), _ld(master)
     d.alpha = alpha
     d.mode = mode
+    if tattn is not None:
+        d.flags |= TATTN
+        d.hw, d.frames, d.heads, d.head_dim, d.attn_scale = t_hw, t_frames, t_heads, t_d, float(t_d) ** -0.5
     if rowstats is not None:
         _req(rowstats, F32, "rowstats")
         if not rowstats.is_contiguous() or rowstats.numel() != M * (N // 32) * 2:
@@ -726,6 +749,8 @@
         _TIMER.add_replay(fam, lambda dc=dc: check(_lib.lib().avsd_gemm_bf16(C.byref(dc), _stream()), "avsd_gemm_bf16"),
                           (a, a2, w, out, bias, rowvec, res1, res2, ws, rowstats, ln, master, stats_pos, ln_pos, a_rest, a2_rest, w_rest, w_frag, out_rest))
         subpix = mode == CONV3 and d.ups == 2
+        if tattn is not None:
+            N = 3 * t_heads * t_d
         _TIMER.stop(ev, fam, 2.0 * M * N * K * (3 if x2 else 1), 2.0 * M * K * (1.0 / (4 if subpix else 9) if mode == CONV3 else 1.0 / 3 if mode == TMIX else 1.0)
                     + 2.0 * N * K + _nbytes(out, res1, res2), flops_once=2.0 * M * N * K, flops_ref=2.0 * M * N * K * (2.25 if subpix else 1.0))
     return out
@@ -947,6 +972,10 @@
     _timed("attention", 4.0 * bq * heads * lq * lk * d * (3 if P.SPLIT else 1), _nbytes(q, out) + 4.0 * (bq // q_per_kv) * lk * Cc,
            (q, k, v, out, key_index), call)
     return out
+
+
+def temporal_attention_fused_supported(C: int, heads: int, frames: int) -> bool:
+    return not P.SPLIT and heads > 0 and C % heads == 0 and (C // heads) in TATTN_TILE and frames in (12, 24)
 
 
 def cross_attention_block_supported(C: int, heads: int, lk_pad: int, M: int, L: int) -> bool:
diff --git a/asva_amd/unet.py b/asva_amd/unet.py
--- a/asva_amd/unet.py
+++ b/asva_amd/unet.py
@@ -13,7 +13,7 @@
 
 from . import ops
 from .conditioning import mask_to_key_index
-from .weights import Blob, _Pk, _Ref, from_act, pack_conv1x1, pack_device, pack_frag, pack_geglu, pack_linear, subpixel_ups, to_act, to_planes
+from .weights import Blob, _Pk, _Ref, from_act, pack_conv1x1, pack_device, pack_frag, pack_geglu, pack_linear, pack_qkv_heads, qkv_heads_packable, subpixel_ups, to_act, to_planes
 
 CONFIG_NAME = "config.json"
 SAFETENSORS_NAME = "diffusion_pytorch_model.safetensors"
@@ -26,6 +26,8 @@
 
 _FUSE_LN = True
 _FUSE_LN_TEMP = True
+_FUSE_TATTN = os.environ.get("AVSD_FUSE_TATTN", "1") != "0"
+_FUSE_TATTN_DIMS = tuple(int(v) for v in os.environ.get("AVSD_FUSE_TATTN_DIMS", "40").split(",") if v)
 _F32_RES = os.environ.get("AVSD_F32_RESIDUAL", "0") != "0"
 _ATTN_FP8 = os.environ.get("AVSD_ATTN_FP8", "0") != "0"
 _FUSE_XATTN = True
@@ -696,7 +698,8 @@
                     ops.gemm(ab, tp.attn_audio.wkv, out=c.audio_kv)
                 self._xa_caches(c, tp, old.key_index, idx_frames, Fr)
             return old
-        blocks = [self.make_cond_block(tp, text, text_pf, audio, audio_pf, Fr, key_index, idx_frames) for tp in self._transformers(pk)]
+        blocks = [self.make_cond_block(tp, text, text_pf, audio, audio_pf, Fr, key_index, idx_frames, heads=hd)
+                  for tp, hd in zip(self._transformers(pk), self._transformer_heads(pk))]
         self._cond_version = getattr(self, "_cond_version", 0) + 1
         self._cond = _Pk(blocks=blocks, key_index=key_index, idx_frames=idx_frames, frames=Fr,
                          batch=text.shape[0] // text_pf, sig=sig, version=self._cond_version, share=share)
@@ -719,7 +722,7 @@
         c._xa_text, c._xa_audio = c.xa_text, c.xa_audio
 
     @staticmethod
-    def make_cond_block(tp, text, text_pf, audio, audio_pf, frames, key_index=None, idx_frames=None):
+    def make_cond_block(tp, text, text_pf, audio, audio_pf, frames, key_index=None, idx_frames=None, heads: int = 8):
         C = tp.dim
         c = _Pk()
         c.text_kv = ops.gemm(text.reshape(-1, text.shape[-1]), tp.attn2.wkv)
@@ -734,8 +737,20 @@
         hid = ops.linear_small_m(emb, tp.pos1.w, tp.pos1.b, act_out=True)
         c.pos = ops.linear_small_m(hid, tp.pos2.w, tp.pos2.b)
         c.posw = None if P.SPLIT else ops.linear_small_m(c.pos, tp.attn_temp.wqkv_ln, None)
+        c.tattn = None
+        if c.posw is not None and qkv_heads_packable(C, heads):
+            at = tp.attn_temp
+            wh, ch, bh = pack_qkv_heads(heads, at.wqkv_ln, at.sqkv_ln, at.bqkv_ln)
+            ph, = pack_qkv_heads(heads, c.posw.t().contiguous())
+            c.tattn = _Pk(heads=heads, w=wh, colsum=ch, bias=bh, posw=ph.t().contiguous())
         AudioUNet3DConditionModel._xa_caches(c, tp, key_index, idx_frames if idx_frames is not None else frames, frames)
         return c
+
+    def _transformer_heads(self, pk):
+        heads = _per_block(self.config.attention_head_dim, len(pk.down))
+        for blocks, hd in zip(list(pk.down) + [pk.mid] + list(pk.up), list(heads) + [heads[-1]] + list(heads[::-1])):
+            if blocks.attentions:
+                yield from [hd] * len(blocks.attentions)
 
     @staticmethod
     def _transformers(pk):
@@ -1022,12 +1037,18 @@
 
     fold_temp = fused and _FUSE_LN_TEMP and not P.SPLIT and getattr(c, "posw", None) is not None and hasattr(p.attn_temp, "wqkv_ln")
     h = cross(h, a2, p.norm2, getattr(c, "xa_text", None), fold_temp, text_attention, stats_pos=(c.pos, L, Fr) if fold_temp else None)
-    if fold_temp:
-        qkv = ops.gemm(h.lo, p.attn_temp.wqkv_ln, bias=p.attn_temp.bqkv_ln, ln=(stats[si], p.attn_temp.sqkv_ln, eps), ln_pos=(c.posw, L, Fr))
+    at = p.attn_temp
+    fused_ok = getattr(ops, "temporal_attention_fused_supported", None)
+    ta = getattr(c, "tattn", None)
+    if fold_temp and _FUSE_TATTN and ta is not None and ta.heads == heads and C // heads in _FUSE_TATTN_DIMS and fused_ok is not None and fused_ok(C, heads, Fr):
+        o = ops.gemm(h.lo, ta.w, bias=ta.bias, ln=(stats[si], ta.colsum, eps), ln_pos=(ta.posw, L, Fr), tattn=(heads, L, Fr))
     else:
-        nt = ops.layernorm(h.lo, p.norm_temp.g, p.norm_temp.b, pos=c.pos, hw=L, frames=Fr)
-        qkv = ops.gemm(nt, p.attn_temp.wqkv)
-    o = ops.temporal_attention(qkv, b=B, frames=Fr, hw=L, heads=heads)
+        if fold_temp:
+            qkv = ops.gemm(h.lo, at.wqkv_ln, bias=at.bqkv_ln, ln=(stats[si], at.sqkv_ln, eps), ln_pos=(c.posw, L, Fr))
+        else:
+            nt = ops.layernorm(h.lo, p.norm_temp.g, p.norm_temp.b, pos=c.pos, hw=L, frames=Fr)
+            qkv = ops.gemm(nt, at.wqkv)
+        o = ops.temporal_attention(qkv, b=B, frames=Fr, hw=L, heads=heads)
     h = stream(o, p.attn_temp.wo, p.attn_temp.bo, h)
     if fused:
         wf = getattr(p, "w1_ln_f", None)
diff --git a/asva_amd/weights.py b/asva_amd/weights.py
--- a/asva_amd/weights.py
+++ b/asva_amd/weights.py
@@ -101,6 +101,32 @@
     N, K = wp.shape
     assert N % 32 == 0 and K % 16 == 0
     return wp.reshape(N // 32, 32, K // 16, 2, 8).permute(0, 2, 3, 1, 4).contiguous().reshape(N // 32, K // 16, 64, 8)
+
+
+TATTN_BN = {40: 128, 80: 256}
+
+
+def qkv_heads_packable(C: int, heads: int) -> bool:
+    return not P.SPLIT and heads > 0 and C % heads == 0 and (C // heads) in TATTN_BN
+
+
+def qkv_head_order(C: int, heads: int) -> torch.Tensor:
+    d = C // heads
+    bn = TATTN_BN[d]
+    order = torch.full((heads, bn), -1, dtype=torch.long)
+    for part in range(3):
+        order[:, part * d:(part + 1) * d] = part * C + torch.arange(heads)[:, None] * d + torch.arange(d)[None, :]
+    return order.reshape(-1)
+
+
+def pack_qkv_heads(heads: int, w: torch.Tensor, *vecs: torch.Tensor):
+    C = w.shape[0] // 3
+    order = qkv_head_order(C, heads).to(w.device)
+    sel, pad = order.clamp(min=0), order < 0
+    out = [torch.where(pad[:, None], torch.zeros((), dtype=w.dtype, device=w.device), w[sel]).contiguous()]
+    for v in vecs:
+        out.append(torch.where(pad, torch.zeros((), dtype=v.dtype, device=v.device), v[..., sel]).contiguous())
+    return out
 
 
 def pad_rows(w: torch.Tensor, mult: int = 4) -> torch.Tensor:
diff --git a/include/avsd.h b/include/avsd.h
--- a/include/avsd.h
+++ b/include/avsd.h
@@ -23,7 +23,7 @@
 enum { AVSD_GEMM_PLAIN = 0, AVSD_GEMM_TMIX = 1, AVSD_GEMM_CONV3 = 2 };
 enum { AVSD_GEMM_GEGLU = 1, AVSD_GEMM_OUT_F32 = 2, AVSD_GEMM_GELU = 4, AVSD_GEMM_XCD_N = 8, AVSD_GEMM_ROWSTATS = 16,
        AVSD_GEMM_LNFUSE = 32, AVSD_GEMM_RES1_F32 = 64, AVSD_GEMM_RES2_F32 = 128, AVSD_GEMM_X2 = 256, AVSD_GEMM_KROT = 512, AVSD_GEMM_W_FRAG = 1024,
-       AVSD_GEMM_OUT_REST = 2048 };
+       AVSD_GEMM_OUT_REST = 2048, AVSD_GEMM_TATTN = 4096 };
 #define AVSD_GEMM_MAX_TILE 33
 #define AVSD_GEMM_MAX_TILE_X2 36
 #define AVSD_GEMM_TILE_256x160_8W 38
@@ -68,6 +68,8 @@
   const float* stats_pos;
   const float* ln_rowvec;
   int32_t pos_hw, pos_frames;
+  int32_t heads, head_dim;
+  float attn_scale;
 } avsd_gemm_desc;
 
 int avsd_gemm_bf16(const avsd_gemm_desc* desc_host, void* stream);
```

After: 85.91 steps/s (median of 6 runs). No clear change (+0.3%).
